# SDFIdk/malstroem

Measured on AMD Instinct MI355X. Metric: Mcells/s fill->D8->accum->label on 16384^2 f32 DEM, higher is better.
Workload: dtype f32 fill / f64 no-flats+D8+accum / u8 flowdir / i32 labels; 1 GPU; 16384x16384 float32 DEM (spectral fBm beta=2 seed 42 (SURVEY 8d recipe)): fill+depths -> no-flats fill -> D8 -> accumulation -> CCL+label_stats -> watersheds+label_count -> pour points; parallelism=1 GPU, one device context, fill_rounds=8, noflat_rounds=84, fill_tiles=70225, fill_visits=43501, fill_cycles=0, noflat_visits=412256, noflat_cycles=412256, nlabels=4637017, fill_algorithm=1, fill_launches=8, noflat_algorithm=2, pour_algorithm=1

## Files before the change

malstroem_amd/csrc/accum.hip:

```cpp
#include "common.hpp"
#include <type_traits>

namespace mh {
namespace {

constexpr int AT = 64;
constexpr int PERIM = 4 * AT - 4;
constexpr int NODE_STRIDE = 256;
constexpr int FS = AT + 32;
constexpr int WOFF = 16;
constexpr uint64_t SRC = 1ull << 63;
constexpr uint64_t TAINT = 1ull << 63;
constexpr uint32_t TAINT32 = 1u << 31;
constexpr int R_SHIFT = 13;
constexpr uint32_t A_MASK = 0x1fffu, R_MASK = 0xfffu, SENT13 = A_MASK;
constexpr uint16_t NO_EXIT = 0xffffu;
#ifndef ACC_ATN
#define ACC_ATN 256
#endif
constexpr int ATN = ACC_ATN;
constexpr int CPT = AT * AT / ATN;
constexpr int MAX_DOUBLINGS = 12;
constexpr int G_SHIFT = 44;
constexpr uint64_t G_ONE = 1ull << G_SHIFT, G_SUM = G_ONE - 1, G_PEND = 0x7ffffull;
// ... 614 lines not shown
        if (d != 0ull && (r0 + r) < H && (c0 + c) < W && !halo_row(r0 + r)) {
            const uint32_t kk = atomicAdd(&wl_n, 1u);
            wl_cell[kk] = (uint32_t)(r * AT + c);
            wl_add[kk] = d;
        }
    }
    for (int side = 0; side < 2; ++side) {
        const int64_t hr = side == 0 ? 0 : H - 1;
        if ((side == 0 ? !fixed_top : !fixed_bot) || hr < r0 || hr >= r0 + AT) continue;
        if (tid < AT && c0 + tid < W) {
            const int r = (int)(hr - r0), c = tid;
            const unsigned code = fd[hr * W + c0 + c];
            const double X = out[hr * W + c0 + c];
            if (code <= 7u && dir_dr((int)code) != 0 && X > 0.0) {
                const int nr = r + dir_dr((int)code), nc = c + dir_dc((int)code);
                if (nr >= 0 && nr < AT && nc >= 0 && nc < AT && (r0 + nr) < H && (c0 + nc) < W && !halo_row(r0 + nr)) {
                    const uint32_t kk = atomicAdd(&wl_n, 1u);
                    wl_cell[kk] = (uint32_t)(nr * AT + nc);
                    wl_add[kk] = (unsigned long long)X;
                }
            }
        }
    }
    __syncthreads();
    const uint32_t nw = wl_n;
    for (uint32_t w = tid; w < nw; w += ATN) {
        uint32_t a = wl_cell[w];
        const unsigned long long v = wl_add[w];
        do {
            if (S[a] == 0ull) break;
            atomicAdd(&S[a], v);
            a = P[a];
        } while (a != SENT13);
    }
    __syncthreads();
    for (int i = tid; i < AT * AT; i += ATN) {
        const int r = i / AT, c = i - r * AT;
        const int64_t rr = r0 + r, cc = c0 + c;
        if (rr < H && cc < W && !halo_row(rr)) out[rr * W + cc] = (double)S[i];
    }
}
}

int accum_band_delta_dev(const uint8_t *d_fd, double *d_out, int64_t H, int64_t W, hipStream_t s, int fixed_top, int fixed_bot, AccumKeep *keep, bool *done)
{
    *done = false;
    if (!keep || !keep->valid || keep->H != H || keep->W != W || keep->fixed_top != fixed_top || keep->fixed_bot != fixed_bot || !keep->nodes.p) return MHIP_OK;
    static const bool off = [] { const char *e = dev_env("MHIP_BAND_ACC"); return e && std::string(e) == "full"; }();
    if (off) return MHIP_OK;
    const int ntr = (int)cdiv(H, AT), ntc = (int)cdiv(W, AT);
    const int64_t ntiles = (int64_t)ntr * ntc, nnodes = ntiles * NODE_STRIDE;
    char *b = keep->nodes.as<char>();
    Nodes nd;
    nd.gstate = reinterpret_cast<uint64_t *>(b + keep->o[0]);
    nd.inflow = reinterpret_cast<uint64_t *>(b + keep->o[1]);
    nd.arrived = reinterpret_cast<uint32_t *>(b + keep->o[2]);
    nd.next = reinterpret_cast<int32_t *>(b + keep->o[3]);
    nd.dst = reinterpret_cast<int32_t *>(b + keep->o[4]);
    nd.exit_of = reinterpret_cast<uint16_t *>(b + keep->o[5]);
    nd.flags = reinterpret_cast<uint8_t *>(b + keep->o[6]);
    nd.halo_first = reinterpret_cast<int32_t *>(b + keep->o[7]);
    nd.bexit = reinterpret_cast<int32_t *>(b + keep->o[8]);
    DevBuf aux;
    MH_TRY(aux.alloc((size_t)ntiles + 64));
    uint8_t *touched = aux.as<uint8_t>() + 64;
    unsigned int *flag = aux.as<unsigned int>();
    MH_HIP(hipMemsetAsync(aux.p, 0, (size_t)ntiles + 64, s));
    MH_HIP(hipMemsetAsync(nd.inflow, 0, 8 * (size_t)nnodes, s));
    hipLaunchKernelGGL(accum_delta_graph_kernel, dim3((unsigned)cdiv(2 * W, 256)), dim3(256), 0, s, nd, d_fd, (const double *)d_out, H, W, ntc, ntiles, fixed_top,
                       fixed_bot, touched, flag);
    MH_HIP(hipGetLastError());
    unsigned int h_flag = 0;
    MH_HIP(hipMemcpyAsync(&h_flag, flag, 4, hipMemcpyDeviceToHost, s));
    MH_HIP(stream_sync(s));
    keep->valid = false;
    if (h_flag) return MHIP_OK;
    hipLaunchKernelGGL(accum_delta_tile_kernel, dim3((unsigned)ntiles), dim3(ATN), 0, s, d_fd, d_out, H, W, ntc, nd, fixed_top, fixed_bot, (const uint8_t *)touched);
    MH_HIP(hipGetLastError());
    MH_HIP(stream_sync(s));
    *done = true;
    return MHIP_OK;
}

int accum_dev(const uint8_t *d_fd, double *d_out, int64_t H, int64_t W, hipStream_t s, int fixed_top, int fixed_bot, int halo_zero,
              int32_t *d_exit_map, PourLink *pour, AccumKeep *keep)
{
    const int ntr = (int)cdiv(H, AT), ntc = (int)cdiv(W, AT);
    const int64_t ntiles = (int64_t)ntr * ntc, nnodes = ntiles * NODE_STRIDE;
    if (nnodes >= (int64_t)INT32_MAX || H * W >= (1ll << 37)) {
        set_error("accumulated_flow: raster too large for the int32 perimeter-node domain");
        return MHIP_ELIMIT;
    }
    DevBuf buf;
    auto align = [](size_t x) { return (x + 255) & ~size_t(255); };
    const size_t o_gstate = 0, o_inflow = align(o_gstate + 8 * (size_t)nnodes), o_arrived = align(o_inflow + 8 * (size_t)nnodes);
    const size_t o_next = align(o_arrived + 4 * (size_t)nnodes), o_dst = align(o_next + 4 * (size_t)nnodes);
    const size_t o_exit = align(o_dst + 4 * (size_t)nnodes), o_flags = align(o_exit + 2 * (size_t)nnodes);
    const size_t o_halo = align(o_flags + (size_t)nnodes);
    const size_t o_bexit = align(o_halo + (d_exit_map ? 8 * (size_t)W : 0));
    MH_TRY(buf.alloc(o_bexit + (d_exit_map ? 4 * (size_t)nnodes : 0)));
    char *b = buf.as<char>();
    Nodes nd;
    nd.gstate = reinterpret_cast<uint64_t *>(b + o_gstate);
    nd.inflow = reinterpret_cast<uint64_t *>(b + o_inflow);
    nd.arrived = reinterpret_cast<uint32_t *>(b + o_arrived);
    nd.next = reinterpret_cast<int32_t *>(b + o_next);
    nd.dst = reinterpret_cast<int32_t *>(b + o_dst);
    nd.exit_of = reinterpret_cast<uint16_t *>(b + o_exit);
    nd.flags = reinterpret_cast<uint8_t *>(b + o_flags);
    nd.halo_first = d_exit_map ? reinterpret_cast<int32_t *>(b + o_halo) : nullptr;
    nd.bexit = d_exit_map ? reinterpret_cast<int32_t *>(b + o_bexit) : nullptr;
    if (d_exit_map) MH_HIP(hipMemsetAsync(nd.halo_first, 0xff, 8 * (size_t)W, s));
    MH_HIP(hipMemsetAsync(nd.inflow, 0, o_next - o_inflow, s));
    const unsigned gn = (unsigned)cdiv(nnodes, 256);
    const bool walk_final = (!(fixed_top || fixed_bot) || halo_zero) && (!d_exit_map || halo_zero) && H * W < (int64_t)0x7fffffff;
    if (walk_final)
        hipLaunchKernelGGL((accum_tile_kernel<false, false, true>), dim3((unsigned)ntiles), dim3(ATN), 0, s, d_fd, d_out, H, W, ntc, nd, fixed_top, fixed_bot, halo_zero);
    else if ((fixed_top || fixed_bot) && !halo_zero)
        hipLaunchKernelGGL((accum_tile_kernel<false, true>), dim3((unsigned)ntiles), dim3(ATN), 0, s, d_fd, d_out, H, W, ntc, nd, fixed_top, fixed_bot, halo_zero);
    else
        hipLaunchKernelGGL((accum_tile_kernel<false, false>), dim3((unsigned)ntiles), dim3(ATN), 0, s, d_fd, d_out, H, W, ntc, nd, fixed_top, fixed_bot, halo_zero);
    hipLaunchKernelGGL(accum_link_kernel, dim3(gn), dim3(256), 0, s, nd, nnodes);
    if (d_exit_map)
        hipLaunchKernelGGL(accum_band_exit_kernel, dim3((unsigned)cdiv(2 * W, 256)), dim3(256), 0, s, nd, H, W, ntc, ntiles, fixed_top, fixed_bot, d_exit_map);
    hipLaunchKernelGGL(accum_mark_kernel, dim3(gn), dim3(256), 0, s, nd, nnodes);
    hipLaunchKernelGGL(accum_graph_walk_kernel, dim3(gn), dim3(256), 0, s, nd, nnodes);
    if (walk_final) {
        PourCandDev pc;
        if (pour && pour->wait && pour->wait(pour->arg) == 1 && pour->dev.key) {
            MH_HIP(hipStreamWaitEvent(s, pour->ev, 0));
            pc = pour->dev;
            pour->consumed = true;
        }
        hipLaunchKernelGGL(accum_final_walk_kernel, dim3((unsigned)ntiles), dim3(ATN), 0, s, d_fd, d_out, H, W, ntc, nd, pc, fixed_top, fixed_bot);
    }
    else if ((!(fixed_top || fixed_bot) || halo_zero) && H * W < (int64_t)0x7fffffff)
        hipLaunchKernelGGL((accum_tile_kernel<true, false>), dim3((unsigned)ntiles), dim3(ATN), 0, s, d_fd, d_out, H, W, ntc, nd, fixed_top, fixed_bot, halo_zero);
    else
        hipLaunchKernelGGL((accum_tile_kernel<true, true>), dim3((unsigned)ntiles), dim3(ATN), 0, s, d_fd, d_out, H, W, ntc, nd, fixed_top, fixed_bot, halo_zero);
    MH_HIP(hipGetLastError());
    MH_HIP(stream_sync(s));
    if (keep) {
        keep->valid = false;
        if (d_exit_map) {
            keep->nodes.release();
            keep->nodes.p = buf.p; keep->nodes.bytes = buf.bytes;
            buf.p = nullptr; buf.bytes = 0;
            const size_t offs[9] = {o_gstate, o_inflow, o_arrived, o_next, o_dst, o_exit, o_flags, o_halo, o_bexit};
            for (int k = 0; k < 9; ++k) keep->o[k] = offs[k];
            keep->H = H; keep->W = W; keep->fixed_top = fixed_top; keep->fixed_bot = fixed_bot;
            keep->valid = true;
        }
    }
#ifdef MH_PROFILE_ACCUM
    {
        unsigned long long pr[2][8];
        MH_HIP(hipMemcpyFromSymbol(pr, HIP_SYMBOL(g_accum_prof), sizeof(pr)));
        for (int f = 0; f < 2; ++f)
            fprintf(stderr, "[accum profile phase %d] ticks/tile (thread 0): load=%.0f init=%.0f solve=%.0f publish/write=%.0f\n", f ? 3 : 1,
                    pr[f][0] / (double)ntiles, pr[f][1] / (double)ntiles, pr[f][2] / (double)ntiles, pr[f][3] / (double)ntiles);
        unsigned long long z[2][8] = {};
        MH_HIP(hipMemcpyToSymbol(HIP_SYMBOL(g_accum_prof), z, sizeof(z)));
    }
#endif
    return MHIP_OK;
}

}
```

malstroem_amd/csrc/common.hpp:

```cpp
#pragma once
#include <hip/hip_runtime.h>
#include <cstdint>
#include <cstdio>
#include <cstring>
#include <string>
#include <vector>

#include "../../include/malstroem_hip.h"

struct mhip_polygons;
struct mhip_flowpaths;

namespace mh {

void set_error(const char *fmt, ...);
const char *get_error();
const char *dev_env(const char *name);
hipError_t stream_sync(hipStream_t s);
int require_device();

#define MH_HIP(expr)                                                                             \
    do {                                                                                         \
        hipError_t _e = (expr);                                                                  \
        if (_e != hipSuccess) {                                                                  \
// ... 164 lines not shown
};
void noflat_seed(FillRun &f, const float *d_filled, double sh, double dg, int64_t ncells_global);
struct PfRun;
struct FillHandover {
    PfRun *run = nullptr;
    const float *dem = nullptr;
    float *filled = nullptr, *depths = nullptr;
    int64_t H = 0, W = 0;
    const uint16_t *bslot = nullptr;
    const uint32_t *tabV = nullptr;
    int ntr = 0, ntc = 0;
    bool pending = false, queued = false, violated = false, repaired = false;
    bool suspect = false;
    FillStats st_repair;
    FillHandover() = default;
    FillHandover(const FillHandover &) = delete;
    FillHandover &operator=(const FillHandover &) = delete;
    ~FillHandover();
    void release();
};
int fill_handover_complete(FillHandover *ho, hipStream_t s);
int fill_handover_repair(FillHandover *ho, hipStream_t s);
int fill_plain_dev(const float *d_dem, float *d_out, int64_t H, int64_t W, hipStream_t s, FillStats *st, float *d_depths = nullptr,
                   bool *depths_done = nullptr, FillHandover *ho = nullptr);
int fill_check_f32_dev(const float *d_dem, const float *d_filled, int64_t H, int64_t W, int fixed_top, int fixed_bot, hipStream_t s,
                       unsigned int *d_flag);
int fill_plain_pflood_dev(const float *d_dem, float *d_out, float *d_depths, int64_t H, int64_t W, hipStream_t s, FillStats *st, bool *violated = nullptr,
                          uint32_t *overflow = nullptr, FillHandover *ho = nullptr);
struct PfRun {
    const float *dem = nullptr;
    float *out = nullptr;
    int64_t H = 0, W = 0;
    int fixed_top = 0, fixed_bot = 0;
    uint32_t overflow = 0;
    struct Impl;
    Impl *impl;
    PfRun();
    ~PfRun();
    PfRun(const PfRun &) = delete;
    PfRun &operator=(const PfRun &) = delete;
    int begin(hipStream_t s);
    int halo_changed(int side, hipStream_t s);
    int batch(hipStream_t s);
    int finish(hipStream_t s, float *d_depths, FillStats *st, bool *violated = nullptr, FillHandover *ho = nullptr);
    int finish_late(hipStream_t s, float *d_depths, bool *violated);
    int proof_flag(hipStream_t s, unsigned int *h_flag);
    int solve(hipStream_t s);
    int pack(hipStream_t s, int row0, int nrows);
    int publish_edges(hipStream_t s);
};
struct StageHook {
    enum Point { FIRST_VISIT = 0, TAIL_ROUNDS = 1, FINISH = 3 };
    void (*fn)(void *, hipStream_t) = nullptr;
    void *arg = nullptr;
    bool fired = false;
    int at = TAIL_ROUNDS;
    void fire(hipStream_t s)
    {
        if (fn && !fired) {
            fired = true;
            fn(arg, s);
        }
    }
    void fire_at(int point, hipStream_t s)
    {
        if (point == at) fire(s);
    }
};

struct GeoRun {
    const float *dem = nullptr, *filled = nullptr;
    double *out = nullptr;
    uint32_t *dist = nullptr;
    int64_t H = 0, W = 0;
    double sh = 0, dg = 0;
    int fixed_top = 0, fixed_bot = 0;
    bool allow_partial = false;
    double seed_add = 0;
    bool partial = false;
    StageHook *tail_hook = nullptr;
    uint8_t *d8_out = nullptr;
    unsigned int *d8_nodir = nullptr;
    bool d8_done = false;
    FillHandover *handover = nullptr;
    struct Impl;
    Impl *impl;
    GeoRun();
    ~GeoRun();
    GeoRun(const GeoRun &) = delete;
    GeoRun &operator=(const GeoRun &) = delete;
    int begin(hipStream_t s, bool *applicable, bool *active);
    int batch(hipStream_t s, bool *active);
    int halo_changed(int side, hipStream_t s);
    int end(hipStream_t s, bool *ok, FillStats *st);
    int launch_rounds(hipStream_t s, int nb);
};
struct D8Sink {
    uint8_t *flowdir = nullptr;
    unsigned int *nodir = nullptr;
    bool done = false;
};
int fill_noflat_geodesic_dev(const float *d_dem, const float *d_filled, double *d_out, int64_t H, int64_t W, double sh, double dg, double seed_add,
                             hipStream_t s, FillStats *st, bool *partial, StageHook *tail_hook = nullptr, D8Sink *d8 = nullptr, FillHandover *ho = nullptr);
int noflat_verify_dev(const float *d_dem, const double *d_out, int64_t H, int64_t W, double sh, double dg, hipStream_t s, bool *ok, int fixed_top = 0,
                      int fixed_bot = 0);
int fill_noflat_dev(const float *d_dem, double *d_out, int64_t H, int64_t W, double sh, double dg, hipStream_t s,
                    FillStats *st = nullptr, const float *d_filled = nullptr, StageHook *tail_hook = nullptr, D8Sink *d8 = nullptr,
                    FillHandover *ho = nullptr);
int short_diag_dev(const float *d_dem, int64_t n, double *sh, double *dg, hipStream_t s);
int depths_dev(const float *d_filled, const float *d_dem, float *d_out, int64_t n, hipStream_t s);
int d8_dev(const double *d_z, uint8_t *d_out, int64_t H, int64_t W, int edges_outward, hipStream_t s, int64_t row_off = 0,
           int64_t Hg = 0, unsigned int *d_interior_nodir = nullptr);
void short_diag_from_minmax(float mn, float mx, bool has_nan, double *sh, double *dg);
int minmax_dev(const float *d_x, int64_t n, float *mn, float *mx, int *has_nan, hipStream_t s);
int row_update_dev(void *d_dst, const void *d_src, int64_t nbytes, int *changed, hipStream_t s);
int copy_bandwidth_dev(size_t bytes, int reps, double *gbs, hipStream_t s);
int read_bandwidth_dev(size_t bytes, int reps, double *gbs, hipStream_t s);
int row_update_async(void *d_dst, const void *d_src, int64_t nbytes, int *d_changed, hipStream_t s);
int trace_downstream_dev(const uint8_t *d_fd, const int32_t *d_lab, int64_t H, int64_t W, const int64_t *d_cells, int64_t n, int use_bg,
                         int32_t bg, int32_t *d_label, int32_t *d_found, int64_t *d_len, const int64_t *d_offsets, int64_t *d_out_cells,
                         hipStream_t s);
int comm_unique_id(void *id128);
int comm_available();
int comm_create(void **comm, const void *id128, int rank, int nranks);
void comm_destroy(void *comm);
int comm_exchange_rows(void *comm, int rank, int nranks, const void *first_row, const void *last_row, void *stage, size_t rowbytes,
                       hipStream_t s);
int comm_allreduce_max(void *comm, double *d_value, hipStream_t s);
struct PourCandDev {
    uint16_t *mask0 = nullptr;
    uint2 *list = nullptr;
    uint32_t *tile_cnt = nullptr;
    unsigned long long *tile_key0 = nullptr;
    uint32_t *flags = nullptr;
    int components = 0;
    unsigned long long *key = nullptr;
    uint32_t nlab = 0;
};
constexpr uint32_t POUR_TILE_CAP = 512;
struct PourLink {
    PourCandDev dev;
    hipEvent_t ev = nullptr;
    void (*notify)(void *, int) = nullptr;
    int (*wait)(void *) = nullptr;
    void *arg = nullptr;
    bool consumed = false;
};
struct AccumKeep {
    DevBuf nodes;
    size_t o[9] = {};
    int64_t H = 0, W = 0;
    int fixed_top = 0, fixed_bot = 0;
    bool valid = false;
};
int accum_dev(const uint8_t *d_fd, double *d_out, int64_t H, int64_t W, hipStream_t s, int fixed_top = 0, int fixed_bot = 0, int halo_zero = 0,
              int32_t *d_exit_map = nullptr, PourLink *pour = nullptr, AccumKeep *keep = nullptr);
int accum_band_delta_dev(const uint8_t *d_fd, double *d_out, int64_t H, int64_t W, hipStream_t s, int fixed_top, int fixed_bot, AccumKeep *keep, bool *done);
int ccl8_f32_dev(const float *d_data, int32_t *d_labels, int32_t *d_tmp, int64_t H, int64_t W, int64_t *nlabels,
                 hipStream_t s, DevBuf *stats_out = nullptr);
int label_emit_stats_dev(const int32_t *d_parent, const unsigned long long *d_rootbits, const uint32_t *d_wordprefix, const float *d_data,
                         int32_t *d_labels, int64_t H, int64_t W, int64_t nlab, mhip_stat_record *d_rec, hipStream_t s);
int ccl8_u8_dev(const uint8_t *d_data, int32_t *d_labels, int32_t *d_tmp, int64_t H, int64_t W, int64_t *nlabels,
                hipStream_t s);
struct CclKeep {
    DevBuf bits, wprefix;
    int64_t H = 0, W = 0, nlocal = 0;
    bool valid = false;
};
int ccl8_f32_begin_dev(const float *d_data, int32_t *d_labels, int32_t *d_tmp, int64_t H, int64_t W, int64_t *nlabels, hipStream_t s, CclKeep *keep);
int ccl_emit_rows_dev(const int32_t *d_parent, const unsigned long long *d_rootbits, const uint32_t *d_wordprefix, int32_t *d_labels, int64_t base,
                      int64_t count, hipStream_t s);
int label_emit_sparse_dev(const int32_t *d_parent, const unsigned long long *d_rootbits, const uint32_t *d_wordprefix, const float *d_data,
                          int32_t *d_labels, int64_t H, int64_t W, int ht, int64_t H_owned, int64_t nlocal, int32_t offset,
                          const int32_t *d_dropped, const int32_t *d_target, int32_t ndropped, int64_t nlab_global, mhip_stat_record *d_rec,
                          hipStream_t s);
int relabel_lut_dev(int32_t *d_labels, const int32_t *d_lut, int64_t nlab, int64_t n, hipStream_t s);
int relabel_range_dev(int32_t *d_labels, int64_t n, int32_t lo, int32_t hi, const int32_t *d_lut, const int32_t *d_fid, const int32_t *d_fnew, int32_t nf,
                      hipStream_t s);
int band_trace_dev(const uint8_t *d_fd, const int32_t *d_lab, int64_t Hl, int64_t W, int64_t row_lo, int64_t own0, int64_t own1, int64_t Hg,
                   const int64_t *d_cells, const int32_t *d_src, int64_t n, int use_bg, int32_t bg, int32_t *d_label, int32_t *d_status,
                   int32_t *d_src_out, int64_t *d_exit, int64_t *d_len, const int64_t *d_offsets, int64_t *d_out_cells, hipStream_t s);
int relabel_sparse_dev(int32_t *d_labels, int64_t n, int64_t nlocal, int32_t offset, const int32_t *d_dropped, const int32_t *d_target,
                       int32_t ndropped, hipStream_t s);
int keep_mask_dev(const int32_t *d_labels, const uint8_t *d_keep, int64_t nlab, int64_t n, uint8_t *d_mask,
                  hipStream_t s);
int label_stats_dev(const float *d_data, const int32_t *d_labels, int64_t n, int64_t nlab, mhip_stat_record *d_rec,
                    hipStream_t s, int64_t W = 0, bool components = false);
int label_stats64_dev(const double *d_data, const int32_t *d_labels, int64_t n, int64_t nlab, mhip_stat_record *d_rec, hipStream_t s);
int label_stats_zero_sign_dev(const float *d_data, const int32_t *d_labels, int64_t n, int64_t nlab, mhip_stat_record *d_rec, hipStream_t s);
int label_stats_zero_sign_dev(const double *d_data, const int32_t *d_labels, int64_t n, int64_t nlab, mhip_stat_record *d_rec, hipStream_t s);
int label_arg_dev(const double *d_data, const int32_t *d_labels, int64_t H, int64_t W, int64_t nlab, bool is_max,
                  mhip_index_record *d_rec, hipStream_t s, bool components = false);
int label_count_dev(const int32_t *d_labels, int64_t n, int64_t nlab, int64_t *d_counts, hipStream_t s, int64_t W = 0);
int label_max_dev(const int32_t *d_labels, int64_t n, int32_t *out_max, hipStream_t s);
constexpr int64_t HYPS_MAX_BINS = (int64_t)1 << 30;
int hyps_layout_dev(const double *d_dmax, int64_t stride, int64_t nlab, double res, int64_t *d_offsets, int64_t *total, hipStream_t s);
int hyps_table_dev(const float *d_data, const int32_t *d_labels, int64_t n, int64_t W, int64_t nlab, double res, const int64_t *d_offsets,
                   int64_t total, uint32_t *d_counts, double *d_sums, int64_t *lds_spills, hipStream_t s, hipEvent_t ev0 = nullptr,
                   hipEvent_t ev1 = nullptr);
int hyps_levels_dev(int64_t nlab, const int64_t *d_offsets, const uint32_t *d_counts, const double *d_sums, const double *d_dmax, int64_t stride,
                    const double *d_q, mhip_final_record *d_rec, hipStream_t s);
int final_depths_dev(const float *d_data, const int32_t *d_labels, int64_t n, int64_t W, int64_t nlab, mhip_final_record *d_rec, float *d_out,
                     hipStream_t s, hipEvent_t ev0 = nullptr, hipEvent_t ev1 = nullptr);
bool wet_at_events_ok(int64_t K, const float *values);
int wet_at_dev(const float *d_data, const int32_t *d_labels, int64_t n, int64_t W, int64_t nlab, int K, const double *d_drawdown, int64_t stride,
               const float *values, float *d_out, int64_t *d_wet, int64_t wet_stride, hipStream_t s, hipEvent_t ev0 = nullptr,
               hipEvent_t ev1 = nullptr);
bool flow_distance_scale_ok(double scale);
int flow_distance_dev(const uint8_t *d_fd, const int32_t *d_lab, int64_t H, int64_t W, double scale, int64_t nlab, float *d_out, mhip_index_record *d_rec,
                      int64_t *unresolved, hipStream_t s);
int burn_check(int64_t nseg, const mhip_burn_segment *segs, int64_t nline, const mhip_burn_line *lines, const mhip_burn_result *results);
int burn_lines_dev(float *d_dem, int64_t H, int64_t W, int64_t nseg, const mhip_burn_segment *segs, int64_t nline, const mhip_burn_line *lines,
                   double nodata, mhip_burn_result *results, hipStream_t s);
int zones_check(int64_t H, int64_t W, int64_t nvert, const double *xy, int64_t nring, const int64_t *ring_offsets, const int32_t *ring_zone,
                int64_t nzone, int grow);
int zones_rasterize_dev(int32_t *d_out, int64_t H, int64_t W, int64_t nvert, const double *xy, int64_t nring, const int64_t *ring_offsets,
                        const int32_t *ring_zone, int64_t nzone, int grow, hipStream_t s);
int zone_stats_dev(const float *d_data, const int32_t *d_zones, int64_t n, int64_t W, int64_t nzone, mhip_zone_record *d_rec, hipStream_t s);
int polygonize_check(int64_t H, int64_t W);
int polygons_fetch_dev(const mhip_polygons *p, int32_t *xy, int64_t *ring_offsets, int32_t *ring_label);
int polygonize_dev(const int32_t *d_lab, int64_t H, int64_t W, DevBuf &d_xy, DevBuf &d_off, DevBuf &d_rl, int64_t *nring, int64_t *nvert, hipStream_t s);
int flowpaths_check(int64_t H, int64_t W, double threshold);
int flowpaths_dev(const uint8_t *d_fd, const double *d_acc, const int32_t *d_lab, int64_t H, int64_t W, double threshold, mhip_flowpaths *p, hipStream_t s);
int flowpaths_fetch_dev(const mhip_flowpaths *p, int32_t *xy, int64_t *reach_offsets, mhip_reach_record *records);
int watersheds_dev(const uint8_t *d_fd, int32_t *d_labels, int64_t H, int64_t W, int32_t unassigned, hipStream_t s,
                   bool band_mode = false, const unsigned int *d_known_interior_nodir = nullptr, const int32_t *d_src = nullptr, PourLink *pour = nullptr);
int pour_finish_dev(unsigned long long *d_key, const unsigned long long *d_tile_key0, int64_t ntiles, int64_t nlab, int64_t W, mhip_index_record *d_rec,
                    hipStream_t s);
int band_pseudo_labels_dev(int32_t *d_ws, int64_t H, int64_t W, int top, int bottom, hipStream_t s);
int negative_lut_dev(int32_t *d_lab, int64_t n, const int32_t *d_lut, int64_t nlut, hipStream_t s);
constexpr int32_t BAND_ROOT = 1, BAND_ROOTLESS = 0x7fffffff;
int band_root_labels_dev(int32_t *d_out, int64_t H, int64_t W, int64_t row_off, int64_t Hg, hipStream_t s);
int band_hide_rootless_dev(const int32_t *d_lab, const int32_t *d_rooted, int32_t *d_out, int64_t n, hipStream_t s);
int band_show_rootless_dev(int32_t *d_ws, const int32_t *d_lab, int64_t n, hipStream_t s);

__host__ __device__ inline int64_t cdiv(int64_t a, int64_t b) { return (a + b - 1) / b; }

constexpr int TR = 32;
struct TileGeom {
// ... 88 lines not shown
```

malstroem_amd/csrc/ctx.hip:

```cpp
#include <mutex>
#include <new>
#include <string>
#include <vector>

#include "ctx.hpp"

namespace mh {

static void drop_hyps(mhip_ctx *c)
{
    c->hyps_total = -1;
    c->have[MHIP_R_FINALDEPTHS] = false;
    c->wetat_events = -1;
    c->wetat_out.release();
}

static void drop_flow_distance(mhip_ctx *c)
{
    std::lock_guard<std::mutex> lk(c->fdist_mu);
    c->fdist_unresolved = -1;
    c->fdist_out.release();
    c->fdist_rec.release();
}

void ctx_wrote(mhip_ctx *c, int which, bool uploaded)
{
    switch (which) {
    case MHIP_R_DEM:
        for (int k = 0; k < MHIP_R_COUNT_; ++k) {
            if (k == MHIP_R_DEM) continue;
            c->have[k] = false;
            ctx_wrote(c, k, true);
        }
        break;
    case MHIP_R_FILLED:
        if (uploaded) c->fill_st.have_minmax = false;
        break;
    case MHIP_R_DEPTHS:
        c->stats_valid = false;
        drop_hyps(c);
        break;
    case MHIP_R_NOFLAT:
        c->pour_valid = false;
        break;
    case MHIP_R_FLOWDIR:
        c->nodir_valid = false;
        c->flowdir_own = false;
        c->acc_keep.valid = false;
        drop_flow_distance(c);
        break;
    case MHIP_R_ACCUM:
        c->acc_keep.valid = false;
        c->pour_valid = false;
        break;
    case MHIP_R_LABELS:
        c->nlabels = c->nlabels_raw = -1;
        c->labels_components = false;
        c->stats_valid = false;
        c->ws_counts_valid = false;
        c->pour_valid = false;
        drop_hyps(c);
        drop_flow_distance(c);
        break;
    case MHIP_R_WATERSHEDS:
        c->ws_counts_valid = false;
        break;
    default:
        break;
    }
}

int ctx_copy_rows(mhip_ctx *c, void *dev_base, size_t elem_bytes, int64_t row0, int64_t nrows, void *host, hipMemcpyKind kind)
{
    MH_HIP(hipSetDevice(c->device));
    const size_t rowb = elem_bytes * (size_t)c->W;
    char *dev = (char *)dev_base + rowb * (size_t)(c->ht + row0);
    const bool up = kind == hipMemcpyHostToDevice;
    MH_HIP(hipMemcpyAsync(up ? (void *)dev : host, up ? host : (void *)dev, rowb * (size_t)nrows, kind, cs(c)));
    MH_HIP(stream_sync(cs(c)));
    return MHIP_OK;
}

int ctx_fetch(mhip_ctx *c, const DevBuf &buf, size_t bytes, void *host)
{
    MH_HIP(hipSetDevice(c->device));
    return download(host, buf, bytes, c->stream);
}

int ctx_fork_join_events(mhip_ctx *c)
{
    if (c->ev_fork) return MHIP_OK;
    for (hipEvent_t *e : {&c->ev_flowdir, &c->ev_join, &c->ev_label, &c->ev_tail, &c->ev_fork}) MH_HIP(hipEventCreateWithFlags(e, hipEventDisableTiming));
    return MHIP_OK;
}

int ctx_ensure_labels_final(mhip_ctx *c, hipStream_t s)
{
    if (!c->labels_filtered) return ctx_apply_keep_on(c, nullptr, s);
    return MHIP_OK;
}

int ctx_label_max(mhip_ctx *c, hipStream_t s)
{
    if (c->nlabels < 0) {
        int32_t m = 0;
        MH_TRY(label_max_dev(c->r[MHIP_R_LABELS].as<int32_t>(), c->H * c->W, &m, s));
        c->nlabels = m < 0 ? 0 : m;
    }
    return MHIP_OK;
}

int ctx_apply_keep_on(mhip_ctx *c, const uint8_t *keep, hipStream_t s)
{
    MH_ARG(c && c->have[MHIP_R_LABELS] && c->nlabels_raw >= 0 && !c->labels_filtered, "ctx_apply_keep needs a fresh LABEL run");
    const int64_t n = c->H * c->W;
    const int64_t nraw = c->nlabels_raw;
    const bool components = c->labels_components;
    ctx_wrote(c, MHIP_R_LABELS);
    c->nlabels_raw = nraw;
    c->labels_components = components;
    if (keep) {
        std::vector<int32_t> lut;
        c->nlabels = build_rank_lut(keep, c->nlabels_raw, lut);
        DevBuf d_lut;
        MH_TRY(d_lut.alloc(lut.size() * 4));
        MH_HIP(hipMemcpyAsync(d_lut.p, lut.data(), lut.size() * 4, hipMemcpyHostToDevice, s));
        MH_TRY(relabel_lut_dev(c->r[MHIP_R_LABELS].as<int32_t>(), d_lut.as<int32_t>(), c->nlabels_raw, n, s));
        MH_TRY(c->stats.alloc(sizeof(mhip_stat_record) * (size_t)(c->nlabels + 1)));
        MH_TRY(label_stats_dev(c->r[MHIP_R_DEPTHS].as<float>(), c->r[MHIP_R_LABELS].as<int32_t>(), n, c->nlabels,
                               c->stats.as<mhip_stat_record>(), s, c->W, c->labels_components));
    } else {
        c->nlabels = c->nlabels_raw;
        MH_TRY(c->stats.alloc(sizeof(mhip_stat_record) * (size_t)(c->nlabels + 1)));
        MH_HIP(hipMemcpyAsync(c->stats.p, c->raw_stats.p, sizeof(mhip_stat_record) * (size_t)(c->nlabels + 1),
                              hipMemcpyDeviceToDevice, s));
    }
    c->labels_filtered = true;
    c->stats_valid = true;
    return MHIP_OK;
}

}

using namespace mh;

extern "C" {

int mhip_comm_available(void) { return comm_available(); }

int mhip_comm_unique_id(void *id128)
{
    MH_ARG(id128, "comm_unique_id(id128)");
    MH_TRY(require_device());
    return comm_unique_id(id128);
}

int mhip_ctx_create_band(mhip_ctx **out, int64_t H_global, int64_t W, int64_t row0, int64_t H_local, int device, int rank,
                         int nranks, const void *nccl_unique_id)
{
    MH_ARG(out && H_global >= 1 && W >= 1 && H_local >= 1 && row0 >= 0 && row0 + H_local <= H_global, "ctx_create_band geometry");
    MH_ARG(rank >= 0 && nranks >= 1 && rank < nranks, "ctx_create_band(rank, nranks)");
    MH_TRY(require_device());
    MH_HIP(hipSetDevice(device));
    void *comm = nullptr;
    if (nccl_unique_id) MH_TRY(comm_create(&comm, nccl_unique_id, rank, nranks));
    mhip_ctx *c = new mhip_ctx();
    c->comm = comm;
    c->ht = row0 > 0 ? 1 : 0;
    c->hb = row0 + H_local < H_global ? 1 : 0;
    c->H_owned = H_local;
    c->H = H_local + c->ht + c->hb;
    c->W = W; c->H_global = H_global; c->row0 = row0;
    c->device = device; c->rank = rank; c->nranks = nranks;
    int prio_least = 0, prio_greatest = 0;
    (void)hipDeviceGetStreamPriorityRange(&prio_least, &prio_greatest);
    if (hipStreamCreateWithPriority(&c->stream, hipStreamDefault, prio_greatest) != hipSuccess) {
        comm_destroy(c->comm);
        delete c;
        set_error("hipStreamCreate failed");
        return MHIP_EHIP;
    }
    *out = c;
    return MHIP_OK;
}

int mhip_ctx_create(mhip_ctx **out, int64_t H, int64_t W, int device)
{
    return mhip_ctx_create_band(out, H, W, 0, H, device, 0, 1, nullptr);
}

int mhip_ctx_destroy(mhip_ctx *c)
{
    if (!c) return MHIP_OK;
    (void)hipSetDevice(c->device);
    (void)stream_sync(c->stream);
    for (StageTimer &t : c->timers)
        for (hipEvent_t e : {t.a, t.b})
            if (e) (void)hipEventDestroy(e);
    (void)hipStreamDestroy(c->stream);
    for (hipStream_t st : {c->stream_b, c->stream_c}) {
        if (st) {
            (void)stream_sync(st);
            (void)hipStreamDestroy(st);
        }
    }
    for (hipEvent_t e : {c->ev_fork, c->ev_flowdir, c->ev_join, c->ev_label, c->ev_tail, c->ev_cand})
        if (e) (void)hipEventDestroy(e);
    delete c->geo;
    delete c->pf;
    delete c->run[0];
    delete c->run[1];
    comm_destroy(c->comm);
    comm_destroy(c->comm_b);
    delete c;
    return MHIP_OK;
}

int mhip_ctx_comm_add_side(mhip_ctx *c, const void *nccl_unique_id)
{
    MH_ARG(c && nccl_unique_id && c->comm && !c->comm_b, "ctx_comm_add_side(ctx, id) needs a band context with a communicator and no side communicator yet");
    MH_HIP(hipSetDevice(c->device));
    return comm_create(&c->comm_b, nccl_unique_id, c->rank, c->nranks);
}

int mhip_ctx_side_begin(mhip_ctx *c)
{
    MH_ARG(c, "ctx");
    MH_HIP(hipSetDevice(c->device));
    if (!c->stream_b) MH_HIP(hipStreamCreateWithFlags(&c->stream_b, hipStreamNonBlocking));
    MH_TRY(ctx_fork_join_events(c));
    MH_HIP(hipEventRecord(c->ev_fork, c->stream));
    MH_HIP(hipStreamWaitEvent(c->stream_b, c->ev_fork, 0));
    t_side_ctx = c;
    return MHIP_OK;
}

int mhip_ctx_side_end(mhip_ctx *c)
{
    MH_ARG(c && t_side_ctx == c, "ctx_side_end without ctx_side_begin on this thread");
    MH_HIP(hipSetDevice(c->device));
    MH_HIP(stream_sync(c->stream_b));
    t_side_ctx = nullptr;
    return MHIP_OK;
}

int mhip_ctx_upload(mhip_ctx *c, int which, const void *host)
{
    MH_ARG(c && host && which >= 0 && which < MHIP_R_COUNT_, "ctx_upload(ctx, which, host)");
    return mhip_ctx_upload_rows(c, which, 0, c->H_owned, host);
}

int mhip_ctx_upload_dem(mhip_ctx *c, const float *dem) { return mhip_ctx_upload(c, MHIP_R_DEM, dem); }

int mhip_ctx_upload_rows(mhip_ctx *c, int which, int64_t row0, int64_t nrows, const void *host)
{
    MH_ARG(c && host && which >= 0 && which < MHIP_R_COUNT_ && row0 >= 0 && nrows >= 1 && row0 + nrows <= c->H_owned,
           "ctx_upload_rows(ctx, which, row0, nrows, host)");
    MH_HIP(hipSetDevice(c->device));
    MH_TRY(ctx_raster(c, which));
    ctx_wrote(c, which, true);
    c->have[which] = false;
    MH_TRY(ctx_copy_rows(c, c->r[which].p, raster_elem(which), row0, nrows, const_cast<void *>(host), hipMemcpyHostToDevice));
    if (row0 + nrows == c->H_owned) {
        c->have[which] = true;
        if (which == MHIP_R_LABELS) c->labels_filtered = true;
    }
    return MHIP_OK;
}

int mhip_ctx_download_rows(mhip_ctx *c, int which, int64_t row0, int64_t nrows, void *host)
{
    MH_ARG(c && host && which >= 0 && which < MHIP_R_COUNT_ && row0 >= 0 && nrows >= 1 && row0 + nrows <= c->H_owned,
           "ctx_download_rows(ctx, which, row0, nrows, host)");
    MH_ARG(c->have[which], "raster has not been computed or uploaded");
    return ctx_copy_rows(c, c->r[which].p, raster_elem(which), row0, nrows, host, hipMemcpyDeviceToHost);
}

int mhip_ctx_download(mhip_ctx *c, int which, void *host)
{
    MH_ARG(c && host && which >= 0 && which < MHIP_R_COUNT_, "ctx_download(ctx, which, host)");
    return mhip_ctx_download_rows(c, which, 0, c->H_owned, host);
}

int mhip_ctx_trace_downstream(mhip_ctx *c, const int64_t *cells_rc, int64_t n, int use_background, int32_t background, int32_t *out_label,
                              int32_t *out_found, int64_t *out_len, const int64_t *offsets, int64_t *out_cells)
{
    MH_ARG(c && n >= 0 && (n == 0 || cells_rc), "ctx_trace_downstream(ctx, cells, n, ...)");
    MH_ARG(c->have[MHIP_R_FLOWDIR] && c->have[MHIP_R_LABELS], "ctx_trace_downstream needs flow directions and labels");
    MH_ARG(!c->ht && !c->hb, "stream tracing runs on an undivided raster");
    if (n == 0) return MHIP_OK;
    MH_HIP(hipSetDevice(c->device));
    return trace_on_device(c->r[MHIP_R_FLOWDIR].as<uint8_t>(), c->r[MHIP_R_LABELS].as<int32_t>(), c->H, c->W, cells_rc, n, use_background,
                           background, out_label, out_found, out_len, offsets, out_cells, c->stream);
}

int mhip_ctx_sync(mhip_ctx *c)
{
    MH_ARG(c, "ctx");
    MH_HIP(stream_sync(c->stream));
    return MHIP_OK;
}

int mhip_ctx_stage_ms(mhip_ctx *c, int stage, float *ms)
{
    MH_ARG(c && ms, "ctx_stage_ms(ctx, stage, ms)");
    const int k = timer_slot(stage);
    MH_ARG(k >= 0 && c->timers[k].valid, "stage has not been run");
    MH_HIP(hipEventSynchronize(c->timers[k].b));
    MH_HIP(hipEventElapsedTime(ms, c->timers[k].a, c->timers[k].b));
    return MHIP_OK;
}

int mhip_ctx_kernel_ms(mhip_ctx *c, const char *kernel, float *ms_total, int32_t *launches)
{
    MH_ARG(c && kernel && ms_total && launches, "ctx_kernel_ms(ctx, kernel, ms, launches)");
    const std::string k(kernel);
    if (k == "d8") {
        *launches = 1;
        return mhip_ctx_stage_ms(c, MHIP_STAGE_FLOWDIR, ms_total);
    }
    if (k == "d8_steady") {
        MH_ARG(c->have[MHIP_R_NOFLAT] && !c->ht && !c->hb, "d8_steady needs the no-flats surface on an undivided context");
        MH_HIP(hipSetDevice(c->device));
        MH_TRY(ctx_raster(c, MHIP_R_FLOWDIR));
        MH_TRY(c->nodir_cnt.alloc(4));
        constexpr int REPS = 16;
        StageTimer *t;
        MH_TRY(ctx_timer(c, D8_STEADY_SLOT, &t));
        hipStream_t s = c->stream;
        ctx_wrote(c, MHIP_R_FLOWDIR);
        MH_HIP(hipMemsetAsync(c->nodir_cnt.p, 0, 4, s));
        for (int i = 0; i < REPS + 2; ++i) {
            if (i == 2) MH_HIP(hipEventRecord(t->a, s));
            MH_TRY(d8_dev(c->r[MHIP_R_NOFLAT].as<double>(), c->r[MHIP_R_FLOWDIR].as<uint8_t>(), c->H, c->W, 1, s, 0, c->H_global,
                          c->nodir_cnt.as<unsigned int>()));
        }
        MH_HIP(hipEventRecord(t->b, s));
        MH_HIP(hipEventSynchronize(t->b));
        MH_HIP(hipEventElapsedTime(ms_total, t->a, t->b));
        c->have[MHIP_R_FLOWDIR] = true;
        c->nodir_valid = true;
        c->flowdir_own = true;
        *launches = REPS;
        return MHIP_OK;
    }
    if (k == "hyps_table" || k == "final_depths") {
        *launches = 1;
        return mhip_ctx_stage_ms(c, k == "hyps_table" ? HYPS_KERNEL_SLOT : FINAL_KERNEL_SLOT, ms_total);
    }
    if (k == "wet_at") {
        *launches = 1;
        return mhip_ctx_stage_ms(c, WETAT_KERNEL_SLOT, ms_total);
    }
    if (k == "fill_round") {
        *launches = c->fill_rounds;
        return mhip_ctx_stage_ms(c, MHIP_STAGE_FILL, ms_total);
    }
    if (k == "noflat_round") {
        *launches = c->noflat_rounds;
        return mhip_ctx_stage_ms(c, MHIP_STAGE_NOFLAT, ms_total);
    }
    set_error("unknown kernel family '%s'", kernel);
    return MHIP_EINVAL;
}

int mhip_ctx_get_i64(mhip_ctx *c, const char *key, int64_t *value)
{
    MH_ARG(c && key && value, "ctx_get_i64(ctx, key, value)");
    const std::string k(key);
    if (k == "nlabels_raw") *value = c->nlabels_raw;
    else if (k == "nlabels") {
        if (c->nlabels < 0 && c->have[MHIP_R_LABELS]) {
            MH_HIP(hipSetDevice(c->device));
            MH_TRY(ctx_label_max(c, c->stream));
        }
        *value = c->nlabels;
    }
    else if (k == "fill_rounds") *value = c->fill_rounds;
    else if (k == "noflat_rounds") *value = c->noflat_rounds;
    else if (k == "fill_visits") *value = c->fill_st.visits;
    else if (k == "fill_cycles") *value = c->fill_st.cycles;
    else if (k == "fill_tiles") *value = c->fill_st.tiles;
    else if (k == "fill_algorithm") *value = c->fill_st.algorithm;
    else if (k == "fill_handover") *value = c->fill_handover;
    else if (k == "fill_handover_rechecks") *value = c->fill_handover_rechecks;
    else if (k == "fill_overflow") *value = c->fill_st.overflow;
    else if (k == "fill_launches") *value = c->fill_st.rounds;
    else if (k == "fill_hot_launches") *value = c->fill_st.hot_launches;
    else if (k == "noflat_hot_launches") *value = c->noflat_st.hot_launches;
    else if (k == "accum_algorithm") *value = c->accum_algorithm;
    else if (k == "flowdir_computed") *value = (c->have[MHIP_R_FLOWDIR] && c->flowdir_own) ? 1 : 0;
    else if (k == "pour_algorithm") *value = c->pour_algorithm;
    else if (k == "noflat_algorithm") *value = c->noflat_st.algorithm;
    else if (k == "noflat_visits") *value = c->noflat_st.visits;
    else if (k == "noflat_reject") *value = c->noflat_st.geo_reject;
    else if (k == "noflat_reject_irregular") *value = c->noflat_st.geo_irregular;
    else if (k == "noflat_reject_unreached") *value = c->noflat_st.geo_unreached;
    else if (k == "noflat_reject_mismatch") *value = c->noflat_st.geo_mismatch;
    else if (k == "noflat_cycles") *value = c->noflat_st.cycles;
    else if (k == "hyps_bins") *value = c->hyps_total;
    else if (k == "hyps_lds_spills") *value = c->hyps_spills;
    else if (k == "wet_at_events") *value = c->wetat_events;
    else if (k == "flow_distance_unresolved") *value = c->fdist_unresolved;
    else if (k == "zones") *value = c->nzone;
    else if (k == "H") *value = c->H;
    else if (k == "W") *value = c->W;
    else {
        set_error("unknown key '%s'", key);
        return MHIP_EINVAL;
    }
    return MHIP_OK;
}

int mhip_ctx_get_f64(mhip_ctx *c, const char *key, double *value)
{
    MH_ARG(c && key && value, "ctx_get_f64(ctx, key, value)");
    const std::string k(key);
    if (k == "short") *value = c->sh;
    else if (k == "diag") *value = c->dg;
    else if (k == "fill_hot_ms") *value = c->fill_st.hot_ms;
    else if (k == "noflat_hot_ms") *value = c->noflat_st.hot_ms;
    else {
        set_error("unknown key '%s'", key);
        return MHIP_EINVAL;
    }
    return MHIP_OK;
}

int mhip_ctx_raw_stats(mhip_ctx *c, mhip_stat_record *records)
{
    MH_ARG(c && records && c->raw_stats.p && c->nlabels_raw >= 0, "ctx_raw_stats needs a LABEL run");
    return ctx_fetch(c, c->raw_stats, sizeof(mhip_stat_record) * (size_t)(c->nlabels_raw + 1), records);
}

int mhip_ctx_apply_keep(mhip_ctx *c, const uint8_t *keep)
{
    MH_ARG(c, "ctx");
    MH_HIP(hipSetDevice(c->device));
    return ctx_apply_keep_on(c, keep, c->stream);
}

int mhip_ctx_stats(mhip_ctx *c, mhip_stat_record *records)
{
    MH_ARG(c && records && c->stats_valid && c->labels_filtered, "ctx_stats needs LABEL + apply_keep (or mhip_ctx_hyps) on the resident depths and labels");
    return ctx_fetch(c, c->stats, sizeof(mhip_stat_record) * (size_t)(c->nlabels + 1), records);
}

int mhip_ctx_watershed_counts(mhip_ctx *c, int64_t *counts)
{
    MH_ARG(c && counts && c->ws_counts_valid, "ctx_watershed_counts needs a WATERSHED run on the resident labels");
    return ctx_fetch(c, c->ws_counts, 8 * (size_t)(c->nlabels + 1), counts);
}

int mhip_ctx_pourpoints(mhip_ctx *c, mhip_index_record *records)
{
    MH_ARG(c && records && c->pour_valid, "ctx_pourpoints needs a POURPOINTS run on the resident labels and accumulated flow");
    return ctx_fetch(c, c->pour, sizeof(mhip_index_record) * (size_t)(c->nlabels + 1), records);
}

int mhip_ctx_hyps(mhip_ctx *c, double res, int64_t *total)
{
    MH_ARG(c && total && hyps_res_ok(res), "ctx_hyps(ctx, 0 < res < inf, total)");
    MH_ARG(!(c->nranks > 1 || c->ht || c->hb), "hypsometry on a row band is not built (the tables of the bands add up: a later step); use an undivided context");
    MH_ARG(c->have[MHIP_R_DEPTHS] && c->have[MHIP_R_LABELS] && !c->ccl_pending, "ctx_hyps needs the DEPTHS and LABELS rasters");
    MH_ARG(c->labels_filtered, "ctx_hyps needs mhip_ctx_apply_keep after the LABEL run");
    MH_HIP(hipSetDevice(c->device));
    hipStream_t s = c->stream;
    const int64_t n = c->H * c->W;
    c->hyps_total = -1;
    if (!c->stats_valid) {
        MH_TRY(ctx_label_max(c, s));
        MH_TRY(c->stats.alloc(sizeof(mhip_stat_record) * (size_t)(c->nlabels + 1)));
        MH_TRY(label_stats_dev(c->r[MHIP_R_DEPTHS].as<float>(), c->r[MHIP_R_LABELS].as<int32_t>(), n, c->nlabels, c->stats.as<mhip_stat_record>(), s,
                               c->W, c->labels_components));
        c->stats_valid = true;
    }
// ... 252 lines not shown
```

malstroem_amd/csrc/ctx.hpp:

```cpp
#pragma once
#include <atomic>
#include <condition_variable>
#include <functional>
#include <mutex>
#include <thread>

#include "common.hpp"

namespace mh {

class SideThread {
    std::thread th_;
    std::mutex mu_;
    std::condition_variable cv_;
    std::function<void()> task_;
    bool busy_ = false, stop_ = false;

public:
    ~SideThread()
    {
        {
            std::lock_guard<std::mutex> lk(mu_);
            stop_ = true;
        }
        cv_.notify_all();
        if (th_.joinable()) th_.join();
    }
    void run(std::function<void()> f)
    {
        std::unique_lock<std::mutex> lk(mu_);
        if (!th_.joinable())
            th_ = std::thread([this] {
                std::unique_lock<std::mutex> l2(mu_);
                for (;;) {
                    cv_.wait(l2, [this] { return stop_ || (busy_ && task_); });
                    if (stop_) return;
                    std::function<void()> f2 = std::move(task_);
                    task_ = nullptr;
                    l2.unlock();
                    f2();
                    l2.lock();
                    busy_ = false;
                    cv_.notify_all();
                }
            });
        task_ = std::move(f);
        busy_ = true;
        cv_.notify_all();
    }
    void wait()
    {
        std::unique_lock<std::mutex> lk(mu_);
        cv_.wait(lk, [this] { return !busy_; });
    }
};

struct StageTimer {
    hipEvent_t a = nullptr, b = nullptr;
    bool valid = false;
};
constexpr int N_STAGE_BITS = 9;
constexpr int WETAT_KERNEL_SLOT = 1 << 27, FINAL_KERNEL_SLOT = 1 << 28, HYPS_KERNEL_SLOT = 1 << 29, D8_STEADY_SLOT = 1 << 30;
constexpr int N_TIMERS = N_STAGE_BITS + 4;

}

struct mhip_ctx {
    mh::SideThread side;
    int64_t H = 0, W = 0;
    int64_t H_global = 0, row0 = 0, H_owned = 0;
    int ht = 0, hb = 0;
    mh::FillRun *run[2] = {nullptr, nullptr};
    mh::GeoRun *geo = nullptr;
    uint32_t pf_overflow = 0;
    mh::PfRun *pf = nullptr;
    bool pf_done = false;
    mh::DevBuf nodir_cnt;
    bool nodir_valid = false;
    bool flowdir_own = false;
    int device = 0, rank = 0, nranks = 1;
    hipStream_t stream = nullptr;
    mh::DevBuf r[MHIP_R_COUNT_];
    bool have[MHIP_R_COUNT_] = {};
    mh::DevBuf tmp_i32;
    mh::CclKeep ccl_keep;
    bool ccl_pending = false;
    bool pf_depths = false;
    mh::DevBuf raw_stats, stats, ws_counts, pour;
    mh::AccumKeep acc_keep;
    int accum_algorithm = 0;
    mh::DevBuf pp_mask0, pp_list, pp_tiles, pp_misc, pp_key;
    hipEvent_t ev_cand = nullptr;
    int pour_algorithm = 0;
    int64_t nlabels_raw = -1, nlabels = -1;
    bool labels_components = false;
    bool labels_filtered = false;
    std::atomic<bool> stats_valid{false};
    std::atomic<bool> ws_counts_valid{false};
    std::atomic<bool> pour_valid{false};
    mh::DevBuf hyps_off, hyps_cnt, hyps_sum, hyps_rec;
    int64_t hyps_total = -1, hyps_spills = 0;
    mh::DevBuf wetat_out;
    int wetat_events = -1;
    mh::DevBuf fdist_out, fdist_rec;
    std::atomic<int64_t> fdist_unresolved{-1};
    std::mutex fdist_mu;
    mh::DevBuf zones;
    int64_t nzone = -1;
    double sh = 0, dg = 0;
    int32_t fill_rounds = 0, noflat_rounds = 0;
    int64_t fill_handover_rechecks = 0;
    int32_t fill_handover = 0;
    mh::FillStats fill_st, noflat_st;
    mh::StageTimer timers[mh::N_TIMERS];
    void *comm = nullptr;
    void *comm_b = nullptr;
    mh::DevBuf comm_stage, comm_word, comm_flags, comm_stage_b;
    hipStream_t stream_b = nullptr, stream_c = nullptr;
    hipEvent_t ev_fork = nullptr, ev_flowdir = nullptr, ev_join = nullptr, ev_label = nullptr, ev_tail = nullptr;
};

namespace mh {

inline size_t raster_elem(int which)
{
    switch (which) {
    case MHIP_R_DEM: case MHIP_R_FILLED: case MHIP_R_DEPTHS: case MHIP_R_LABELS: case MHIP_R_WATERSHEDS: case MHIP_R_NGDIST:
    case MHIP_R_FINALDEPTHS: return 4;
    case MHIP_R_NOFLAT: case MHIP_R_ACCUM: return 8;
    case MHIP_R_FLOWDIR: return 1;
    default: return 0;
    }
}

inline int ctx_raster(mhip_ctx *c, int which)
{
    if (!c->r[which].p) MH_TRY(c->r[which].alloc(raster_elem(which) * (size_t)(c->H * c->W)));
    return MHIP_OK;
}

inline int timer_slot(int stage)
{
    for (int b = 0; b < N_STAGE_BITS; ++b)
        if (stage == 1 << b) return b;
    return stage == FINAL_KERNEL_SLOT ? N_STAGE_BITS : stage == HYPS_KERNEL_SLOT ? N_STAGE_BITS + 1 : stage == D8_STEADY_SLOT ? N_STAGE_BITS + 2 :
           stage == WETAT_KERNEL_SLOT ? N_STAGE_BITS + 3 : -1;
}
inline int ctx_timer(mhip_ctx *c, int stage, StageTimer **t)
{
    const int k = timer_slot(stage);
    MH_ARG(k >= 0, "not a stage");
    *t = &c->timers[k];
    if (!(*t)->a) {
        hipEvent_t e0, e1;
        MH_HIP(hipEventCreate(&e0));
        MH_HIP(hipEventCreate(&e1));
        (*t)->a = e0;
        (*t)->b = e1;
    }
    return MHIP_OK;
}
inline int stage_begin(mhip_ctx *c, int stage, hipStream_t s)
{
    StageTimer *t;
    MH_TRY(ctx_timer(c, stage, &t));
    MH_HIP(hipEventRecord(t->a, s));
    return MHIP_OK;
}
inline int stage_end(mhip_ctx *c, int stage, hipStream_t s)
{
    StageTimer &t = c->timers[timer_slot(stage)];
    MH_HIP(hipEventRecord(t.b, s));
    t.valid = true;
    return MHIP_OK;
}

inline thread_local mhip_ctx *t_side_ctx = nullptr;
static inline hipStream_t cs(mhip_ctx *c) { return (t_side_ctx == c && c->stream_b) ? c->stream_b : c->stream; }
static inline bool on_side(mhip_ctx *c) { return t_side_ctx == c; }

void ctx_wrote(mhip_ctx *c, int which, bool uploaded = false);
int ctx_copy_rows(mhip_ctx *c, void *dev_base, size_t elem_bytes, int64_t row0, int64_t nrows, void *host, hipMemcpyKind kind);
int ctx_fetch(mhip_ctx *c, const DevBuf &buf, size_t bytes, void *host);
int ctx_fork_join_events(mhip_ctx *c);
int ctx_apply_keep_on(mhip_ctx *c, const uint8_t *keep, hipStream_t s);
int ctx_ensure_labels_final(mhip_ctx *c, hipStream_t s);
int ctx_label_max(mhip_ctx *c, hipStream_t s);

}
```

malstroem_amd/csrc/ctx_band.hip:

```cpp
#include <string>

#include "ctx.hpp"

using namespace mh;

static size_t row_bytes(mhip_ctx *c, int which) { return raster_elem(which) * (size_t)c->W; }
static char *row_ptr(mhip_ctx *c, int which, int side)
{
    const int64_t row = side == 0 ? c->ht : side == 1 ? c->ht + c->H_owned - 1 : side == 2 ? 0 : c->H - 1;
    return c->r[which].as<char>() + row_bytes(c, which) * (size_t)row;
}

static int update_halo_rows(mhip_ctx *c, int which, const void *top, const void *bottom, int *d_flags, int32_t *changed, hipStream_t s)
{
    const int64_t rowb = (int64_t)row_bytes(c, which);
    MH_HIP(hipMemsetAsync(d_flags, 0, 8, s));
    if (top) MH_TRY(row_update_async(row_ptr(c, which, 2), top, rowb, d_flags, s));
    if (bottom) MH_TRY(row_update_async(row_ptr(c, which, 3), bottom, rowb, d_flags + 1, s));
    int h[2] = {0, 0};
    MH_HIP(hipMemcpyAsync(h, d_flags, 8, hipMemcpyDeviceToHost, s));
    MH_HIP(stream_sync(s));
    changed[0] = h[0];
    changed[1] = h[1];
    return MHIP_OK;
}

static int copy_edge_rows(mhip_ctx *c, int which, int side0, void *dst0, int side1, void *dst1, hipMemcpyKind kind, const char *usage)
{
    MH_ARG(c && which >= 0 && which < MHIP_R_COUNT_, usage);
    MH_ARG(c->r[which].p, "raster has not been computed or uploaded");
    const int side[2] = {side0, side1};
    void *const dst[2] = {dst0, dst1};
    for (int k = 0; k < 2; ++k) MH_ARG(!dst[k] || side[k] < 2 || (side[k] == 2 ? c->ht : c->hb), "this band has no halo row on that side");
    if (!dst0 && !dst1) return MHIP_OK;
    MH_HIP(hipSetDevice(c->device));
    hipStream_t s = cs(c);
    for (int k = 0; k < 2; ++k)
        if (dst[k]) MH_HIP(hipMemcpyAsync(dst[k], row_ptr(c, which, side[k]), row_bytes(c, which), kind, s));
    MH_HIP(stream_sync(s));
    return MHIP_OK;
}

static void labels_renumbered(mhip_ctx *c, int64_t nlabels)
{
    const bool components = c->labels_components;
    ctx_wrote(c, MHIP_R_LABELS);
    c->labels_components = components;
    c->nlabels = c->nlabels_raw = nlabels;
    c->labels_filtered = true;
}

static FillRun *new_fill_run(mhip_ctx *c, int kind)
{
    delete c->run[kind];
    FillRun *f = c->run[kind] = new FillRun();
    f->noflat = kind != 0;
    f->dem = c->r[MHIP_R_DEM].as<float>();
    f->out = c->r[kind ? MHIP_R_NOFLAT : MHIP_R_FILLED].p;
    f->H = c->H; f->W = c->W;
    f->fixed_top = c->ht; f->fixed_bot = c->hb;
    f->rounds_per_batch = 16;
    return f;
}
static bool fill_begun(mhip_ctx *c, int kind) { return c->run[kind] || (kind == 0 && (c->pf || c->pf_done)); }

extern "C" {


int mhip_ctx_band_info(mhip_ctx *c, int64_t *row_off, int64_t *rows_local, int32_t *halo_top, int32_t *halo_bottom)
{
    MH_ARG(c, "ctx");
    if (row_off) *row_off = c->row0 - c->ht;
    if (rows_local) *rows_local = c->H;
    if (halo_top) *halo_top = c->ht;
    if (halo_bottom) *halo_bottom = c->hb;
    return MHIP_OK;
}

int mhip_ctx_get_edge_row(mhip_ctx *c, int which, int side, void *host)
{
    static const char *const usage = "ctx_get_edge_row(ctx, which, side, host)";
    MH_ARG(host && side >= 0 && side <= 3, usage);
    return copy_edge_rows(c, which, side, host, 0, nullptr, hipMemcpyDeviceToHost, usage);
}

int mhip_ctx_set_halo_row(mhip_ctx *c, int which, int side, const void *host, int32_t *changed)
{
    MH_ARG(c && host && which >= 0 && which < MHIP_R_COUNT_ && (side == 0 || side == 1), "ctx_set_halo_row(ctx, which, side, host)");
    MH_ARG(side == 0 ? c->ht : c->hb, "this band has no halo row on that side");
    int32_t ch[2];
    MH_TRY(mhip_ctx_set_halo_rows(c, which, side == 0 ? host : nullptr, side == 1 ? host : nullptr, ch));
    if (changed) *changed = ch[side];
    return MHIP_OK;
}

int mhip_ctx_get_edge_row_dev(mhip_ctx *c, int which, int side, void *dev_dst)
{
    static const char *const usage = "ctx_get_edge_row_dev(ctx, which, side, dev)";
    MH_ARG(dev_dst && side >= 0 && side <= 3, usage);
    return copy_edge_rows(c, which, side, dev_dst, 0, nullptr, hipMemcpyDeviceToDevice, usage);
}

int mhip_ctx_set_halo_row_dev(mhip_ctx *c, int which, int side, const void *dev_src, int32_t *changed)
{
    MH_ARG(c && dev_src && which >= 0 && which < MHIP_R_COUNT_ && (side == 0 || side == 1), "ctx_set_halo_row_dev(ctx, which, side, dev)");
    MH_ARG(side == 0 ? c->ht : c->hb, "this band has no halo row on that side");
    MH_HIP(hipSetDevice(c->device));
    MH_TRY(ctx_raster(c, which));
    int ch = 0;
    MH_TRY(row_update_dev(row_ptr(c, which, 2 + side), dev_src, (int64_t)row_bytes(c, which), &ch, cs(c)));
    if (changed) *changed = ch;
    return MHIP_OK;
}

int mhip_ctx_get_edge_rows(mhip_ctx *c, int which, void *host_first, void *host_last)
{
    return copy_edge_rows(c, which, 0, host_first, 1, host_last, hipMemcpyDeviceToHost, "ctx_get_edge_rows(ctx, which, first, last)");
}

int mhip_ctx_set_halo_rows(mhip_ctx *c, int which, const void *host_top, const void *host_bottom, int32_t *changed)
{
    MH_ARG(c && changed && which >= 0 && which < MHIP_R_COUNT_, "ctx_set_halo_rows(ctx, which, top, bottom, changed[2])");
    MH_ARG((!host_top || c->ht) && (!host_bottom || c->hb), "this band has no halo row on that side");
    changed[0] = changed[1] = 0;
    if (!host_top && !host_bottom) return MHIP_OK;
    MH_HIP(hipSetDevice(c->device));
    MH_TRY(ctx_raster(c, which));
    hipStream_t s = cs(c);
    const size_t rowb = row_bytes(c, which);
    DevBuf &stage = on_side(c) ? c->comm_stage_b : c->comm_stage;
    DevBuf flags;
    MH_TRY(stage.alloc(2 * rowb));
    MH_TRY(flags.alloc(8));
    char *top = stage.as<char>(), *bottom = top + rowb;
    if (host_top) MH_HIP(hipMemcpyAsync(top, host_top, rowb, hipMemcpyHostToDevice, s));
    if (host_bottom) MH_HIP(hipMemcpyAsync(bottom, host_bottom, rowb, hipMemcpyHostToDevice, s));
    return update_halo_rows(c, which, host_top ? top : nullptr, host_bottom ? bottom : nullptr, flags.as<int>(), changed, s);
}

int mhip_ctx_exchange_halo(mhip_ctx *c, int which, int32_t *changed)
{
    MH_ARG(c && changed && which >= 0 && which < MHIP_R_COUNT_, "ctx_exchange_halo(ctx, which, changed[2])");
    MH_ARG(c->comm || c->nranks == 1, "this band context has no RCCL communicator (created without an ncclUniqueId)");
    changed[0] = changed[1] = 0;
    if (!c->ht && !c->hb) return MHIP_OK;
    MH_ARG(c->r[which].p, "raster has not been computed or uploaded");
    MH_HIP(hipSetDevice(c->device));
    hipStream_t s = cs(c);
    const size_t rowb = row_bytes(c, which);
    MH_TRY(c->comm_stage.alloc(2 * rowb));
    MH_TRY(c->comm_flags.alloc(8));
    char *from_up = c->comm_stage.as<char>(), *from_down = from_up + rowb;
    MH_TRY(comm_exchange_rows(c->comm, c->rank, c->nranks, row_ptr(c, which, 0), row_ptr(c, which, 1), from_up, rowb, s));
    return update_halo_rows(c, which, c->ht ? from_up : nullptr, c->hb ? from_down : nullptr, c->comm_flags.as<int>(), changed, s);
}

int mhip_ctx_exchange_edge_rows(mhip_ctx *c, int which, void *host_from_up, void *host_from_down)
{
    MH_ARG(c && which >= 0 && which < MHIP_R_COUNT_, "ctx_exchange_edge_rows(ctx, which, from_up, from_down)");
    void *comm = on_side(c) ? c->comm_b : c->comm;
    MH_ARG(comm || c->nranks == 1, on_side(c) ? "this band context has no side communicator (mhip_ctx_comm_add_side)"
                                              : "this band context has no RCCL communicator (created without an ncclUniqueId)");
    if (!c->ht && !c->hb) return MHIP_OK;
    MH_ARG(c->r[which].p, "raster has not been computed or uploaded");
    MH_ARG((!c->ht || host_from_up) && (!c->hb || host_from_down), "ctx_exchange_edge_rows: a buffer per neighbour");
    MH_HIP(hipSetDevice(c->device));
    hipStream_t s = cs(c);
    const size_t rowb = row_bytes(c, which);
    DevBuf &stage = on_side(c) ? c->comm_stage_b : c->comm_stage;
    MH_TRY(stage.alloc(2 * rowb));
    MH_TRY(comm_exchange_rows(comm, c->rank, c->nranks, row_ptr(c, which, 0), row_ptr(c, which, 1), stage.p, rowb, s));
    if (c->ht) MH_HIP(hipMemcpyAsync(host_from_up, stage.p, rowb, hipMemcpyDeviceToHost, s));
    if (c->hb) MH_HIP(hipMemcpyAsync(host_from_down, stage.as<char>() + rowb, rowb, hipMemcpyDeviceToHost, s));
    MH_HIP(stream_sync(s));
    return MHIP_OK;
}

int mhip_ctx_allreduce_max(mhip_ctx *c, double value, double *out)
{
    MH_ARG(c && out, "ctx_allreduce_max(ctx, value, out)");
    if (c->nranks == 1 && !c->comm) {
        *out = value;
        return MHIP_OK;
    }
    MH_ARG(c->comm, "this band context has no RCCL communicator (created without an ncclUniqueId)");
    MH_HIP(hipSetDevice(c->device));
    hipStream_t s = cs(c);
    MH_TRY(c->comm_word.alloc(8));
    MH_HIP(hipMemcpyAsync(c->comm_word.p, &value, 8, hipMemcpyHostToDevice, s));
    MH_TRY(comm_allreduce_max(c->comm, c->comm_word.as<double>(), s));
    MH_HIP(hipMemcpyAsync(out, c->comm_word.p, 8, hipMemcpyDeviceToHost, s));
    MH_HIP(stream_sync(s));
    return MHIP_OK;
}

int mhip_ctx_has_comm(mhip_ctx *c) { return (c && c->comm) ? ((c->comm_b) ? 2 : 1) : 0; }

int mhip_ctx_zero_raster(mhip_ctx *c, int which)
{
    MH_ARG(c && which >= 0 && which < MHIP_R_COUNT_, "ctx_zero_raster(ctx, which)");
    MH_HIP(hipSetDevice(c->device));
    MH_TRY(ctx_raster(c, which));
    ctx_wrote(c, which);
    MH_HIP(hipMemsetAsync(c->r[which].p, 0, raster_elem(which) * (size_t)(c->H * c->W), cs(c)));
    return MHIP_OK;
}

int mhip_ctx_band_accum_boundary(mhip_ctx *c, int32_t *exit_map)
{
    MH_ARG(c && exit_map && c->have[MHIP_R_FLOWDIR], "ctx_band_accum_boundary(ctx, exit_map[2 * W]) needs flow directions");
    MH_HIP(hipSetDevice(c->device));
    MH_TRY(ctx_raster(c, MHIP_R_ACCUM));
    DevBuf d_map;
    MH_TRY(d_map.alloc(8 * (size_t)c->W));
    ctx_wrote(c, MHIP_R_ACCUM);
    MH_TRY(accum_dev(c->r[MHIP_R_FLOWDIR].as<uint8_t>(), c->r[MHIP_R_ACCUM].as<double>(), c->H, c->W, cs(c), c->ht, c->hb, 1,
                     d_map.as<int32_t>(), nullptr, &c->acc_keep));
    MH_HIP(hipMemcpyAsync(exit_map, d_map.p, 8 * (size_t)c->W, hipMemcpyDeviceToHost, cs(c)));
    MH_HIP(stream_sync(cs(c)));
    return MHIP_OK;
}

int mhip_ctx_band_ccl_local(mhip_ctx *c, int64_t *nlocal)
{
    MH_ARG(c && nlocal && c->have[MHIP_R_DEPTHS], "ctx_band_ccl_local needs bluespot depths");
    MH_HIP(hipSetDevice(c->device));
    MH_TRY(ctx_raster(c, MHIP_R_LABELS));
    if (!c->tmp_i32.p) MH_TRY(c->tmp_i32.alloc(4 * (size_t)(c->H * c->W)));
    ctx_wrote(c, MHIP_R_LABELS);
    MH_TRY(ccl8_f32_dev(c->r[MHIP_R_DEPTHS].as<float>(), c->r[MHIP_R_LABELS].as<int32_t>(), c->tmp_i32.as<int32_t>(), c->H, c->W,
                        nlocal, cs(c)));
    c->nlabels_raw = *nlocal;
    c->have[MHIP_R_LABELS] = true;
    c->labels_components = true;
    c->labels_filtered = false;
    return MHIP_OK;
}

int mhip_ctx_band_relabel(mhip_ctx *c, const int32_t *lut, int64_t nlocal, int64_t nlabels_global)
{
    MH_ARG(c && lut && nlocal >= 0 && c->have[MHIP_R_LABELS], "ctx_band_relabel(ctx, lut, nlocal, nglobal)");
    MH_HIP(hipSetDevice(c->device));
    DevBuf d_lut;
    MH_TRY(d_lut.alloc(4 * (size_t)(nlocal + 1)));
    MH_HIP(hipMemcpyAsync(d_lut.p, lut, 4 * (size_t)(nlocal + 1), hipMemcpyHostToDevice, cs(c)));
    MH_TRY(relabel_lut_dev(c->r[MHIP_R_LABELS].as<int32_t>(), d_lut.as<int32_t>(), nlocal, c->H * c->W, cs(c)));
    labels_renumbered(c, nlabels_global);
    return MHIP_OK;
}

int mhip_ctx_band_relabel_sparse(mhip_ctx *c, int64_t nlocal, int64_t offset, const int32_t *dropped, const int32_t *target,
                                 int64_t ndropped, int64_t nlabels_global)
{
    MH_ARG(c && nlocal >= 0 && ndropped >= 0 && (ndropped == 0 || (dropped && target)) && c->have[MHIP_R_LABELS] &&
               offset + nlocal < (int64_t)INT32_MAX, "ctx_band_relabel_sparse");
    for (int64_t k = 1; k < ndropped; ++k) MH_ARG(dropped[k - 1] < dropped[k], "ctx_band_relabel_sparse: dropped labels must be sorted and unique");
    MH_HIP(hipSetDevice(c->device));
    DevBuf d_d, d_t;
    MH_TRY(d_d.alloc(4 * (size_t)(ndropped + 1)));
    MH_TRY(d_t.alloc(4 * (size_t)(ndropped + 1)));
    if (ndropped) {
        MH_HIP(hipMemcpyAsync(d_d.p, dropped, 4 * (size_t)ndropped, hipMemcpyHostToDevice, cs(c)));
        MH_HIP(hipMemcpyAsync(d_t.p, target, 4 * (size_t)ndropped, hipMemcpyHostToDevice, cs(c)));
    }
    MH_TRY(relabel_sparse_dev(c->r[MHIP_R_LABELS].as<int32_t>(), c->H * c->W, nlocal, (int32_t)offset, d_d.as<int32_t>(), d_t.as<int32_t>(),
                              (int32_t)ndropped, cs(c)));
    labels_renumbered(c, nlabels_global);
    return MHIP_OK;
}

int mhip_ctx_band_ccl_begin(mhip_ctx *c, int64_t *nlocal)
{
    MH_ARG(c && nlocal && c->have[MHIP_R_DEPTHS], "ctx_band_ccl_begin needs bluespot depths");
    MH_HIP(hipSetDevice(c->device));
    MH_TRY(ctx_raster(c, MHIP_R_LABELS));
    ctx_wrote(c, MHIP_R_LABELS);
    c->have[MHIP_R_LABELS] = false;
    if (!c->tmp_i32.p) MH_TRY(c->tmp_i32.alloc(4 * (size_t)(c->H * c->W)));
    MH_TRY(ccl8_f32_begin_dev(c->r[MHIP_R_DEPTHS].as<float>(), c->r[MHIP_R_LABELS].as<int32_t>(), c->tmp_i32.as<int32_t>(), c->H, c->W,
                              nlocal, cs(c), &c->ccl_keep));
    c->ccl_keep.nlocal = *nlocal;
    c->ccl_pending = true;
    return MHIP_OK;
}

// ... 150 lines not shown
        MH_HIP(stream_sync(s));
        c->have[MHIP_R_WATERSHEDS] = true;
        return MHIP_OK;
    }
    c->have[MHIP_R_WATERSHEDS] = false;
    DevBuf tmp, zero;
    MH_TRY(tmp.alloc(4 * (size_t)n));
    MH_TRY(zero.alloc(4));
    MH_HIP(hipMemsetAsync(zero.p, 0, 4, s));
    if (step == 1) MH_TRY(band_root_labels_dev(tmp.as<int32_t>(), c->H, c->W, c->row0 - c->ht, c->H_global, s));
    else MH_TRY(band_hide_rootless_dev(lab, ws, tmp.as<int32_t>(), n, s));
    MH_TRY(band_pseudo_labels_dev(tmp.as<int32_t>(), c->H, c->W, c->ht, c->hb, s));
    MH_TRY(watersheds_dev(c->r[MHIP_R_FLOWDIR].as<uint8_t>(), ws, c->H, c->W, 0, s, true, zero.as<unsigned int>(), tmp.as<int32_t>(), nullptr));
    MH_HIP(stream_sync(s));
    return MHIP_OK;
}

int mhip_ctx_band_apply_neg_lut(mhip_ctx *c, int which, const int32_t *lut, int64_t n)
{
    MH_ARG(c && lut && n >= 1 && (which == MHIP_R_WATERSHEDS || which == MHIP_R_LABELS) && c->r[which].p, "ctx_band_apply_neg_lut");
    MH_HIP(hipSetDevice(c->device));
    if (which == MHIP_R_LABELS) labels_renumbered(c, c->nlabels);
    else ctx_wrote(c, which);
    DevBuf d_lut;
    MH_TRY(d_lut.alloc(4 * (size_t)n));
    MH_HIP(hipMemcpyAsync(d_lut.p, lut, 4 * (size_t)n, hipMemcpyHostToDevice, cs(c)));
    MH_TRY(negative_lut_dev(c->r[which].as<int32_t>(), c->H * c->W, d_lut.as<int32_t>(), n, cs(c)));
    MH_HIP(stream_sync(cs(c)));
    return MHIP_OK;
}

namespace {
__global__ void global_rows_kernel(mhip_index_record *rec, int64_t n, int64_t row0)
{
    const int64_t i = (int64_t)blockIdx.x * blockDim.x + threadIdx.x;
    if (i < n && rec[i].row >= 0) rec[i].row += row0;
}
__global__ void gather_bytes_kernel(const char *src, const int64_t *ids, int64_t nids, int elem, char *dst)
{
    const int64_t i = (int64_t)blockIdx.x * blockDim.x + threadIdx.x;
    if (i >= nids * elem) return;
    dst[i] = src[ids[i / elem] * elem + i % elem];
}
__global__ void foreign_counts_kernel(const int64_t *cnt, int64_t n, int64_t lo, int64_t hi, int64_t cap, int64_t *ids, int64_t *vals,
                                      unsigned long long *nout)
{
    const int64_t i = (int64_t)blockIdx.x * blockDim.x + threadIdx.x;
    if (i <= 0 || i >= n || (i >= lo && i <= hi)) return;
    const int64_t v = cnt[i];
    if (v <= 0) return;
    const unsigned long long k = atomicAdd(nout, 1ull);
    if ((int64_t)k < cap) {
        ids[k] = i;
        vals[k] = v;
    }
}
}

static size_t band_record_size(int which) { return which == 0 ? sizeof(mhip_stat_record) : which == 1 ? 8 : sizeof(mhip_index_record); }
static DevBuf &band_record_buf(mhip_ctx *c, int which) { return which == 0 ? c->stats : which == 1 ? c->ws_counts : c->pour; }
static std::atomic<bool> &band_record_valid(mhip_ctx *c, int which) { return which == 0 ? c->stats_valid : which == 1 ? c->ws_counts_valid : c->pour_valid; }
static const char *const BAND_RECORDS_MISSING = "the record set needs mhip_ctx_band_records(which) on the resident rasters (which 0: or mhip_ctx_band_ccl_finish with statistics)";

int mhip_ctx_band_records(mhip_ctx *c, int which)
{
    MH_ARG(c && which >= 0 && which <= 3 && c->have[MHIP_R_LABELS] && c->nlabels >= 0, "ctx_band_records(ctx, which) needs global labels");
    MH_HIP(hipSetDevice(c->device));
    const int64_t off = c->W * c->ht, n = c->H_owned * c->W, nrec = c->nlabels + 1;
    DevBuf &buf = band_record_buf(c, which);
    MH_TRY(buf.alloc(band_record_size(which) * (size_t)nrec));
    if (which == 0) {
        MH_ARG(c->have[MHIP_R_DEPTHS], "label_stats needs the depths");
        MH_TRY(label_stats_dev(c->r[MHIP_R_DEPTHS].as<float>() + off, c->r[MHIP_R_LABELS].as<int32_t>() + off, n, c->nlabels,
                               buf.as<mhip_stat_record>(), cs(c), c->W, c->labels_components));
        if (!c->labels_components)
            MH_TRY(label_stats_zero_sign_dev(c->r[MHIP_R_DEPTHS].as<float>() + off, c->r[MHIP_R_LABELS].as<int32_t>() + off, n, c->nlabels,
                                             buf.as<mhip_stat_record>(), cs(c)));
    } else if (which == 1) {
        MH_ARG(c->have[MHIP_R_WATERSHEDS], "watershed counts need the watersheds");
        MH_TRY(label_count_dev(c->r[MHIP_R_WATERSHEDS].as<int32_t>() + off, n, c->nlabels, buf.as<int64_t>(), cs(c), c->W));
    } else {
        const int src = which == 2 ? MHIP_R_ACCUM : MHIP_R_NOFLAT;
        MH_ARG(c->have[src], which == 2 ? "pour points need the accumulated flow" : "pour points need the no-flats surface");
        MH_TRY(label_arg_dev(c->r[src].as<double>() + off, c->r[MHIP_R_LABELS].as<int32_t>() + off, c->H_owned, c->W, c->nlabels,
                             which == 2, buf.as<mhip_index_record>(), cs(c), c->labels_components));
        hipLaunchKernelGGL(global_rows_kernel, dim3((unsigned)cdiv(nrec, 256)), dim3(256), 0, cs(c), buf.as<mhip_index_record>(), nrec,
                           c->row0);
        MH_HIP(hipGetLastError());
    }
    band_record_valid(c, which) = true;
    return MHIP_OK;
}

int mhip_ctx_band_fetch(mhip_ctx *c, int which, int64_t first, int64_t count, void *out)
{
    MH_ARG(c && which >= 0 && which <= 3 && first >= 0 && count >= 0 && (out || count == 0), "ctx_band_fetch(ctx, which, first, count, out)");
    MH_ARG(band_record_valid(c, which), BAND_RECORDS_MISSING);
    MH_ARG(first + count <= c->nlabels + 1, "ctx_band_fetch: records outside [0, nlabels]");
    if (count == 0) return MHIP_OK;
    MH_HIP(hipSetDevice(c->device));
    const size_t e = band_record_size(which);
    MH_HIP(hipMemcpyAsync(out, band_record_buf(c, which).as<char>() + e * (size_t)first, e * (size_t)count, hipMemcpyDeviceToHost, cs(c)));
    MH_HIP(stream_sync(cs(c)));
    return MHIP_OK;
}

int mhip_ctx_band_gather(mhip_ctx *c, int which, const int64_t *ids, int64_t nids, void *out)
{
    MH_ARG(c && which >= 0 && which <= 3 && nids >= 0 && ((ids && out) || nids == 0), "ctx_band_gather");
    MH_ARG(band_record_valid(c, which), BAND_RECORDS_MISSING);
    if (nids == 0) return MHIP_OK;
    for (int64_t k = 0; k < nids; ++k) MH_ARG(ids[k] >= 0 && ids[k] <= c->nlabels, "ctx_band_gather: label outside [0, nlabels]");
    MH_HIP(hipSetDevice(c->device));
    const int e = (int)band_record_size(which);
    DevBuf d_ids, d_out;
    MH_TRY(d_ids.alloc(8 * (size_t)nids));
    MH_TRY(d_out.alloc((size_t)e * (size_t)nids));
    MH_HIP(hipMemcpyAsync(d_ids.p, ids, 8 * (size_t)nids, hipMemcpyHostToDevice, cs(c)));
    hipLaunchKernelGGL(gather_bytes_kernel, dim3((unsigned)cdiv(nids * e, 256)), dim3(256), 0, cs(c), band_record_buf(c, which).as<char>(),
                       d_ids.as<int64_t>(), nids, e, d_out.as<char>());
    MH_HIP(hipGetLastError());
    MH_HIP(hipMemcpyAsync(out, d_out.p, (size_t)e * (size_t)nids, hipMemcpyDeviceToHost, cs(c)));
    MH_HIP(stream_sync(cs(c)));
    return MHIP_OK;
}

int mhip_ctx_band_foreign_counts(mhip_ctx *c, int64_t lo, int64_t hi, int64_t cap, int64_t *ids, int64_t *counts, int64_t *nfound)
{
    MH_ARG(c && cap >= 0 && nfound && ((ids && counts) || cap == 0), "ctx_band_foreign_counts");
    MH_ARG(c->ws_counts_valid, BAND_RECORDS_MISSING);
    MH_HIP(hipSetDevice(c->device));
    DevBuf d_ids, d_vals, d_n;
    MH_TRY(d_ids.alloc(8 * (size_t)(cap + 1)));
    MH_TRY(d_vals.alloc(8 * (size_t)(cap + 1)));
    MH_TRY(d_n.alloc(8));
    MH_HIP(hipMemsetAsync(d_n.p, 0, 8, cs(c)));
    const int64_t nrec = c->nlabels + 1;
    hipLaunchKernelGGL(foreign_counts_kernel, dim3((unsigned)cdiv(nrec, 256)), dim3(256), 0, cs(c), c->ws_counts.as<int64_t>(), nrec, lo, hi,
                       cap, d_ids.as<int64_t>(), d_vals.as<int64_t>(), d_n.as<unsigned long long>());
    MH_HIP(hipGetLastError());
    unsigned long long k = 0;
    MH_HIP(hipMemcpyAsync(&k, d_n.p, 8, hipMemcpyDeviceToHost, cs(c)));
    MH_HIP(stream_sync(cs(c)));
    *nfound = (int64_t)k;
    const int64_t take = (int64_t)k < cap ? (int64_t)k : cap;
    if (take > 0) {
        MH_HIP(hipMemcpyAsync(ids, d_ids.p, 8 * (size_t)take, hipMemcpyDeviceToHost, cs(c)));
        MH_HIP(hipMemcpyAsync(counts, d_vals.p, 8 * (size_t)take, hipMemcpyDeviceToHost, cs(c)));
        MH_HIP(stream_sync(cs(c)));
    }
    return MHIP_OK;
}

int mhip_ctx_dem_minmax(mhip_ctx *c, float *mn, float *mx, int32_t *has_nan)
{
    MH_ARG(c && mn && mx && has_nan && c->have[MHIP_R_DEM], "ctx_dem_minmax needs the DEM");
    MH_HIP(hipSetDevice(c->device));
    if (c->have[MHIP_R_FILLED] && c->fill_st.have_minmax) {
        *mn = c->fill_st.dem_min;
        *mx = c->fill_st.dem_max;
        *has_nan = c->fill_st.dem_nan ? 1 : 0;
        return MHIP_OK;
    }
    int hn = 0;
    MH_TRY(minmax_dev(c->r[MHIP_R_DEM].as<float>() + c->W * c->ht, c->H_owned * c->W, mn, mx, &hn, cs(c)));
    *has_nan = hn;
    return MHIP_OK;
}

int mhip_ctx_fill_begin(mhip_ctx *c, int kind, double short_, double diag, int32_t *active)
{
    MH_ARG(c && active && (kind == 0 || kind == 1) && c->have[MHIP_R_DEM], "ctx_fill_begin(ctx, kind, short, diag, active)");
    MH_HIP(hipSetDevice(c->device));
    const int which = kind ? MHIP_R_NOFLAT : MHIP_R_FILLED;
    MH_TRY(ctx_raster(c, which));
    ctx_wrote(c, which);
    if (kind == 0) {
        const bool force_iter = [] { const char *e = dev_env("MHIP_FILL"); return e && std::string(e) == "iterative"; }();
        delete c->pf;
        c->pf = nullptr;
        c->pf_done = false;
        c->pf_depths = false;
        c->pf_overflow = 0;
        if (!force_iter) {
            PfRun *p = new PfRun();
            p->dem = c->r[MHIP_R_DEM].as<float>();
            p->out = c->r[MHIP_R_FILLED].as<float>();
            p->H = c->H; p->W = c->W;
            p->fixed_top = c->ht; p->fixed_bot = c->hb;
            const int rc = p->begin(c->stream);
            if (rc == MHIP_OK) {
                c->pf = p;
                *active = 0;
                return MHIP_OK;
            }
            c->pf_overflow = p->overflow;
            delete p;
            if (rc != MHIP_ELIMIT) return rc;
        }
    }
    if (kind) {
        delete c->geo;
        c->geo = nullptr;
    }
    FillRun *f = new_fill_run(c, kind);
    if (kind) {
        MH_ARG(c->have[MHIP_R_FILLED], "the no-flats fill of a band starts from the converged plain fill");
        f->sh = short_; f->dg = diag;
        c->sh = short_; c->dg = diag;
        noflat_seed(*f, c->r[MHIP_R_FILLED].as<float>(), short_, diag, c->H_global * c->W);
    }
    bool a = false;
    MH_TRY(f->begin(c->stream, &a));
    *active = a;
    return MHIP_OK;
}

int mhip_ctx_fill_attach(mhip_ctx *c, int kind, double short_, double diag)
{
    MH_ARG(c && (kind == 0 || kind == 1) && c->have[MHIP_R_DEM], "ctx_fill_attach(ctx, kind, short, diag)");
    const int which = kind ? MHIP_R_NOFLAT : MHIP_R_FILLED;
    MH_ARG(c->r[which].p, "ctx_fill_attach: the raster to start from does not exist");
    MH_HIP(hipSetDevice(c->device));
    ctx_wrote(c, which);
    if (kind == 0) {
        delete c->pf;
        c->pf = nullptr;
    }
    FillRun *f = new_fill_run(c, kind);
    if (kind) {
        f->sh = short_; f->dg = diag;
        c->sh = short_; c->dg = diag;
    }
    return f->attach(c->stream);
}

int mhip_ctx_noflat_verify(mhip_ctx *c, int32_t *ok)
{
    MH_ARG(c && ok && c->have[MHIP_R_NOFLAT] && c->have[MHIP_R_DEM], "ctx_noflat_verify(ctx, ok) needs the no-flats surface");
    MH_HIP(hipSetDevice(c->device));
    bool good = false;
    MH_TRY(noflat_verify_dev(c->r[MHIP_R_DEM].as<float>(), c->r[MHIP_R_NOFLAT].as<double>(), c->H, c->W, c->sh, c->dg, c->stream, &good, c->ht, c->hb));
    *ok = good ? 1 : 0;
    return MHIP_OK;
}

static int ctx_attach_iterative_fill(mhip_ctx *c) { return new_fill_run(c, 0)->attach(c->stream); }

int mhip_ctx_fill_batch(mhip_ctx *c, int kind, int32_t *active)
{
    MH_ARG(c && active && (kind == 0 || kind == 1) && fill_begun(c, kind), "ctx_fill_batch needs ctx_fill_begin");
    MH_HIP(hipSetDevice(c->device));
    if (kind == 0 && !c->pf && !c->run[0]) {
        *active = 0;
        return MHIP_OK;
    }
    if (kind == 0 && c->pf) {
        const int rc = c->pf->batch(c->stream);
        *active = 0;
        if (rc != MHIP_ELIMIT) return rc;
        c->pf_overflow = c->pf->overflow;
        delete c->pf;
        c->pf = nullptr;
        bool a0 = false;
        MH_TRY(new_fill_run(c, 0)->begin(c->stream, &a0));
        *active = a0;
        return MHIP_OK;
    }
    bool a = false;
    MH_TRY(c->run[kind]->batch(c->stream, &a));
    *active = a;
    return MHIP_OK;
}

int mhip_ctx_fill_certify(mhip_ctx *c, int kind, int32_t *changed)
{
    MH_ARG(c && changed && (kind == 0 || kind == 1) && fill_begun(c, kind), "ctx_fill_certify needs ctx_fill_begin");
    MH_HIP(hipSetDevice(c->device));
    if (kind == 0 && c->pf) {
        bool violated = false;
        FillStats st;
        MH_TRY(ctx_raster(c, MHIP_R_DEPTHS));
        ctx_wrote(c, MHIP_R_DEPTHS);
        MH_TRY(c->pf->finish(c->stream, c->r[MHIP_R_DEPTHS].as<float>(), &st, &violated));
        delete c->pf;
        c->pf = nullptr;
        c->fill_st = st;
        c->fill_rounds = st.rounds;
        c->pf_done = true;
        c->pf_depths = true;
        *changed = 0;
        if (violated) {
            MH_TRY(ctx_attach_iterative_fill(c));
            *changed = 1;
        }
        return MHIP_OK;
    }
    if (kind == 0 && c->pf_done && !c->run[0]) {
        *changed = 0;
        return MHIP_OK;
    }
    bool ch = false;
    MH_TRY(c->run[kind]->certify(c->stream, &ch));
    *changed = ch ? 1 : 0;
    return MHIP_OK;
}

int mhip_ctx_fill_halo_changed(mhip_ctx *c, int kind, int side)
{
    MH_ARG(c && (kind == 0 || kind == 1) && fill_begun(c, kind) && (side == 0 || side == 1), "ctx_fill_halo_changed needs ctx_fill_begin");
    MH_HIP(hipSetDevice(c->device));
    if (kind == 0 && c->pf) return c->pf->halo_changed(side, c->stream);
    if (kind == 0 && !c->run[0]) MH_TRY(ctx_attach_iterative_fill(c));
    return c->run[kind]->activate_row(side, c->stream);
}

int mhip_ctx_fill_end(mhip_ctx *c, int kind)
{
    MH_ARG(c && (kind == 0 || kind == 1) && fill_begun(c, kind), "ctx_fill_end needs ctx_fill_begin");
    MH_HIP(hipSetDevice(c->device));
    FillStats st;
    bool depths_written = false;
    if (kind == 0 && c->pf) {
        MH_TRY(ctx_raster(c, MHIP_R_DEPTHS));
        MH_TRY(c->pf->finish(c->stream, c->r[MHIP_R_DEPTHS].as<float>(), &st));
        delete c->pf;
        c->pf = nullptr;
        depths_written = true;
    } else if (kind == 0 && !c->run[0]) {
        st = c->fill_st;
        depths_written = c->pf_depths;
    } else {
        MH_TRY(c->run[kind]->finish(c->stream, &st));
        delete c->run[kind];
        c->run[kind] = nullptr;
        if (kind == 0 && c->pf_done) {
            st.rounds += c->fill_st.rounds;
            st.visits += c->fill_st.visits;
            st.algorithm = 4;
        }
    }
    if (kind == 0) {
        c->pf_done = false;
        st.overflow = c->pf_overflow;
    }
    if (kind) { c->noflat_rounds = st.rounds; c->noflat_st = st; ctx_wrote(c, MHIP_R_NOFLAT); c->have[MHIP_R_NOFLAT] = true; }
    else {
        c->fill_rounds = st.rounds; c->fill_st = st; c->have[MHIP_R_FILLED] = true;
        ctx_wrote(c, MHIP_R_DEPTHS);
        c->pf_depths = false;
        MH_TRY(ctx_raster(c, MHIP_R_DEPTHS));
        const float *f = c->r[MHIP_R_FILLED].as<float>(), *d = c->r[MHIP_R_DEM].as<float>();
        float *o = c->r[MHIP_R_DEPTHS].as<float>();
        if (!depths_written) {
            MH_TRY(depths_dev(f, d, o, c->H * c->W, c->stream));
        } else {
            if (c->ht) MH_TRY(depths_dev(f, d, o, c->ht * c->W, c->stream));
            const int64_t below = (c->ht + c->H_owned) * c->W;
            if (c->hb) MH_TRY(depths_dev(f + below, d + below, o + below, c->hb * c->W, c->stream));
        }
        c->have[MHIP_R_DEPTHS] = true;
    }
    return MHIP_OK;
}

int mhip_ctx_geo_begin(mhip_ctx *c, double short_, double diag, int32_t *applicable, int32_t *active)
{
    MH_ARG(c && applicable && active && c->have[MHIP_R_DEM] && c->have[MHIP_R_FILLED], "ctx_geo_begin(ctx, short, diag, applicable, active) needs the plain fill");
    MH_HIP(hipSetDevice(c->device));
    MH_TRY(ctx_raster(c, MHIP_R_NOFLAT));
    MH_TRY(ctx_raster(c, MHIP_R_NGDIST));
    ctx_wrote(c, MHIP_R_NOFLAT);
    delete c->geo;
    GeoRun *g = c->geo = new GeoRun();
    g->dem = c->r[MHIP_R_DEM].as<float>();
    g->filled = c->r[MHIP_R_FILLED].as<float>();
    g->out = c->r[MHIP_R_NOFLAT].as<double>();
    g->dist = c->r[MHIP_R_NGDIST].as<uint32_t>();
    g->H = c->H; g->W = c->W; g->sh = short_; g->dg = diag;
    g->fixed_top = c->ht; g->fixed_bot = c->hb;
    g->allow_partial = true;
    g->seed_add = 1.01 * (double)(c->H_global * c->W) * diag;
    c->sh = short_; c->dg = diag;
    bool ap = false, ac = false;
    MH_TRY(g->begin(c->stream, &ap, &ac));
    *applicable = ap ? 1 : 0;
    *active = ac ? 1 : 0;
    if (!ap) {
        delete c->geo;
        c->geo = nullptr;
    }
    c->have[MHIP_R_NGDIST] = ap;
    return MHIP_OK;
}

int mhip_ctx_geo_batch(mhip_ctx *c, int32_t *active)
{
    MH_ARG(c && active && c->geo, "ctx_geo_batch needs ctx_geo_begin");
    MH_HIP(hipSetDevice(c->device));
    bool a = false;
    MH_TRY(c->geo->batch(c->stream, &a));
    *active = a ? 1 : 0;
    return MHIP_OK;
}

int mhip_ctx_geo_halo_changed(mhip_ctx *c, int side)
{
    MH_ARG(c && c->geo && (side == 0 || side == 1), "ctx_geo_halo_changed needs ctx_geo_begin");
    MH_HIP(hipSetDevice(c->device));
    return c->geo->halo_changed(side, c->stream);
}

int mhip_ctx_geo_end(mhip_ctx *c, int32_t *ok, int32_t *partial)
{
    MH_ARG(c && ok && partial && c->geo, "ctx_geo_end needs ctx_geo_begin");
    MH_HIP(hipSetDevice(c->device));
    FillStats st;
    bool good = false;
    MH_TRY(c->geo->end(c->stream, &good, &st));
    *partial = c->geo->partial ? 1 : 0;
    delete c->geo;
    c->geo = nullptr;
    *ok = good ? 1 : 0;
    if (good) {
        c->noflat_rounds = st.rounds;
        c->noflat_st = st;
        ctx_wrote(c, MHIP_R_NOFLAT);
        c->have[MHIP_R_NOFLAT] = true;
    }
    return MHIP_OK;
}

}
```

malstroem_amd/csrc/ctx_run.hip:

```cpp
#include <atomic>
#include <future>
#include <string>

#include "ctx.hpp"

using namespace mh;

constexpr int LABEL_START_DEFAULT = 3;
constexpr int FILL_HANDOVER_DEFAULT = 1;

static bool fill_handover_env()
{
    const char *e = dev_env("MHIP_FILL_HANDOVER");
    return e ? e[0] != '0' : FILL_HANDOVER_DEFAULT != 0;
}

static int stage_depths(mhip_ctx *c, hipStream_t s)
{
    MH_ARG(c->have[MHIP_R_FILLED] && c->have[MHIP_R_DEM], "depths need the filled surface");
    MH_TRY(ctx_raster(c, MHIP_R_DEPTHS));
    MH_TRY(depths_dev(c->r[MHIP_R_FILLED].as<float>(), c->r[MHIP_R_DEM].as<float>(), c->r[MHIP_R_DEPTHS].as<float>(), c->H * c->W, s));
    ctx_wrote(c, MHIP_R_DEPTHS);
    c->have[MHIP_R_DEPTHS] = true;
    return MHIP_OK;
}

static int stage_fill(mhip_ctx *c, hipStream_t s, bool with_depths = true, FillHandover *ho = nullptr)
{
    const int64_t H = c->H, W = c->W;
    MH_ARG(c->have[MHIP_R_DEM], "FILL needs the DEM");
    MH_TRY(ctx_raster(c, MHIP_R_FILLED));
    MH_TRY(ctx_raster(c, MHIP_R_DEPTHS));
    MH_TRY(stage_begin(c, MHIP_STAGE_FILL, s));
    FillStats st;
    bool depths_done = false;
    MH_TRY(fill_plain_dev(c->r[MHIP_R_DEM].as<float>(), c->r[MHIP_R_FILLED].as<float>(), H, W, s, &st, c->r[MHIP_R_DEPTHS].as<float>(),
                          &depths_done, ho));
    ctx_wrote(c, MHIP_R_FILLED);
    ctx_wrote(c, MHIP_R_DEPTHS);
    const bool owed = ho && ho->pending;
    c->have[MHIP_R_FILLED] = !owed;
    c->have[MHIP_R_DEPTHS] = depths_done && !owed;
    if (with_depths && !depths_done) MH_TRY(stage_depths(c, s));
    MH_TRY(stage_end(c, MHIP_STAGE_FILL, s));
    c->fill_rounds = st.rounds;
    c->fill_st = st;
    return MHIP_OK;
}

static void ctx_handover_settled(mhip_ctx *c, FillHandover *ho)
{
    if (!ho || ho->pending || c->have[MHIP_R_FILLED]) return;
    c->have[MHIP_R_FILLED] = true;
    c->have[MHIP_R_DEPTHS] = true;
    c->fill_handover = ho->queued ? 1 : 0;
    if (ho->suspect) ++c->fill_handover_rechecks;
    if (ho->repaired) {
        c->fill_st.algorithm = 4;
        c->fill_st.rounds += ho->st_repair.rounds;
        c->fill_st.visits += ho->st_repair.visits;
        c->fill_st.cycles += ho->st_repair.cycles;
        c->fill_rounds = c->fill_st.rounds;
    }
}

static int stage_noflat(mhip_ctx *c, hipStream_t s, bool shdg_done = false, StageHook *tail_hook = nullptr, bool with_flowdir = false,
                        bool *flowdir_done = nullptr, FillHandover *ho = nullptr)
{
    const int64_t H = c->H, W = c->W, n = H * W;
    MH_ARG(c->have[MHIP_R_DEM], "NOFLAT needs the DEM");
    MH_TRY(ctx_raster(c, MHIP_R_NOFLAT));
    MH_TRY(stage_begin(c, MHIP_STAGE_NOFLAT, s));
    if (!shdg_done) {
        if ((c->have[MHIP_R_FILLED] || (ho && ho->pending)) && c->fill_st.have_minmax) short_diag_from_minmax(c->fill_st.dem_min, c->fill_st.dem_max, c->fill_st.dem_nan, &c->sh, &c->dg);
        else MH_TRY(short_diag_dev(c->r[MHIP_R_DEM].as<float>(), n, &c->sh, &c->dg, s));
    }
    FillStats st;
    if (!c->have[MHIP_R_FILLED] && !(ho && ho->pending)) {
        MH_TRY(ctx_raster(c, MHIP_R_FILLED));
        FillStats st0;
        MH_TRY(fill_plain_dev(c->r[MHIP_R_DEM].as<float>(), c->r[MHIP_R_FILLED].as<float>(), H, W, s, &st0));
        ctx_wrote(c, MHIP_R_FILLED);
        c->have[MHIP_R_FILLED] = true;
    }
    D8Sink d8;
    static const bool fuse_d8 = [] { const char *e = dev_env("MHIP_D8_FUSE"); return !(e && e[0] == '0'); }();
    if (with_flowdir && fuse_d8 && !c->ht && !c->hb) {
        MH_TRY(ctx_raster(c, MHIP_R_FLOWDIR));
        MH_TRY(c->nodir_cnt.alloc(4));
        MH_HIP(hipMemsetAsync(c->nodir_cnt.p, 0, 4, s));
        d8.flowdir = c->r[MHIP_R_FLOWDIR].as<uint8_t>();
        d8.nodir = c->nodir_cnt.as<unsigned int>();
    }
    const int rc_nf = fill_noflat_dev(c->r[MHIP_R_DEM].as<float>(), c->r[MHIP_R_NOFLAT].as<double>(), H, W, c->sh, c->dg, s, &st,
                                      c->r[MHIP_R_FILLED].as<float>(), tail_hook, d8.flowdir ? &d8 : nullptr, ho);
    ctx_handover_settled(c, ho);
    MH_TRY(rc_nf);
    if (flowdir_done) *flowdir_done = d8.done;
    MH_TRY(stage_end(c, MHIP_STAGE_NOFLAT, s));
    c->noflat_rounds = st.rounds;
    c->noflat_st = st;
    ctx_wrote(c, MHIP_R_NOFLAT);
    c->have[MHIP_R_NOFLAT] = true;
    return MHIP_OK;
}

static int stage_flowdir(mhip_ctx *c, hipStream_t s)
{
    MH_ARG(c->have[MHIP_R_NOFLAT], "FLOWDIR needs the no-flats surface");
    MH_TRY(ctx_raster(c, MHIP_R_FLOWDIR));
    MH_TRY(stage_begin(c, MHIP_STAGE_FLOWDIR, s));
    ctx_wrote(c, MHIP_R_FLOWDIR);
    MH_TRY(c->nodir_cnt.alloc(4));
    MH_HIP(hipMemsetAsync(c->nodir_cnt.p, 0, 4, s));
    MH_TRY(d8_dev(c->r[MHIP_R_NOFLAT].as<double>(), c->r[MHIP_R_FLOWDIR].as<uint8_t>(), c->H, c->W, 1, s, c->row0 - c->ht,
                  c->H_global, c->nodir_cnt.as<unsigned int>()));
    MH_TRY(stage_end(c, MHIP_STAGE_FLOWDIR, s));
    c->have[MHIP_R_FLOWDIR] = true;
    c->flowdir_own = true;
    c->nodir_valid = !c->ht && !c->hb;
    return MHIP_OK;
}

static int stage_flowdir_fused(mhip_ctx *c, hipStream_t s)
{
    MH_TRY(stage_begin(c, MHIP_STAGE_FLOWDIR, s));
    MH_TRY(stage_end(c, MHIP_STAGE_FLOWDIR, s));
    ctx_wrote(c, MHIP_R_FLOWDIR);
    c->have[MHIP_R_FLOWDIR] = true;
    c->nodir_valid = true;
    c->flowdir_own = true;
    return MHIP_OK;
}

static int stage_accum(mhip_ctx *c, hipStream_t s, PourLink *pour = nullptr)
{
    MH_ARG(c->have[MHIP_R_FLOWDIR], "ACCUM needs flow directions");
    MH_TRY(ctx_raster(c, MHIP_R_ACCUM));
    MH_TRY(stage_begin(c, MHIP_STAGE_ACCUM, s));
    bool delta_done = false;
    if ((c->ht || c->hb) && c->acc_keep.valid)
        MH_TRY(accum_band_delta_dev(c->r[MHIP_R_FLOWDIR].as<uint8_t>(), c->r[MHIP_R_ACCUM].as<double>(), c->H, c->W, s, c->ht, c->hb, &c->acc_keep, &delta_done));
    c->accum_algorithm = delta_done ? 1 : 0;
    ctx_wrote(c, MHIP_R_ACCUM);
    if (!delta_done)
        MH_TRY(accum_dev(c->r[MHIP_R_FLOWDIR].as<uint8_t>(), c->r[MHIP_R_ACCUM].as<double>(), c->H, c->W, s, c->ht, c->hb, 0, nullptr, pour));
    MH_TRY(stage_end(c, MHIP_STAGE_ACCUM, s));
    c->have[MHIP_R_ACCUM] = true;
    return MHIP_OK;
}

static int stage_label(mhip_ctx *c, hipStream_t s)
{
    const int64_t H = c->H, W = c->W, n = H * W;
    MH_ARG(c->have[MHIP_R_DEPTHS] || c->have[MHIP_R_FILLED], "LABEL needs bluespot depths");
    MH_TRY(ctx_raster(c, MHIP_R_LABELS));
    if (!c->tmp_i32.p) MH_TRY(c->tmp_i32.alloc(4 * (size_t)n));
    MH_TRY(stage_begin(c, MHIP_STAGE_LABEL, s));
    if (!c->have[MHIP_R_DEPTHS]) MH_TRY(stage_depths(c, s));
    ctx_wrote(c, MHIP_R_LABELS);
    MH_TRY(ccl8_f32_dev(c->r[MHIP_R_DEPTHS].as<float>(), c->r[MHIP_R_LABELS].as<int32_t>(), c->tmp_i32.as<int32_t>(), H, W,
                        &c->nlabels_raw, s, &c->raw_stats));
    MH_TRY(stage_end(c, MHIP_STAGE_LABEL, s));
    c->have[MHIP_R_LABELS] = true;
    c->labels_components = true;
    c->labels_filtered = false;
    c->nlabels = c->nlabels_raw;
    return MHIP_OK;
}

static int pour_link_buffers(mhip_ctx *c, PourLink *pl, hipStream_t s)
{
    const int64_t H = c->H, W = c->W;
    const int64_t ntiles = cdiv(H, 64) * cdiv(W, 64);
    MH_TRY(c->pp_mask0.alloc(2 * 256 * (size_t)ntiles));
    MH_TRY(c->pp_list.alloc(8 * (size_t)POUR_TILE_CAP * (size_t)ntiles));
    MH_TRY(c->pp_tiles.alloc(12 * (size_t)ntiles));
    MH_TRY(c->pp_misc.alloc(16));
    MH_TRY(c->pp_key.alloc(8 * (size_t)(c->nlabels + 1)));
    MH_HIP(hipMemsetAsync(c->pp_misc.p, 0, 16, s));
    MH_HIP(hipMemsetAsync(c->pp_key.p, 0, 8 * (size_t)(c->nlabels + 1), s));
    pl->dev.mask0 = c->pp_mask0.as<uint16_t>();
    pl->dev.list = c->pp_list.as<uint2>();
    pl->dev.tile_key0 = c->pp_tiles.as<unsigned long long>();
    pl->dev.tile_cnt = reinterpret_cast<uint32_t *>(c->pp_tiles.as<unsigned long long>() + ntiles);
    pl->dev.flags = c->pp_misc.as<uint32_t>() + 1;
    pl->dev.components = c->labels_components ? 1 : 0;
    pl->dev.key = c->pp_key.as<unsigned long long>();
    pl->dev.nlab = (uint32_t)c->nlabels;
    pl->ev = c->ev_cand;
    return MHIP_OK;
}

static int stage_watershed(mhip_ctx *c, hipStream_t s, PourLink *pour = nullptr)
{
    const int64_t H = c->H, W = c->W, n = H * W;
    MH_ARG(c->have[MHIP_R_LABELS] && c->have[MHIP_R_FLOWDIR], "WATERSHED needs labels and flow directions");
    MH_TRY(ctx_ensure_labels_final(c, s));
    MH_TRY(ctx_label_max(c, s));
    MH_TRY(ctx_raster(c, MHIP_R_WATERSHEDS));
    MH_TRY(stage_begin(c, MHIP_STAGE_WATERSHED, s));
    ctx_wrote(c, MHIP_R_WATERSHEDS);
    if (pour) MH_TRY(pour_link_buffers(c, pour, s));
    MH_TRY(watersheds_dev(c->r[MHIP_R_FLOWDIR].as<uint8_t>(), c->r[MHIP_R_WATERSHEDS].as<int32_t>(), H, W, 0, s, false,
                          c->nodir_valid ? c->nodir_cnt.as<unsigned int>() : nullptr, c->r[MHIP_R_LABELS].as<int32_t>(), pour));
    MH_TRY(c->ws_counts.alloc(8 * (size_t)(c->nlabels + 1)));
    MH_TRY(label_count_dev(c->r[MHIP_R_WATERSHEDS].as<int32_t>(), n, c->nlabels, c->ws_counts.as<int64_t>(), s, W));
    MH_TRY(stage_end(c, MHIP_STAGE_WATERSHED, s));
    c->have[MHIP_R_WATERSHEDS] = true;
    c->ws_counts_valid = true;
    return MHIP_OK;
}

static int stage_pourpoints(mhip_ctx *c, hipStream_t s, PourLink *pour = nullptr)
{
    const int64_t H = c->H, W = c->W;
    MH_ARG(c->have[MHIP_R_LABELS] && (c->have[MHIP_R_ACCUM] || c->have[MHIP_R_NOFLAT]),
           "POURPOINTS needs labels and accumulated flow or the no-flats surface");
    MH_TRY(ctx_ensure_labels_final(c, s));
    MH_TRY(ctx_label_max(c, s));
    MH_TRY(c->pour.alloc(sizeof(mhip_index_record) * (size_t)(c->nlabels + 1)));
    MH_TRY(stage_begin(c, MHIP_STAGE_POURPOINTS, s));
    bool from_keys = false;
    if (pour && pour->consumed && c->have[MHIP_R_ACCUM]) {
        uint32_t h[3] = {0, 1, 1};
        MH_HIP(hipMemcpyAsync(h, c->pp_misc.p, 12, hipMemcpyDeviceToHost, s));
        MH_TRY(pour_finish_dev(c->pp_key.as<unsigned long long>(), c->pp_tiles.as<unsigned long long>(), cdiv(H, 64) * cdiv(W, 64), c->nlabels, W,
                               c->pour.as<mhip_index_record>(), s));
        MH_HIP(stream_sync(s));
        from_keys = !h[1] && !h[2];
    }
    c->pour_algorithm = from_keys ? 1 : 0;
    if (from_keys) {
    } else if (c->have[MHIP_R_ACCUM])
        MH_TRY(label_arg_dev(c->r[MHIP_R_ACCUM].as<double>(), c->r[MHIP_R_LABELS].as<int32_t>(), H, W, c->nlabels, true,
                             c->pour.as<mhip_index_record>(), s, c->labels_components));
    else
        MH_TRY(label_arg_dev(c->r[MHIP_R_NOFLAT].as<double>(), c->r[MHIP_R_LABELS].as<int32_t>(), H, W, c->nlabels, false,
                             c->pour.as<mhip_index_record>(), s));
    MH_TRY(stage_end(c, MHIP_STAGE_POURPOINTS, s));
    c->pour_valid = true;
    return MHIP_OK;
}

static int label_start_env()
{
    const char *e = dev_env("MHIP_LABEL_START");
    const int v = e ? atoi(e) : LABEL_START_DEFAULT;
    return v >= 0 && v <= 3 ? v : LABEL_START_DEFAULT;
}

extern "C" int mhip_ctx_run(mhip_ctx *c, int mask)
{
    MH_ARG(c, "ctx");
    MH_HIP(hipSetDevice(c->device));
    hipStream_t s = c->stream;
    if (c->nranks > 1 || c->ht || c->hb) {
        MH_ARG((mask & ~(MHIP_STAGE_FLOWDIR | MHIP_STAGE_ACCUM)) == 0,
               "this stage runs through the band entry points on a row band (mhip_ctx_fill_*, mhip_ctx_band_*)");
    }
    const bool serial_env = [] { const char *e = dev_env("MHIP_SERIAL"); return e && e[0] == '1'; }();
    const int side_a = mask & (MHIP_STAGE_NOFLAT | MHIP_STAGE_FLOWDIR | MHIP_STAGE_ACCUM);
    const int side_b = mask & (MHIP_STAGE_LABEL | MHIP_STAGE_WATERSHED);
    const bool overlap = side_a && side_b && !serial_env;
    FillHandover handover;
    FillHandover *const ho =
        ((mask & MHIP_STAGE_FILL) && (mask & MHIP_STAGE_NOFLAT) && c->nranks == 1 && !c->ht && !c->hb && fill_handover_env()) ? &handover : nullptr;
    c->fill_handover = 0;

    if (!overlap) {
        if (mask & MHIP_STAGE_FILL) MH_TRY(stage_fill(c, s, true, ho));
        bool fd_done = false;
        if (mask & MHIP_STAGE_NOFLAT) MH_TRY(stage_noflat(c, s, false, nullptr, (mask & MHIP_STAGE_FLOWDIR) != 0, &fd_done, ho));
        if (mask & MHIP_STAGE_FLOWDIR) MH_TRY(fd_done ? stage_flowdir_fused(c, s) : stage_flowdir(c, s));
        if (mask & MHIP_STAGE_ACCUM) MH_TRY(stage_accum(c, s));
        if (mask & MHIP_STAGE_LABEL) MH_TRY(stage_label(c, s));
        if (mask & MHIP_STAGE_WATERSHED) MH_TRY(stage_watershed(c, s));
        if (mask & MHIP_STAGE_POURPOINTS) MH_TRY(stage_pourpoints(c, s));
        return MHIP_OK;
    }

    StageTimer *t;
    for (int st : {MHIP_STAGE_FILL, MHIP_STAGE_NOFLAT, MHIP_STAGE_FLOWDIR, MHIP_STAGE_ACCUM, MHIP_STAGE_LABEL, MHIP_STAGE_WATERSHED,
                   MHIP_STAGE_POURPOINTS})
        if (mask & st) MH_TRY(ctx_timer(c, st, &t));
    auto side_stream = [&](hipStream_t *st) -> int {
        int least = 0, greatest = 0;
        MH_HIP(hipDeviceGetStreamPriorityRange(&least, &greatest));
        MH_HIP(hipStreamCreateWithPriority(st, hipStreamNonBlocking, least));
        return MHIP_OK;
    };
    if (!c->stream_b) MH_TRY(side_stream(&c->stream_b));
    if (!c->stream_c) MH_TRY(side_stream(&c->stream_c));
    MH_TRY(ctx_fork_join_events(c));
    if (!c->ev_cand) MH_HIP(hipEventCreateWithFlags(&c->ev_cand, hipEventDisableTiming));
    hipStream_t sb = c->stream_b;
    const bool do_fill = (mask & MHIP_STAGE_FILL) != 0;
    MH_ARG(c->have[MHIP_R_DEM] || !(mask & (MHIP_STAGE_FILL | MHIP_STAGE_NOFLAT)), "FILL / NOFLAT need the DEM");

    std::promise<int> fill_done, shdg_done, flowdir_ready, label_ready, tail_reached;
    std::future<int> fill_fut = fill_done.get_future(), shdg_fut = shdg_done.get_future(), tail_fut = tail_reached.get_future();
    struct TailCtx {
        mhip_ctx *c;
        std::promise<int> *p;
        FillHandover *ho;
    } tail_ctx{c, &tail_reached, ho};
    StageHook tail_hook;
    tail_hook.arg = &tail_ctx;
    tail_hook.fn = [](void *arg, hipStream_t st) {
        TailCtx *t = static_cast<TailCtx *>(arg);
        ctx_handover_settled(t->c, t->ho);
        t->p->set_value(hipEventRecord(t->c->ev_tail, st) == hipSuccess ? MHIP_OK : MHIP_EHIP);
    };
    std::future<int> flowdir_fut = flowdir_ready.get_future(), label_fut = label_ready.get_future();
    struct CandHand {
        std::promise<int> p;
        std::future<int> f;
        std::atomic<bool> set{false};
    } cand_hand;
    cand_hand.f = cand_hand.p.get_future();
    PourLink pour_link;
    pour_link.arg = &cand_hand;
    pour_link.notify = [](void *a, int v) {
        CandHand *h = static_cast<CandHand *>(a);
        if (!h->set.exchange(true)) h->p.set_value(v);
    };
    pour_link.wait = [](void *a) { return static_cast<CandHand *>(a)->f.get(); };
    static const bool pour_pass = [] { const char *e = dev_env("MHIP_POUR"); return e && std::string(e) == "pass"; }();
    PourLink *const pour = ((mask & MHIP_STAGE_ACCUM) && (mask & MHIP_STAGE_WATERSHED) && (mask & MHIP_STAGE_POURPOINTS) && !pour_pass) ? &pour_link : nullptr;
    const bool ws_needs_new_flowdir = (mask & MHIP_STAGE_WATERSHED) && (mask & MHIP_STAGE_FLOWDIR);
    int rc_b = MHIP_OK;
    char err_b[512] = "";
    bool shdg_set = false, label_set = false;
    c->side.run([&] {
        rc_b = [&]() -> int {
            MH_HIP(hipSetDevice(c->device));
            int rc_e = MHIP_OK;
            if ((mask & MHIP_STAGE_NOFLAT) && !do_fill) rc_e = short_diag_dev(c->r[MHIP_R_DEM].as<float>(), c->H * c->W, &c->sh, &c->dg, sb);
            if (rc_e != MHIP_OK) snprintf(err_b, sizeof(err_b), "%s", get_error());
            shdg_done.set_value(rc_e);
            shdg_set = true;
            int rc_l = rc_e == MHIP_OK ? fill_fut.get() : rc_e;
            if (rc_l == MHIP_OK) rc_l = tail_fut.get();
            if (rc_l == MHIP_OK && hipStreamWaitEvent(sb, c->ev_tail, 0) != hipSuccess) rc_l = MHIP_EHIP;
            if (rc_l == MHIP_OK && (mask & MHIP_STAGE_LABEL)) rc_l = stage_label(c, sb);
            else if (rc_l == MHIP_OK && do_fill && !c->have[MHIP_R_DEPTHS]) rc_l = stage_depths(c, sb);
            if (rc_l == MHIP_OK && (mask & (MHIP_STAGE_WATERSHED | MHIP_STAGE_POURPOINTS)) && c->have[MHIP_R_LABELS]) {
                rc_l = ctx_ensure_labels_final(c, sb);
                if (rc_l == MHIP_OK) rc_l = ctx_label_max(c, sb);
            }
            if (rc_l == MHIP_OK && hipEventRecord(c->ev_label, sb) != hipSuccess) rc_l = MHIP_EHIP;
            if (rc_l != MHIP_OK && !err_b[0]) snprintf(err_b, sizeof(err_b), "%s", get_error());
            label_ready.set_value(rc_l);
            label_set = true;
            MH_TRY(rc_l);
            hipStream_t sw = sb;
            if (mask & MHIP_STAGE_WATERSHED) {
                sw = c->stream_c;
                MH_HIP(hipStreamWaitEvent(sw, c->ev_label, 0));
                if (ws_needs_new_flowdir) {
                    MH_TRY(flowdir_fut.get());
                    MH_HIP(hipStreamWaitEvent(sw, c->ev_flowdir, 0));
                }
                MH_TRY(stage_watershed(c, sw, pour));
            }
            MH_HIP(hipEventRecord(c->ev_join, sw));
            return MHIP_OK;
        }();
        if (rc_b != MHIP_OK && !err_b[0]) snprintf(err_b, sizeof(err_b), "%s", get_error());
        if (!shdg_set) shdg_done.set_value(rc_b);
        if (!label_set) label_ready.set_value(rc_b);
        pour_link.notify(pour_link.arg, 0);
    });
    int rc_a = MHIP_OK;
    if (do_fill) rc_a = stage_fill(c, s, false, ho);
    if (rc_a == MHIP_OK && hipEventRecord(c->ev_fork, s) != hipSuccess) rc_a = MHIP_EHIP;
    fill_done.set_value(rc_a);
    const int rc_e = shdg_fut.get();
    if (rc_a == MHIP_OK) rc_a = [&]() -> int {
        MH_TRY(rc_e);
        if (do_fill && (mask & MHIP_STAGE_NOFLAT)) {
            if (c->fill_st.have_minmax) short_diag_from_minmax(c->fill_st.dem_min, c->fill_st.dem_max, c->fill_st.dem_nan, &c->sh, &c->dg);
            else MH_TRY(short_diag_dev(c->r[MHIP_R_DEM].as<float>(), c->H * c->W, &c->sh, &c->dg, s));
        }
        const int label_start = label_start_env();
        const bool owed = ho && ho->pending;
        if (label_start == 0 && !owed) tail_hook.fire(s);
        tail_hook.at = label_start;
        const bool armed = label_start == StageHook::TAIL_ROUNDS || label_start == StageHook::FINISH || (label_start == StageHook::FIRST_VISIT && owed);
        bool fd_done = false;
        if (mask & MHIP_STAGE_NOFLAT)
            MH_TRY(stage_noflat(c, s, true, armed ? &tail_hook : nullptr, (mask & MHIP_STAGE_FLOWDIR) != 0, &fd_done, ho));
        if (mask & MHIP_STAGE_FLOWDIR) {
            MH_TRY(fd_done ? stage_flowdir_fused(c, s) : stage_flowdir(c, s));
            MH_HIP(hipEventRecord(c->ev_flowdir, s));
        }
        return MHIP_OK;
    }();
    tail_hook.fire(s);
    flowdir_ready.set_value(rc_a);
    if (rc_a == MHIP_OK && (mask & MHIP_STAGE_ACCUM)) rc_a = stage_accum(c, s, pour);
    const int rc_l = label_fut.get();
    if (rc_a == MHIP_OK && rc_l == MHIP_OK && (mask & MHIP_STAGE_POURPOINTS)) {
        rc_a = hipStreamWaitEvent(s, c->ev_label, 0) == hipSuccess ? stage_pourpoints(c, s, pour) : MHIP_EHIP;
    }
    c->side.wait();
    if (rc_a != MHIP_OK) return rc_a;
    if (rc_b != MHIP_OK) {
        set_error("%s", err_b);
        return rc_b;
    }
    MH_HIP(hipStreamWaitEvent(s, c->ev_join, 0));
    return MHIP_OK;
}
```

malstroem_amd/csrc/noflat_geo.hip:

```cpp
#include <algorithm>
#include <cmath>
#include <cstdlib>
#include <mutex>
#include <string>
#include <type_traits>
#include <vector>

#include "common.hpp"
#include "handover_addr.hpp"

namespace mh {

namespace {

constexpr int WN = 64;
constexpr int TI = 62;
constexpr uint32_t DINF = 0xE0000000u;
constexpr uint32_t WMAX = 1u << 28;
constexpr uint32_t D_IRR = 0xFFFFFFFFu;
constexpr uint32_t M_NOFLAT = 0xFF00u;
constexpr uint32_t M_IRR = 0xFD00u;
constexpr uint32_t M_WALL = 0xFE00u;
constexpr int DPP_WF_SL1 = 0x130;
constexpr int DPP_WF_SR1 = 0x138;
// ... 940 lines not shown
                if (lane == 0) base = atomicAdd(a.count_next, (uint32_t)__builtin_popcountll(bal));
                base = (uint32_t)__builtin_amdgcn_readfirstlane((int)base);
                if (fresh) a.list_next[base + (uint32_t)__builtin_popcountll(bal & ((1ull << lane) - 1ull))] = tp;
            }
        } else if (mine) {
            a.mark[tp] = 1;
        }
    }
#ifdef NG_PROFILE
    if (!FIRST) {
        asm volatile("s_waitcnt vmcnt(0)" ::: "memory");
        const long long tp4 = __builtin_amdgcn_s_memtime();
        if (lane == 0) {
            const int o = C_STATS + 128 + ((hdr & HDR_OPEN) ? 8 : 0);
            atomicAdd(&a.counters[o + 0], 1ull);
            atomicAdd(&a.counters[o + 1], (unsigned long long)(tp1 - tp0));
            atomicAdd(&a.counters[o + 2], (unsigned long long)(tp2 - tp1));
            atomicAdd(&a.counters[o + 3], (unsigned long long)(tp3 - tp2));
            atomicAdd(&a.counters[o + 4], (unsigned long long)(tp4 - tp3));
        }
    }
#endif
}

template <bool FIRST, int WPB = 4, bool HANDOVER = false>
__device__ __forceinline__ void round_body(const GeoArgs &a)
{
    extern __shared__ __attribute__((aligned(16))) uint32_t lds[];
    const int lane = threadIdx.x & 63;
    const int wave = __builtin_amdgcn_readfirstlane(threadIdx.x >> 6);
    const uint32_t scr_b = (uint32_t)(uintptr_t)(__attribute__((address_space(3))) uint32_t *)(lds + wave * (WN * (WN + 1)));
    uint32_t *tab_l = lds + WPB * (WN * (WN + 1));
    const int nwaves = (int)gridDim.x * WPB, gw = (int)blockIdx.x * WPB + wave;
    uint32_t tw[512 / (64 * WPB)];
#pragma unroll
    for (int k = 0; k < 512 / (64 * WPB); ++k) tw[k] = a.tab[threadIdx.x + k * 64 * WPB];
    const int n = FIRST ? a.nt : (int)__builtin_amdgcn_readfirstlane((int)*a.count);
    const int t_first = FIRST ? 0 : a.list[gw < a.nt ? gw : a.nt - 1];
#pragma unroll
    for (int k = 0; k < 512 / (64 * WPB); ++k) tab_l[threadIdx.x + k * 64 * WPB] = tw[k];
    __syncthreads();
    unsigned visits = 0, cycles = 0;
    for (int i = gw; i < n; i += nwaves) {
        const int t = FIRST ? i : __builtin_amdgcn_readfirstlane(i == gw ? t_first : a.list[i]);
        visit<FIRST, HANDOVER>(a, t, tab_l, scr_b, lane, visits, cycles);
    }
    if (lane == 0 && visits) {
        unsigned long long *st = a.counters + C_STATS + 2 * (gw & 63);
        atomicAdd(&st[0], (unsigned long long)visits);
        atomicAdd(&st[1], (unsigned long long)cycles);
    }
}
__global__ __launch_bounds__(256, 2) void ng_first_kernel(GeoArgs a) { round_body<true>(a); }
__global__ __launch_bounds__(256, 2) void ng_round_kernel(GeoArgs a) { round_body<false>(a); }
__global__ __launch_bounds__(64, 2) void ng_round_w1_kernel(GeoArgs a) { round_body<false, 1>(a); }
__global__ __launch_bounds__(256, 2) void ng_handover_kernel(GeoArgs a) { round_body<true, 4, true>(a); }

__global__ __launch_bounds__(256) void ng_compact_kernel(unsigned long long *mark8, int nwords, int *list, uint32_t *count)
{
    __shared__ uint32_t n_l, base_l;
    if (threadIdx.x == 0) n_l = 0;
    __syncthreads();
    const int w = (int)blockIdx.x * 256 + (int)threadIdx.x;
    const unsigned long long v = w < nwords ? mark8[w] : 0ull;
    unsigned k = 0;
    uint32_t o = 0;
    if (v) {
        mark8[w] = 0;
#pragma unroll
        for (int j = 0; j < 8; ++j) k += ((v >> (8 * j)) & 0xffull) ? 1u : 0u;
        o = atomicAdd(&n_l, k);
    }
    __syncthreads();
    if (threadIdx.x == 0) base_l = n_l ? atomicAdd(count, n_l) : 0u;
    __syncthreads();
    if (v) {
        o += base_l;
#pragma unroll
        for (int j = 0; j < 8; ++j)
            if ((v >> (8 * j)) & 0xffull) list[o++] = 8 * w + j;
    }
}

__global__ __launch_bounds__(256) void ng_assemble_kernel(const float *__restrict__ F, const uint32_t *__restrict__ d, double *__restrict__ G, int64_t n,
                                                          double seed_add, unsigned long long *counters)
{
    const int64_t i0 = ((int64_t)blockIdx.x * 256 + threadIdx.x) * 4;
    if (i0 >= n) return;
    unsigned bad = 0;
    auto value = [&](float f, uint32_t dd) {
        if (dd == D_IRR) return (double)f + seed_add;
        if (dd >= 0x80000000u) {
            ++bad;
            return (double)f + seed_add;
        }
        const uint32_t e = class_above(f);
        return dd ? (double)f + (double)dd * class_ulp(e) : (double)f;
    };
    if (i0 + 4 <= n) {
        const float4 f = *reinterpret_cast<const float4 *>(F + i0);
        const uint4 dv = *reinterpret_cast<const uint4 *>(d + i0);
        typedef double __attribute__((ext_vector_type(2))) v2d;
        *reinterpret_cast<v2d *>(G + i0) = v2d{value(f.x, dv.x), value(f.y, dv.y)};
        *reinterpret_cast<v2d *>(G + i0 + 2) = v2d{value(f.z, dv.z), value(f.w, dv.w)};
    } else {
        for (int64_t i = i0; i < n; ++i) G[i] = value(F[i], d[i]);
    }
    if (bad) atomicAdd(&counters[C_UNREACHED], (unsigned long long)bad);
}

constexpr int VRB = 16;
__global__ __launch_bounds__(256) void ng_verify_kernel(const float *__restrict__ dem, const double *__restrict__ G, int64_t H, int64_t W, double sh,
                                                        double dg, int fixed_top, int fixed_bot, unsigned long long *counters)
{
    const int64_t c = (int64_t)blockIdx.x * 256 + threadIdx.x;
    const int64_t rb = (int64_t)blockIdx.y * VRB;
    if (c >= W) return;
    const double PINF = __builtin_inf();
    const bool cl = c > 0, cr = c + 1 < W;
    auto row = [&](int64_t r, double (&v)[3]) {
        const bool in = r >= 0 && r < H;
        const double *p = G + (in ? r : 0) * W + c;
        v[0] = (in && cl) ? p[-1] : PINF;
        v[1] = in ? p[0] : PINF;
        v[2] = (in && cr) ? p[1] : PINF;
    };
    double a[3], b[3], n[3];
    row(rb - 1, a);
    row(rb, b);
    unsigned bad = 0;
#pragma unroll 4
    for (int i = 0; i < VRB; ++i) {
        const int64_t r = rb + i;
        if (r >= H) break;
        row(r + 1, n);
        const double own = b[1], dv = (double)dem[r * W + c];
        double want = dv;
        if (r > 0 && r < H - 1 && cl && cr) {
            const double md = fmin(fmin(a[0], a[2]), fmin(n[0], n[2])) + dg;
            const double me = fmin(fmin(a[1], b[0]), fmin(b[2], n[1])) + sh;
            want = fmax(fmin(md, me), dv);
        }
        const bool halo = (r == 0 && fixed_top) || (r == H - 1 && fixed_bot);
        bad += (own == want || halo) ? 0u : 1u;
#pragma unroll
        for (int k = 0; k < 3; ++k) {
            a[k] = b[k];
            b[k] = n[k];
        }
    }
    if (bad) atomicAdd(&counters[C_MISMATCH], (unsigned long long)bad);
}

constexpr int FRB = 32;
__device__ __forceinline__ double dleft(double v)
{
    const uint64_t b = (uint64_t)__double_as_longlong(v);
    const uint32_t lo = from_left((uint32_t)b), hi = from_left((uint32_t)(b >> 32));
    return __longlong_as_double((long long)(((uint64_t)hi << 32) | lo));
}
__device__ __forceinline__ double dright(double v)
{
    const uint64_t b = (uint64_t)__double_as_longlong(v);
    const uint32_t lo = from_right((uint32_t)b), hi = from_right((uint32_t)(b >> 32));
    return __longlong_as_double((long long)(((uint64_t)hi << 32) | lo));
}
template <bool D8>
__global__ __launch_bounds__(256) void ng_finish_kernel(const float *__restrict__ F, const uint32_t *__restrict__ d, const float *__restrict__ dem,
                                                        double *__restrict__ G, int64_t H, int64_t W, double sh, double dg, double seed_add, int fixed_top,
                                                        int fixed_bot, unsigned long long *counters, uint8_t *__restrict__ flowdir, unsigned int *nodir)
{
    const int lane = threadIdx.x & 63, wave = threadIdx.x >> 6;
    const int64_t c = ((int64_t)blockIdx.x * 4 + wave) * TI + lane - 1;
    const int64_t rb = (int64_t)blockIdx.y * FRB;
    const bool col_in = c >= 0 && c < W;
    const int64_t cc = c < 0 ? 0 : (c < W ? c : W - 1);
    const bool mine = lane >= 1 && lane <= TI && col_in;
    const bool inner_col = c > 0 && c + 1 < W;
    const double PINF = __builtin_inf();
    unsigned unreached = 0, bad = 0, anynodir = 0;
    auto value = [&](int64_t r) -> double {
        if (!(r >= 0 && r < H && col_in)) return PINF;
        const float f = F[r * W + cc];
        const uint32_t dd = d[r * W + cc];
        if (dd == D_IRR) return (double)f + seed_add;
        if (dd >= 0x80000000u) {
            unreached += mine && r >= rb && r < rb + FRB ? 1u : 0u;
            return (double)f + seed_add;
        }
        return dd ? (double)f + (double)dd * class_ulp(class_above(f)) : (double)f;
    };
    double a = value(rb - 1), b = value(rb);
    for (int i = 0; i < FRB; ++i) {
        const int64_t r = rb + i;
        if (r >= H) break;
        const double n = value(r + 1);
        const double al = dleft(a), ar = dright(a), bl = dleft(b), br = dright(b), nl = dleft(n), nr = dright(n);
        if (mine) {
            const double dv = (double)dem[r * W + c];
            double want = dv;
            if (r > 0 && r < H - 1 && inner_col) {
                const double md = fmin(fmin(al, ar), fmin(nl, nr)) + dg;
                const double me = fmin(fmin(a, bl), fmin(br, n)) + sh;
                want = fmax(fmin(md, me), dv);
            }
            const bool halo = (r == 0 && fixed_top) || (r == H - 1 && fixed_bot);
            bad += (b == want || halo) ? 0u : 1u;
            G[r * W + c] = b;
            if (D8) {
                unsigned code;
                if (r == 0 || r == H - 1 || c == 0 || c == W - 1) code = edge_code(r, c, H - 1, W - 1);
                else {
                    code = d8_code(b, a, ar, br, nr, n, nl, bl, al);
                    anynodir |= code == 8u ? 1u : 0u;
                }
                flowdir[r * W + c] = (uint8_t)code;
            }
        }
        a = b;
        b = n;
    }
    if (unreached) atomicAdd(&counters[C_UNREACHED], (unsigned long long)unreached);
    if (bad) atomicAdd(&counters[C_MISMATCH], (unsigned long long)bad);
    if (D8 && __any(anynodir != 0u) && lane == 0) *nodir = 1u;
}

#ifndef NG_FINISH_AHEAD
#define NG_FINISH_AHEAD 1
#endif
#ifndef NG_FINISH_WAVES
#define NG_FINISH_WAVES 8
#endif
#if NG_FINISH_WAVES < 8
#define NG_FINISH_RESIDENCY __attribute__((amdgpu_waves_per_eu(1, NG_FINISH_WAVES)))
#else
#define NG_FINISH_RESIDENCY
#endif
#if NG_FINISH_AHEAD
template <>
__global__ __launch_bounds__(256) NG_FINISH_RESIDENCY void ng_finish_kernel<true>(const float *__restrict__ F, const uint32_t *__restrict__ d,
                                                                                  const float *__restrict__ dem, double *__restrict__ G, int64_t H, int64_t W,
                                                                                  double sh, double dg, double seed_add, int fixed_top, int fixed_bot,
                                                                                  unsigned long long *counters, uint8_t *__restrict__ flowdir,
                                                                                  unsigned int *nodir)
{
    const int lane = threadIdx.x & 63, wave = threadIdx.x >> 6;
    const int64_t c = ((int64_t)blockIdx.x * 4 + wave) * TI + lane - 1;
    const int64_t rb = (int64_t)blockIdx.y * FRB;
    const bool col_in = c >= 0 && c < W;
    const int64_t cc = c < 0 ? 0 : (c < W ? c : W - 1);
    const bool mine = lane >= 1 && lane <= TI && col_in;
    const bool inner_col = c > 0 && c + 1 < W;
    const double PINF = __builtin_inf();
    unsigned unreached = 0, bad = 0, anynodir = 0;
    struct Row {
        float f, z;
        uint32_t dd;
    };
    auto load = [&](int64_t r) -> Row {
        const int64_t at = (r < 0 ? 0 : (r < H ? r : H - 1)) * W + cc;
        return Row{F[at], dem[at], d[at]};
    };
    auto value = [&](int64_t r, const Row &x) -> double {
        if (!(r >= 0 && r < H && col_in)) return PINF;
        if (x.dd == D_IRR) return (double)x.f + seed_add;
        if (x.dd >= 0x80000000u) {
            unreached += mine && r >= rb && r < rb + FRB ? 1u : 0u;
            return (double)x.f + seed_add;
        }
        return x.dd ? (double)x.f + (double)x.dd * class_ulp(class_above(x.f)) : (double)x.f;
    };
    const Row xa = load(rb - 1), xb = load(rb);
    Row x0 = load(rb + 1), x1{0.0f, 0.0f, 0u};
    double a = value(rb - 1, xa), b = value(rb, xb);
    double dvb = (double)xb.z;
    auto row = [&](int i, const Row &xn, Row &xnn, auto more) {
        const int64_t r = rb + i;
        const double dv = dvb;
        if (decltype(more)::value) xnn = load(r + 2);
        const double n = value(r + 1, xn);
        dvb = (double)xn.z;
        asm volatile("" : "+v"(dvb));
        const double al = dleft(a), ar = dright(a), bl = dleft(b), br = dright(b), nl = dleft(n), nr = dright(n);
        if (mine && r < H) {
            double want = dv;
            if (r > 0 && r < H - 1 && inner_col) {
                const double md = fmin(fmin(al, ar), fmin(nl, nr)) + dg;
                const double me = fmin(fmin(a, bl), fmin(br, n)) + sh;
                want = fmax(fmin(md, me), dv);
            }
            const bool halo = (r == 0 && fixed_top) || (r == H - 1 && fixed_bot);
            bad += (b == want || halo) ? 0u : 1u;
            G[r * W + c] = b;
            unsigned code;
            if (r == 0 || r == H - 1 || c == 0 || c == W - 1) code = edge_code(r, c, H - 1, W - 1);
            else {
                code = d8_code(b, a, ar, br, nr, n, nl, bl, al);
                anynodir |= code == 8u ? 1u : 0u;
            }
            flowdir[r * W + c] = (uint8_t)code;
        }
        a = b;
        b = n;
    };
    static_assert(FRB % 2 == 0, "rows in pairs");
    int i = 0;
    for (; i < FRB - 2 && rb + i < H; i += 2) {
        row(i, x0, x1, std::true_type());
        row(i + 1, x1, x0, std::true_type());
    }
    if (i == FRB - 2 && rb + i < H) {
        row(i, x0, x1, std::true_type());
        row(i + 1, x1, x0, std::false_type());
    }
    if (unreached) atomicAdd(&counters[C_UNREACHED], (unsigned long long)unreached);
    if (bad) atomicAdd(&counters[C_MISMATCH], (unsigned long long)bad);
    if (__any(anynodir != 0u) && lane == 0) *nodir = 1u;
}
#endif

uint32_t class_weight(double eps, int e)
{
    if (!(eps > 0.0) || std::isinf(eps)) return 0;
    int q;
    const double fr = std::frexp(eps, &q);
    const uint64_t M = (uint64_t)std::ldexp(fr, 53);
    const int k = (e - 127 - 52) - (q - 53);
    if (k <= 24 || k > 52) return 0;
    const uint64_t half = 1ull << (k - 1), rem = M & ((1ull << k) - 1);
    if (rem == half) return 0;
    const uint64_t w = (M >> k) + (rem > half ? 1 : 0);
    return (w >= 1 && w < WMAX) ? (uint32_t)w : 0;
}

}

struct GeoRun::Impl {
    DevBuf ws;
    uint32_t *d_tab = nullptr, *d_any = nullptr, *d_hdr = nullptr, *d_blk = nullptr;
    unsigned long long *d_cnt = nullptr;
    uint8_t *d_mark = nullptr;
    int *d_list = nullptr, *d_list2 = nullptr, *d_amark = nullptr;
    int ntr = 0, ntc = 0, round = 0, used = 0;
    std::vector<std::pair<hipEvent_t, hipEvent_t>> span;
    int span_rounds = 0;
    uint32_t last_count = 0xffffffffu;
    bool light = false;
    int light_from = 0;
    int64_t nt = 0;
    size_t lds = 0;
    int maxcyc = NG_MAXCYC;
    bool debug = false;
    unsigned long long irregular = 0;
};
namespace {
constexpr int MAXR = 8192, BATCH = 32, BATCH_HEAD = 16;
constexpr uint32_t LIGHT_TILES = 6144;
__global__ void ng_mark_row_kernel(uint8_t *mark, int ti, int ntc)
{
    const int tj = blockIdx.x * blockDim.x + threadIdx.x;
    if (tj < ntc) mark[(int64_t)ti * ntc + tj] = 1;
}
}

GeoRun::GeoRun() : impl(new Impl) {}
GeoRun::~GeoRun()
{
    for (auto &e : impl->span) {
        (void)hipEventDestroy(e.first);
        (void)hipEventDestroy(e.second);
    }
    delete impl;
}

int GeoRun::launch_rounds(hipStream_t s, int nb)
{
    {
        Impl &mm = *impl;
        hipEvent_t e0, e1;
        MH_HIP(hipEventCreate(&e0));
        MH_HIP(hipEventCreate(&e1));
        mm.span.emplace_back(e0, e1);
        MH_HIP(hipEventRecord(e0, s));
    }
    struct CloseSpan {
        Impl &m;
        hipStream_t s;
        ~CloseSpan() { (void)hipEventRecord(m.span.back().second, s); }
    } close_span{*impl, s};
    Impl &m = *impl;
    GeoArgs a;
    a.H = H; a.W = W; a.ntr = m.ntr; a.ntc = m.ntc; a.nt = (int)m.nt; a.F = filled; a.d = dist; a.tab = m.d_tab; a.counters = m.d_cnt;
    a.blk = m.d_blk; a.hdr = m.d_hdr; a.mark = m.d_mark; a.list = m.d_list; a.fixed_top = fixed_top; a.fixed_bot = fixed_bot;
    a.append = 0; a.round_next = 0; a.amark = m.d_amark; a.list_next = nullptr; a.count_next = nullptr;
    a.ho_dem = nullptr; a.ho_bslot = nullptr; a.ho_tabV = nullptr; a.ho_F = nullptr; a.ho_depths = nullptr;
    const unsigned grid = (unsigned)std::min<int64_t>((m.nt + 3) / 4, 512);
    for (int k = 0; k < nb; ++k, ++m.round) {
        a.maxcyc = m.maxcyc;
        a.count = m.d_any + m.round;
        if (!m.round && handover && handover->pending) {
            a.ho_dem = handover->dem; a.ho_bslot = handover->bslot; a.ho_tabV = handover->tabV;
// ... 90 lines not shown
        }
    }
    m.round = 0;
    m.last_count = 0xffffffffu;
    m.used = 0;
    if (handover && handover->pending &&
        !(handover->ntr == m.ntr && handover->ntc == m.ntc && handover->H == H && handover->W == W && handover->filled == filled && handover->dem == dem &&
          !fixed_top && !fixed_bot))
        MH_TRY(fill_handover_complete(handover, s));
    const bool took = handover && handover->pending;
    MH_TRY(launch_rounds(s, 1));
    unsigned long long h_c[5] = {0, 0, 0, 0, 0};
    MH_HIP(hipMemcpyAsync(h_c, m.d_cnt, sizeof(h_c), hipMemcpyDeviceToHost, s));
    MH_HIP(stream_sync(s));
    if (took) {
        if (h_c[C_PROOF] != 0 || dev_env("MHIP_HO_RECHECK") != nullptr) {
            handover->suspect = true;
            m.ws.release();
            return MHIP_OK;
        }
        handover->release();
    }
    m.used = 1;
    m.irregular = h_c[C_IRREGULAR];
    if (h_c[C_FATAL] || (m.irregular && !allow_partial)) {
        if (m.debug) fprintf(stderr, "[noflat geodesic] %llu irregular flat cells, %llu NaN cells: float64 relaxation\n", m.irregular, h_c[C_FATAL]);
        return MHIP_OK;
    }
    *applicable = true;
    *active = true;
    return MHIP_OK;
}

int GeoRun::batch(hipStream_t s, bool *active)
{
    Impl &m = *impl;
    const char *eb = dev_env("MHIP_NG_BATCH");
    const int nb_env = eb && atoi(eb) >= 1 && atoi(eb) <= BATCH ? atoi(eb) : 0;
    for (;;) {
        const int nb = nb_env ? nb_env : (!m.light ? BATCH_HEAD : (m.last_count <= 64 ? 8 : (m.last_count <= 512 ? 16 : BATCH)));
        if (m.round + BATCH > MAXR) {
            set_error("no-flats fill (geodesic) did not converge within %d rounds", MAXR);
            return MHIP_ENOTCONV;
        }
        MH_TRY(launch_rounds(s, nb));
        if (tail_hook) tail_hook->fire_at(StageHook::TAIL_ROUNDS, s);
        uint32_t h_any[BATCH];
        MH_HIP(hipMemcpyAsync(h_any, m.d_any + (m.round - nb), sizeof(uint32_t) * nb, hipMemcpyDeviceToHost, s));
        MH_HIP(stream_sync(s));
        for (int k = 0; k < nb; ++k) {
            if (!h_any[k]) {
                *active = false;
                m.light = false;
                return MHIP_OK;
            }
            ++m.used;
        }
        m.last_count = h_any[nb - 1];
        if (!m.light && h_any[nb - 1] <= LIGHT_TILES) {
            m.light = true;
            m.light_from = m.round;
        }
    }
}

int GeoRun::halo_changed(int side, hipStream_t s)
{
    Impl &m = *impl;
    hipLaunchKernelGGL(ng_mark_row_kernel, dim3((unsigned)((m.ntc + 255) / 256)), dim3(256), 0, s, m.d_mark, side == 0 ? 0 : m.ntr - 1, m.ntc);
    MH_HIP(hipGetLastError());
    return MHIP_OK;
}

int GeoRun::end(hipStream_t s, bool *ok, FillStats *st)
{
    Impl &m = *impl;
    const int64_t n = H * W;
    partial = m.irregular != 0 && allow_partial;
    if (dev_env("MHIP_NG_CORRUPT") && W > 8)
        MH_HIP(hipMemsetAsync(dist + (H / 2) * W + 1, 0x01, 4 * (size_t)(W - 2), s));
    d8_done = false;
    const bool with_d8 = !partial && d8_out && d8_nodir && !fixed_top && !fixed_bot;
    if (tail_hook) tail_hook->fire_at(StageHook::FINISH, s);
    if (with_d8)
        hipLaunchKernelGGL(ng_finish_kernel<true>, dim3((unsigned)((W + 4 * TI - 1) / (4 * TI)), (unsigned)((H + FRB - 1) / FRB)), dim3(256), 0, s, filled, dist, dem,
                           out, H, W, sh, dg, seed_add, fixed_top, fixed_bot, m.d_cnt, d8_out, d8_nodir);
    else if (!partial)
        hipLaunchKernelGGL(ng_finish_kernel<false>, dim3((unsigned)((W + 4 * TI - 1) / (4 * TI)), (unsigned)((H + FRB - 1) / FRB)), dim3(256), 0, s, filled, dist, dem,
                           out, H, W, sh, dg, seed_add, fixed_top, fixed_bot, m.d_cnt, (uint8_t *)nullptr, (unsigned int *)nullptr);
    else
        hipLaunchKernelGGL(ng_assemble_kernel, dim3((unsigned)((n + 1023) / 1024)), dim3(256), 0, s, filled, dist, out, n, seed_add, m.d_cnt);
    MH_HIP(hipGetLastError());
    unsigned long long h_all[C_STATS + 128 + 16];
    MH_HIP(hipMemcpyAsync(h_all, m.d_cnt, sizeof(h_all), hipMemcpyDeviceToHost, s));
    MH_HIP(stream_sync(s));
    if (allow_partial && h_all[C_UNREACHED]) partial = true;
    if (st) {
        *st = FillStats();
        st->geo_irregular = (int64_t)m.irregular;
        st->geo_unreached = (int64_t)h_all[C_UNREACHED];
        st->geo_mismatch = (int64_t)h_all[C_MISMATCH];
        st->rounds = m.used;
        st->tiles = m.nt;
        st->algorithm = partial ? 3 : 2;
        for (auto &e : m.span) {
            float ms = 0;
            if (hipEventElapsedTime(&ms, e.first, e.second) == hipSuccess) st->hot_ms += ms;
            else (void)hipGetLastError();
        }
        st->hot_launches = m.used > 0 ? m.used - 1 : 0;
        for (int k = 0; k < 64; ++k) {
            st->visits += (int64_t)h_all[C_STATS + 2 * k];
            st->cycles += (int64_t)h_all[C_STATS + 2 * k + 1];
        }
    }
    if (m.debug) {
        std::vector<uint32_t> cnt((size_t)m.round);
        MH_HIP(hipMemcpy(cnt.data(), m.d_any, 4 * (size_t)m.round, hipMemcpyDeviceToHost));
        unsigned long long v = 0, cy = 0;
        for (int k = 0; k < 64; ++k) {
            v += h_all[C_STATS + 2 * k];
            cy += h_all[C_STATS + 2 * k + 1];
        }
        fprintf(stderr, "[noflat geodesic] tiles %lld, visits %llu, cycles %llu; tiles per round:", (long long)m.nt, v, cy);
        for (int k = 1; k < m.round && k < 200; ++k) fprintf(stderr, " %u", cnt[k]);
#ifdef NG_PROFILE
        for (int o = 0; o < 2; ++o) {
            const unsigned long long *q = h_all + C_STATS + 128 + 8 * o;
            if (q[0]) fprintf(stderr, "\n[noflat visits, %s] %llu: ticks per visit: setup+issue %.0f, wait for loads %.0f, relax %.0f, store %.0f", o ? "open" : "masked", q[0],
                              (double)q[1] / q[0], (double)q[2] / q[0], (double)q[3] / q[0], (double)q[4] / q[0]);
        }
#endif
        fprintf(stderr, "\n[noflat geodesic] %lld x %lld: rounds %d, unreached %llu, mismatches %llu\n", (long long)H, (long long)W, m.used, h_all[C_UNREACHED],
                h_all[C_MISMATCH]);
    }
    *ok = partial ? true : !(h_all[C_UNREACHED] || h_all[C_MISMATCH]);
    d8_done = with_d8 && !partial && *ok;
    m.ws.release();
    return MHIP_OK;
}

int noflat_verify_dev(const float *d_dem, const double *d_out, int64_t H, int64_t W, double sh, double dg, hipStream_t s, bool *ok, int fixed_top,
                      int fixed_bot)
{
    DevBuf cnt;
    MH_TRY(cnt.alloc(8 * (C_STATS + 128 + 16)));
    MH_HIP(hipMemsetAsync(cnt.p, 0, 8 * (C_STATS + 128), s));
    hipLaunchKernelGGL(ng_verify_kernel, dim3((unsigned)((W + 255) / 256), (unsigned)((H + VRB - 1) / VRB)), dim3(256), 0, s, d_dem, d_out, H, W, sh, dg, fixed_top,
                       fixed_bot, cnt.as<unsigned long long>());
    MH_HIP(hipGetLastError());
    unsigned long long bad = 0;
    MH_HIP(hipMemcpyAsync(&bad, cnt.as<unsigned long long>() + C_MISMATCH, 8, hipMemcpyDeviceToHost, s));
    MH_HIP(stream_sync(s));
    *ok = bad == 0;
    return MHIP_OK;
}

int fill_noflat_geodesic_dev(const float *d_dem, const float *d_filled, double *d_out, int64_t H, int64_t W, double sh, double dg, double seed_add,
                             hipStream_t s, FillStats *st, bool *partial, StageHook *tail_hook, D8Sink *d8, FillHandover *ho)
{
    GeoRun g;
    g.handover = ho;
    g.tail_hook = tail_hook;
    if (d8) { g.d8_out = d8->flowdir; g.d8_nodir = d8->nodir; d8->done = false; }
    g.dem = d_dem; g.filled = d_filled; g.out = d_out; g.H = H; g.W = W; g.sh = sh; g.dg = dg;
    g.allow_partial = partial != nullptr && seed_add == seed_add && seed_add < 1e300;
    g.seed_add = seed_add;
    bool applicable = false, active = false, ok = false;
    MH_TRY(g.begin(s, &applicable, &active));
    if (ho && ho->pending) {
        const bool again = ho->suspect;
        MH_TRY(fill_handover_complete(ho, s));
        if (again) {
            g.handover = nullptr;
            MH_TRY(g.begin(s, &applicable, &active));
        }
    }
    if (tail_hook) tail_hook->fire_at(StageHook::FIRST_VISIT, s);
    if (!applicable) {
        if (st) st->geo_reject = 1;
        return MHIP_ELIMIT;
    }
    while (active) MH_TRY(g.batch(s, &active));
    MH_TRY(g.end(s, &ok, st));
    if (partial) *partial = g.partial;
    if (d8) d8->done = g.d8_done;
    if (!ok && st) st->geo_reject = 2;
    return ok ? MHIP_OK : MHIP_ELIMIT;
}

}
```

malstroem_amd/csrc/pflood.hip:

```cpp
#include "common.hpp"
#include <algorithm>
#include <vector>

namespace mh {

namespace {

constexpr int WN = 64, TI = 62, NC = WN * WN;
constexpr int NBMAX = 1024;
constexpr int HE = 2048;
constexpr int HEU = 2032;
constexpr int SE = 512;
constexpr int SPMAX = 192;
constexpr int LMAX = 256;
constexpr int NSMAX = 128;
constexpr int LH = 1024;
constexpr uint32_t KINV = 0xFFFFFFFFu;
constexpr uint32_t EMPTY = 0xFFFFFFFFu;
constexpr int OCEAN = 255, NOLAB = 254;
constexpr unsigned PF_OV_NB = 1u, PF_OV_PAIRS = 2u, PF_OV_NS = 4u, PF_OV_SPILL = 8u, PF_OV_LINKS = 16u, PF_OV_EMAX = 32u, PF_OV_HALO = 64u;
constexpr uint8_t C_VALID = 1, C_BORDER = 2, C_RING = 4;

struct PfArgs {
    int64_t H, W;
// ... 925 lines not shown
    unsigned int pad3[58];
    unsigned int slots[1];
};
static_assert(offsetof(PfQueue, slots) == 1024, "header = four lines of 256 bytes");
constexpr unsigned int PFQ_SPIN_LIMIT = 1u << 21;
constexpr int PFQ_BLK_BITS = 20;

__device__ __forceinline__ unsigned int ld_sc1(const unsigned int *p) { return __hip_atomic_load(p, __ATOMIC_RELAXED, __HIP_MEMORY_SCOPE_AGENT); }
__device__ __forceinline__ void st_sc1(unsigned int *p, unsigned int v) { __hip_atomic_store(p, v, __ATOMIC_RELAXED, __HIP_MEMORY_SCOPE_AGENT); }

__global__ void pf_queue_init_kernel(PfQueue *q, unsigned int *mark, int nbr, int nbc, int mode, int row_a, int row_b, unsigned int cap_mask)
{
    const int i = (int)(blockIdx.x * blockDim.x + threadIdx.x);
    int n, blk;
    if (mode == 0) {
        const int h = nbr, w = nbc;
        n = (h == 1 || w == 1) ? h * w : 2 * (w - 1) + 2 * (h - 1);
        if (i >= n) return;
        int bi, bj;
        if (h == 1 || w == 1) { bi = w == 1 ? i : 0; bj = w == 1 ? 0 : i; }
        else if (i < w - 1) { bi = 0; bj = i; }
        else if (i < (w - 1) + (h - 1)) { bi = i - (w - 1); bj = w - 1; }
        else if (i < 2 * (w - 1) + (h - 1)) { bi = h - 1; bj = w - 1 - (i - (w - 1) - (h - 1)); }
        else { bi = h - 1 - (i - 2 * (w - 1) - (h - 1)); bj = 0; }
        blk = bi * nbc + bj;
    } else {
        const int two = row_b != row_a ? 2 : 1;
        n = two * nbc;
        if (i >= n) return;
        blk = (i < nbc ? row_a : row_b) * nbc + (i < nbc ? i : i - nbc);
    }
    mark[blk] = 1u;
    q->slots[i] = (1u << PFQ_BLK_BITS) | (unsigned int)blk;
    if (i == 0) {
        q->head = 0u;
        q->tail = (unsigned int)n;
        q->finished = 0u;
        q->abort = 0u;
        q->cap_mask = cap_mask;
    }
}

__device__ __forceinline__ void pf_solve_queue_body(const SolveArgs &sa, PfQueue *q, const int *__restrict__ ecount)
{
    __shared__ uint32_t L[RT * RT * NSMAX + 4];
    constexpr int LSENT = RT * RT * NSMAX;
    __shared__ uint32_t Lold[BT * BT * NSMAX];
    __shared__ int s_wake, s_blk, s_or[3];
    const PfArgs &a = sa.a;
    const int t = threadIdx.x;
    int or_turn = 0;
    auto wg_or = [&](bool p) -> bool {
        if (__any(p) && (t & 63) == 0) s_or[or_turn] = 1;
        __syncthreads();
        const bool r = s_or[or_turn] != 0;
        if (t == 0) s_or[or_turn == 0 ? 2 : or_turn - 1] = 0;
        or_turn = or_turn == 2 ? 0 : or_turn + 1;
        return r;
    };
    if (t == 0) { s_or[0] = 0; s_or[1] = 0; s_or[2] = 0; L[LSENT] = 0u; }
    const unsigned int cap_mask = q->cap_mask, cap_shift = (unsigned int)__builtin_popcount(cap_mask);
    for (;;) {
        __syncthreads();
        if (t == 0) {
            int blk = -1;
            const unsigned int ticket = atomicAdd(&q->head, 1u);
            const unsigned int gen = (ticket >> cap_shift) + 1u;
            if (gen >= (1u << (32 - PFQ_BLK_BITS)) - 1u) atomicExch(&q->abort, 1u);
            else {
                const unsigned int *slot = &q->slots[ticket & cap_mask];
                for (unsigned int n = 0;; ++n) {
                    const unsigned int v = ld_sc1(slot);
                    if ((v >> PFQ_BLK_BITS) == gen) { blk = (int)(v & ((1u << PFQ_BLK_BITS) - 1u)); break; }
                    if ((n & 7u) == 7u) {
                        const unsigned int fin = ld_sc1(&q->finished);
                        asm volatile("s_waitcnt vmcnt(0)" ::: "memory");
                        if (fin == ld_sc1(&q->tail) || ld_sc1(&q->abort)) break;
                    }
                    if (n > PFQ_SPIN_LIMIT) { atomicExch(&q->abort, 1u); break; }
                    if (n < 64u) __builtin_amdgcn_s_sleep(8);
                    else __builtin_amdgcn_s_sleep(48);
                }
            }
            if (blk >= 0) (void)atomicExch(&sa.mark_cur[blk], 2u);
            s_blk = blk;
            s_wake = 0;
        }
        __syncthreads();
        const int blk = s_blk;
        if (blk < 0) return;
        const int bi = blk / sa.nbc, bj = blk - bi * sa.nbc;
        int tv = t;
        asm volatile("" : "+v"(tv));
        {
            constexpr int NLV = RT * RT * NSMAX / ST;
            uint32_t lv[NLV];
#pragma unroll
            for (int u = 0; u < NLV; ++u) {
                const int i = tv + u * ST;
                const int rt = i / NSMAX, k = i - rt * NSMAX;
                const int p = bi * BT + rt / RT - 1, qq = bj * BT + rt % RT - 1;
                const bool ok = p >= 0 && p < a.ntr && qq >= 0 && qq < a.ntc;
                lv[u] = EMPTY;
                if (ok) lv[u] = ld_sc1(&a.Lv[(size_t)(p * a.ntc + qq) * NSMAX + k]);
            }
#pragma unroll
            for (int u = 0; u < NLV; ++u) {
                const int i = tv + u * ST;
                const int rt = i / NSMAX, k = i - rt * NSMAX, ri = rt / RT, rj = rt - ri * RT;
                L[i] = lv[u];
                if (ri >= 1 && ri <= BT && rj >= 1 && rj <= BT) Lold[((ri - 1) * BT + rj - 1) * NSMAX + k] = lv[u];
            }
        }
        const int ne = ecount[blk];
        unsigned long long er[EMAX / ST];
#pragma unroll
        for (int k = 0; k < EMAX / ST; ++k) {
            er[k] = ~0ull;
            if (t + k * ST < ne) er[k] = sa.eblk[(size_t)blk * EMAX + t + k * ST];
        }
#pragma unroll
        for (int k = 0; k < EMAX / ST; ++k) {
            const unsigned long long r = er[k];
            const unsigned src = (unsigned)(r >> 32) & 0xffffu;
            const unsigned long long dst = r == ~0ull ? (unsigned long long)LSENT : r >> 48;
            er[k] = (dst << 48) | ((unsigned long long)(src == 0xFFFFu ? (unsigned)LSENT : src) << 32) | (r & 0xffffffffull);
        }
        __syncthreads();
        int dbg_sweeps = 0;
        for (int it = 0; it < BT * BT * NSMAX; ++it) {
            bool ch = false;
            ++dbg_sweeps;
#pragma unroll
            for (int k = 0; k < EMAX / ST; ++k) {
                const unsigned long long r = er[k];
                const int dst = (int)(r >> 48), src = (int)((r >> 32) & 0xffffu);
                const uint32_t v = max((uint32_t)r, L[src]);
                if (v < L[dst]) {
                    atomicMin(&L[dst], v);
                    ch = true;
                }
            }
            if (!wg_or(ch)) break;
        }
        bool moved = false;
        for (int i = tv; i < BT * BT * NSMAX; i += ST) {
            const int bt = i / NSMAX, k = i - bt * NSMAX;
            const int p = bi * BT + bt / BT, qq = bj * BT + bt % BT;
            const uint32_t v = L[((bt / BT + 1) * RT + bt % BT + 1) * NSMAX + k];
            if (v < Lold[i] && p < a.ntr && qq < a.ntc) {
                atomicMin(&a.Lv[(size_t)(p * a.ntc + qq) * NSMAX + k], v);
                moved = true;
            }
        }
        asm volatile("s_waitcnt vmcnt(0)" ::: "memory");
        const bool dbg_moved = wg_or(moved);
        if (dbg_moved) {
            unsigned wake = 0;
#pragma unroll
            for (int k = 0; k < EMAX / ST; ++k) {
                const unsigned long long r = er[k];
                const int dst = (int)(r >> 48), src = (int)((r >> 32) & 0xffffu);
                if (src == LSENT) continue;
                const int st = src / NSMAX, si = st / RT, sj = st % RT;
                if (si >= 1 && si <= BT && sj >= 1 && sj <= BT) continue;
                const int dt = dst / NSMAX, di_ = dt / RT - 1, dj_ = dt % RT - 1;
                if (L[dst] < Lold[(di_ * BT + dj_) * NSMAX + dst % NSMAX]) {
// ... 797 lines not shown
```

Before: 12680 Mcells/s.

## Defer no-flats f64 surface store and pre-allocate accumulation node buffers

The geodesic no-flats finish kernel gains a template flag that skips writing the f64 no-flats raster when D8 is fused. The surface is instead assembled lazily from the filled raster and distance field the first time it is read, through a settle hook added to every context accessor. Accumulation node buffers can also be allocated and zeroed ahead of time on another stream and handed over through an event. The aim is to remove a large f64 write and the allocation/memset from the timed critical path, at the cost of extra bookkeeping and a risk of stale reads if an accessor misses the settle hook. A wait on the vector memory counter is also added after a pflood queue atomic.

```diff
diff --git a/malstroem_amd/csrc/accum.hip b/malstroem_amd/csrc/accum.hip
--- a/malstroem_amd/csrc/accum.hip
+++ b/malstroem_amd/csrc/accum.hip
@@ -720,8 +720,44 @@
     return MHIP_OK;
 }
 
+namespace {
+struct NodeLayout {
+    size_t o_gstate, o_inflow, o_arrived, o_next, o_dst, o_exit, o_flags, o_halo, o_bexit, bytes;
+    NodeLayout(int64_t nnodes, int64_t W, bool exit_map)
+    {
+        auto align = [](size_t x) { return (x + 255) & ~size_t(255); };
+        o_gstate = 0; o_inflow = align(o_gstate + 8 * (size_t)nnodes); o_arrived = align(o_inflow + 8 * (size_t)nnodes);
+        o_next = align(o_arrived + 4 * (size_t)nnodes); o_dst = align(o_next + 4 * (size_t)nnodes);
+        o_exit = align(o_dst + 4 * (size_t)nnodes); o_flags = align(o_exit + 2 * (size_t)nnodes);
+        o_halo = align(o_flags + (size_t)nnodes);
+        o_bexit = align(o_halo + (exit_map ? 8 * (size_t)W : 0));
+        bytes = o_bexit + (exit_map ? 4 * (size_t)nnodes : 0);
+    }
+};
+inline int64_t accum_nodes(int64_t H, int64_t W) { return cdiv(H, AT) * cdiv(W, AT) * NODE_STRIDE; }
+}
+
+AccumPrep::~AccumPrep()
+{
+    if (valid && ready) (void)hipEventSynchronize(ready);
+}
+
+int accum_prepare_dev(AccumPrep *prep, int64_t H, int64_t W, hipStream_t s, hipEvent_t ready)
+{
+    prep->valid = false;
+    const int64_t nnodes = accum_nodes(H, W);
+    if (nnodes >= (int64_t)INT32_MAX || H * W >= (1ll << 37)) return MHIP_OK;
+    const NodeLayout L(nnodes, W, false);
+    MH_TRY(prep->nodes.alloc(L.bytes));
+    MH_HIP(hipMemsetAsync(prep->nodes.as<char>() + L.o_inflow, 0, L.o_next - L.o_inflow, s));
+    MH_HIP(hipEventRecord(ready, s));
+    prep->ready = ready; prep->H = H; prep->W = W;
+    prep->valid = true;
+    return MHIP_OK;
+}
+
 int accum_dev(const uint8_t *d_fd, double *d_out, int64_t H, int64_t W, hipStream_t s, int fixed_top, int fixed_bot, int halo_zero,
-              int32_t *d_exit_map, PourLink *pour, AccumKeep *keep)
+              int32_t *d_exit_map, PourLink *pour, AccumKeep *keep, AccumPrep *prep)
 {
     const int ntr = (int)cdiv(H, AT), ntc = (int)cdiv(W, AT);
     const int64_t ntiles = (int64_t)ntr * ntc, nnodes = ntiles * NODE_STRIDE;
@@ -730,13 +766,17 @@
         return MHIP_ELIMIT;
     }
     DevBuf buf;
-    auto align = [](size_t x) { return (x + 255) & ~size_t(255); };
-    const size_t o_gstate = 0, o_inflow = align(o_gstate + 8 * (size_t)nnodes), o_arrived = align(o_inflow + 8 * (size_t)nnodes);
-    const size_t o_next = align(o_arrived + 4 * (size_t)nnodes), o_dst = align(o_next + 4 * (size_t)nnodes);
-    const size_t o_exit = align(o_dst + 4 * (size_t)nnodes), o_flags = align(o_exit + 2 * (size_t)nnodes);
-    const size_t o_halo = align(o_flags + (size_t)nnodes);
-    const size_t o_bexit = align(o_halo + (d_exit_map ? 8 * (size_t)W : 0));
-    MH_TRY(buf.alloc(o_bexit + (d_exit_map ? 4 * (size_t)nnodes : 0)));
+    const NodeLayout L(nnodes, W, d_exit_map != nullptr);
+    const size_t o_gstate = L.o_gstate, o_inflow = L.o_inflow, o_arrived = L.o_arrived, o_next = L.o_next, o_dst = L.o_dst, o_exit = L.o_exit,
+                 o_flags = L.o_flags, o_halo = L.o_halo, o_bexit = L.o_bexit;
+    const bool prepared = prep && prep->valid && prep->H == H && prep->W == W && !d_exit_map && !keep;
+    if (prepared) {
+        buf.p = prep->nodes.p; buf.bytes = prep->nodes.bytes;
+        prep->nodes.p = nullptr; prep->nodes.bytes = 0;
+        prep->valid = false;
+        MH_HIP(hipStreamWaitEvent(s, prep->ready, 0));
+    } else
+        MH_TRY(buf.alloc(L.bytes));
     char *b = buf.as<char>();
     Nodes nd;
     nd.gstate = reinterpret_cast<uint64_t *>(b + o_gstate);
@@ -749,7 +789,7 @@
     nd.halo_first = d_exit_map ? reinterpret_cast<int32_t *>(b + o_halo) : nullptr;
     nd.bexit = d_exit_map ? reinterpret_cast<int32_t *>(b + o_bexit) : nullptr;
     if (d_exit_map) MH_HIP(hipMemsetAsync(nd.halo_first, 0xff, 8 * (size_t)W, s));
-    MH_HIP(hipMemsetAsync(nd.inflow, 0, o_next - o_inflow, s));
+    if (!prepared) MH_HIP(hipMemsetAsync(nd.inflow, 0, o_next - o_inflow, s));
     const unsigned gn = (unsigned)cdiv(nnodes, 256);
     const bool walk_final = (!(fixed_top || fixed_bot) || halo_zero) && (!d_exit_map || halo_zero) && H * W < (int64_t)0x7fffffff;
     if (walk_final)
diff --git a/malstroem_amd/csrc/common.hpp b/malstroem_amd/csrc/common.hpp
--- a/malstroem_amd/csrc/common.hpp
+++ b/malstroem_amd/csrc/common.hpp
@@ -270,6 +270,8 @@
     uint8_t *d8_out = nullptr;
     unsigned int *d8_nodir = nullptr;
     bool d8_done = false;
+    bool defer_out = false;
+    bool out_deferred = false;
     FillHandover *handover = nullptr;
     struct Impl;
     Impl *impl;
@@ -287,7 +289,10 @@
     uint8_t *flowdir = nullptr;
     unsigned int *nodir = nullptr;
     bool done = false;
-};
+    uint32_t *dist = nullptr;
+    bool defer = false, deferred = false;
+};
+int noflat_assemble_dev(const float *d_filled, const uint32_t *d_dist, double *d_out, int64_t n, double seed_add, hipStream_t s);
 int fill_noflat_geodesic_dev(const float *d_dem, const float *d_filled, double *d_out, int64_t H, int64_t W, double sh, double dg, double seed_add,
                              hipStream_t s, FillStats *st, bool *partial, StageHook *tail_hook = nullptr, D8Sink *d8 = nullptr, FillHandover *ho = nullptr);
 int noflat_verify_dev(const float *d_dem, const double *d_out, int64_t H, int64_t W, double sh, double dg, hipStream_t s, bool *ok, int fixed_top = 0,
@@ -341,8 +346,16 @@
     int fixed_top = 0, fixed_bot = 0;
     bool valid = false;
 };
+struct AccumPrep {
+    DevBuf nodes;
+    int64_t H = 0, W = 0;
+    hipEvent_t ready = nullptr;
+    bool valid = false;
+    ~AccumPrep();
+};
+int accum_prepare_dev(AccumPrep *prep, int64_t H, int64_t W, hipStream_t s, hipEvent_t ready);
 int accum_dev(const uint8_t *d_fd, double *d_out, int64_t H, int64_t W, hipStream_t s, int fixed_top = 0, int fixed_bot = 0, int halo_zero = 0,
-              int32_t *d_exit_map = nullptr, PourLink *pour = nullptr, AccumKeep *keep = nullptr);
+              int32_t *d_exit_map = nullptr, PourLink *pour = nullptr, AccumKeep *keep = nullptr, AccumPrep *prep = nullptr);
 int accum_band_delta_dev(const uint8_t *d_fd, double *d_out, int64_t H, int64_t W, hipStream_t s, int fixed_top, int fixed_bot, AccumKeep *keep, bool *done);
 int ccl8_f32_dev(const float *d_data, int32_t *d_labels, int32_t *d_tmp, int64_t H, int64_t W, int64_t *nlabels,
                  hipStream_t s, DevBuf *stats_out = nullptr);
diff --git a/malstroem_amd/csrc/ctx.hip b/malstroem_amd/csrc/ctx.hip
--- a/malstroem_amd/csrc/ctx.hip
+++ b/malstroem_amd/csrc/ctx.hip
@@ -27,6 +27,7 @@
 {
     switch (which) {
     case MHIP_R_DEM:
+        c->noflat_pending = false;
         for (int k = 0; k < MHIP_R_COUNT_; ++k) {
             if (k == MHIP_R_DEM) continue;
             c->have[k] = false;
@@ -78,6 +79,19 @@
     const bool up = kind == hipMemcpyHostToDevice;
     MH_HIP(hipMemcpyAsync(up ? (void *)dev : host, up ? host : (void *)dev, rowb * (size_t)nrows, kind, cs(c)));
     MH_HIP(stream_sync(cs(c)));
+    return MHIP_OK;
+}
+
+int ctx_noflat(mhip_ctx *c, double **g)
+{
+    if (c->noflat_pending) {
+        MH_HIP(hipSetDevice(c->device));
+        MH_TRY(noflat_assemble_dev(c->r[MHIP_R_FILLED].as<float>(), c->r[MHIP_R_NGDIST].as<uint32_t>(), c->r[MHIP_R_NOFLAT].as<double>(), c->H * c->W, 0.0,
+                                   c->stream));
+        c->noflat_pending = false;
+        if (cs(c) != c->stream) MH_HIP(stream_sync(c->stream));
+    }
+    if (g) *g = c->r[MHIP_R_NOFLAT].as<double>();
     return MHIP_OK;
 }
 
@@ -204,7 +218,7 @@
             (void)hipStreamDestroy(st);
         }
     }
-    for (hipEvent_t e : {c->ev_fork, c->ev_flowdir, c->ev_join, c->ev_label, c->ev_tail, c->ev_cand})
+    for (hipEvent_t e : {c->ev_fork, c->ev_flowdir, c->ev_join, c->ev_label, c->ev_tail, c->ev_cand, c->ev_prep})
         if (e) (void)hipEventDestroy(e);
     delete c->geo;
     delete c->pf;
@@ -258,6 +272,7 @@
            "ctx_upload_rows(ctx, which, row0, nrows, host)");
     MH_HIP(hipSetDevice(c->device));
     MH_TRY(ctx_raster(c, which));
+    MH_TRY(ctx_settle(c, which, true));
     ctx_wrote(c, which, true);
     c->have[which] = false;
     MH_TRY(ctx_copy_rows(c, c->r[which].p, raster_elem(which), row0, nrows, const_cast<void *>(host), hipMemcpyHostToDevice));
@@ -273,6 +288,7 @@
     MH_ARG(c && host && which >= 0 && which < MHIP_R_COUNT_ && row0 >= 0 && nrows >= 1 && row0 + nrows <= c->H_owned,
            "ctx_download_rows(ctx, which, row0, nrows, host)");
     MH_ARG(c->have[which], "raster has not been computed or uploaded");
+    MH_TRY(ctx_settle(c, which, false));
     return ctx_copy_rows(c, c->r[which].p, raster_elem(which), row0, nrows, host, hipMemcpyDeviceToHost);
 }
 
@@ -322,6 +338,8 @@
     if (k == "d8_steady") {
         MH_ARG(c->have[MHIP_R_NOFLAT] && !c->ht && !c->hb, "d8_steady needs the no-flats surface on an undivided context");
         MH_HIP(hipSetDevice(c->device));
+        double *g = nullptr;
+        MH_TRY(ctx_noflat(c, &g));
         MH_TRY(ctx_raster(c, MHIP_R_FLOWDIR));
         MH_TRY(c->nodir_cnt.alloc(4));
         constexpr int REPS = 16;
@@ -332,8 +350,7 @@
         MH_HIP(hipMemsetAsync(c->nodir_cnt.p, 0, 4, s));
         for (int i = 0; i < REPS + 2; ++i) {
             if (i == 2) MH_HIP(hipEventRecord(t->a, s));
-            MH_TRY(d8_dev(c->r[MHIP_R_NOFLAT].as<double>(), c->r[MHIP_R_FLOWDIR].as<uint8_t>(), c->H, c->W, 1, s, 0, c->H_global,
-                          c->nodir_cnt.as<unsigned int>()));
+            MH_TRY(d8_dev(g, c->r[MHIP_R_FLOWDIR].as<uint8_t>(), c->H, c->W, 1, s, 0, c->H_global, c->nodir_cnt.as<unsigned int>()));
         }
         MH_HIP(hipEventRecord(t->b, s));
         MH_HIP(hipEventSynchronize(t->b));
@@ -392,6 +409,7 @@
     else if (k == "flowdir_computed") *value = (c->have[MHIP_R_FLOWDIR] && c->flowdir_own) ? 1 : 0;
     else if (k == "pour_algorithm") *value = c->pour_algorithm;
     else if (k == "noflat_algorithm") *value = c->noflat_st.algorithm;
+    else if (k == "noflat_pending") *value = c->noflat_pending ? 1 : 0;
     else if (k == "noflat_visits") *value = c->noflat_st.visits;
     else if (k == "noflat_reject") *value = c->noflat_st.geo_reject;
     else if (k == "noflat_reject_irregular") *value = c->noflat_st.geo_irregular;
diff --git a/malstroem_amd/csrc/ctx.hpp b/malstroem_amd/csrc/ctx.hpp
--- a/malstroem_amd/csrc/ctx.hpp
+++ b/malstroem_amd/csrc/ctx.hpp
@@ -82,6 +82,7 @@
     hipStream_t stream = nullptr;
     mh::DevBuf r[MHIP_R_COUNT_];
     bool have[MHIP_R_COUNT_] = {};
+    bool noflat_pending = false;
     mh::DevBuf tmp_i32;
     mh::CclKeep ccl_keep;
     bool ccl_pending = false;
@@ -91,6 +92,7 @@
     int accum_algorithm = 0;
     mh::DevBuf pp_mask0, pp_list, pp_tiles, pp_misc, pp_key;
     hipEvent_t ev_cand = nullptr;
+    hipEvent_t ev_prep = nullptr;
     int pour_algorithm = 0;
     int64_t nlabels_raw = -1, nlabels = -1;
     bool labels_components = false;
@@ -180,6 +182,12 @@
 static inline bool on_side(mhip_ctx *c) { return t_side_ctx == c; }
 
 void ctx_wrote(mhip_ctx *c, int which, bool uploaded = false);
+int ctx_noflat(mhip_ctx *c, double **g = nullptr);
+inline int ctx_settle(mhip_ctx *c, int which, bool write)
+{
+    if (which == MHIP_R_NOFLAT || (write && (which == MHIP_R_FILLED || which == MHIP_R_NGDIST))) return ctx_noflat(c);
+    return MHIP_OK;
+}
 int ctx_copy_rows(mhip_ctx *c, void *dev_base, size_t elem_bytes, int64_t row0, int64_t nrows, void *host, hipMemcpyKind kind);
 int ctx_fetch(mhip_ctx *c, const DevBuf &buf, size_t bytes, void *host);
 int ctx_fork_join_events(mhip_ctx *c);
diff --git a/malstroem_amd/csrc/ctx_band.hip b/malstroem_amd/csrc/ctx_band.hip
--- a/malstroem_amd/csrc/ctx_band.hip
+++ b/malstroem_amd/csrc/ctx_band.hip
@@ -29,6 +29,7 @@
 {
     MH_ARG(c && which >= 0 && which < MHIP_R_COUNT_, usage);
     MH_ARG(c->r[which].p, "raster has not been computed or uploaded");
+    MH_TRY(ctx_settle(c, which, false));
     const int side[2] = {side0, side1};
     void *const dst[2] = {dst0, dst1};
     for (int k = 0; k < 2; ++k) MH_ARG(!dst[k] || side[k] < 2 || (side[k] == 2 ? c->ht : c->hb), "this band has no halo row on that side");
@@ -107,6 +108,7 @@
     MH_ARG(side == 0 ? c->ht : c->hb, "this band has no halo row on that side");
     MH_HIP(hipSetDevice(c->device));
     MH_TRY(ctx_raster(c, which));
+    MH_TRY(ctx_settle(c, which, true));
     int ch = 0;
     MH_TRY(row_update_dev(row_ptr(c, which, 2 + side), dev_src, (int64_t)row_bytes(c, which), &ch, cs(c)));
     if (changed) *changed = ch;
@@ -126,6 +128,7 @@
     if (!host_top && !host_bottom) return MHIP_OK;
     MH_HIP(hipSetDevice(c->device));
     MH_TRY(ctx_raster(c, which));
+    MH_TRY(ctx_settle(c, which, true));
     hipStream_t s = cs(c);
     const size_t rowb = row_bytes(c, which);
     DevBuf &stage = on_side(c) ? c->comm_stage_b : c->comm_stage;
@@ -146,6 +149,7 @@
     if (!c->ht && !c->hb) return MHIP_OK;
     MH_ARG(c->r[which].p, "raster has not been computed or uploaded");
     MH_HIP(hipSetDevice(c->device));
+    MH_TRY(ctx_settle(c, which, true));
     hipStream_t s = cs(c);
     const size_t rowb = row_bytes(c, which);
     MH_TRY(c->comm_stage.alloc(2 * rowb));
@@ -165,6 +169,7 @@
     MH_ARG(c->r[which].p, "raster has not been computed or uploaded");
     MH_ARG((!c->ht || host_from_up) && (!c->hb || host_from_down), "ctx_exchange_edge_rows: a buffer per neighbour");
     MH_HIP(hipSetDevice(c->device));
+    MH_TRY(ctx_settle(c, which, false));
     hipStream_t s = cs(c);
     const size_t rowb = row_bytes(c, which);
     DevBuf &stage = on_side(c) ? c->comm_stage_b : c->comm_stage;
@@ -201,6 +206,7 @@
     MH_ARG(c && which >= 0 && which < MHIP_R_COUNT_, "ctx_zero_raster(ctx, which)");
     MH_HIP(hipSetDevice(c->device));
     MH_TRY(ctx_raster(c, which));
+    MH_TRY(ctx_settle(c, which, true));
     ctx_wrote(c, which);
     MH_HIP(hipMemsetAsync(c->r[which].p, 0, raster_elem(which) * (size_t)(c->H * c->W), cs(c)));
     return MHIP_OK;
@@ -517,6 +523,7 @@
     } else {
         const int src = which == 2 ? MHIP_R_ACCUM : MHIP_R_NOFLAT;
         MH_ARG(c->have[src], which == 2 ? "pour points need the accumulated flow" : "pour points need the no-flats surface");
+        MH_TRY(ctx_settle(c, src, false));
         MH_TRY(label_arg_dev(c->r[src].as<double>() + off, c->r[MHIP_R_LABELS].as<int32_t>() + off, c->H_owned, c->W, c->nlabels,
                              which == 2, buf.as<mhip_index_record>(), cs(c), c->labels_components));
         hipLaunchKernelGGL(global_rows_kernel, dim3((unsigned)cdiv(nrec, 256)), dim3(256), 0, cs(c), buf.as<mhip_index_record>(), nrec,
@@ -609,6 +616,7 @@
     MH_HIP(hipSetDevice(c->device));
     const int which = kind ? MHIP_R_NOFLAT : MHIP_R_FILLED;
     MH_TRY(ctx_raster(c, which));
+    MH_TRY(ctx_settle(c, which, true));
     ctx_wrote(c, which);
     if (kind == 0) {
         const bool force_iter = [] { const char *e = dev_env("MHIP_FILL"); return e && std::string(e) == "iterative"; }();
@@ -657,6 +665,7 @@
     const int which = kind ? MHIP_R_NOFLAT : MHIP_R_FILLED;
     MH_ARG(c->r[which].p, "ctx_fill_attach: the raster to start from does not exist");
     MH_HIP(hipSetDevice(c->device));
+    MH_TRY(ctx_settle(c, which, true));
     ctx_wrote(c, which);
     if (kind == 0) {
         delete c->pf;
@@ -675,7 +684,9 @@
     MH_ARG(c && ok && c->have[MHIP_R_NOFLAT] && c->have[MHIP_R_DEM], "ctx_noflat_verify(ctx, ok) needs the no-flats surface");
     MH_HIP(hipSetDevice(c->device));
     bool good = false;
-    MH_TRY(noflat_verify_dev(c->r[MHIP_R_DEM].as<float>(), c->r[MHIP_R_NOFLAT].as<double>(), c->H, c->W, c->sh, c->dg, c->stream, &good, c->ht, c->hb));
+    double *g = nullptr;
+    MH_TRY(ctx_noflat(c, &g));
+    MH_TRY(noflat_verify_dev(c->r[MHIP_R_DEM].as<float>(), g, c->H, c->W, c->sh, c->dg, c->stream, &good, c->ht, c->hb));
     *ok = good ? 1 : 0;
     return MHIP_OK;
 }
@@ -805,6 +816,7 @@
     MH_HIP(hipSetDevice(c->device));
     MH_TRY(ctx_raster(c, MHIP_R_NOFLAT));
     MH_TRY(ctx_raster(c, MHIP_R_NGDIST));
+    MH_TRY(ctx_noflat(c));
     ctx_wrote(c, MHIP_R_NOFLAT);
     delete c->geo;
     GeoRun *g = c->geo = new GeoRun();
diff --git a/malstroem_amd/csrc/ctx_run.hip b/malstroem_amd/csrc/ctx_run.hip
--- a/malstroem_amd/csrc/ctx_run.hip
+++ b/malstroem_amd/csrc/ctx_run.hip
@@ -8,11 +8,18 @@
 
 constexpr int LABEL_START_DEFAULT = 3;
 constexpr int FILL_HANDOVER_DEFAULT = 1;
+constexpr int NOFLAT_LAZY_DEFAULT = 1;
 
 static bool fill_handover_env()
 {
     const char *e = dev_env("MHIP_FILL_HANDOVER");
     return e ? e[0] != '0' : FILL_HANDOVER_DEFAULT != 0;
+}
+
+static bool noflat_lazy_env()
+{
+    const char *e = dev_env("MHIP_NOFLAT_LAZY");
+    return e ? e[0] != '0' : NOFLAT_LAZY_DEFAULT != 0;
 }
 
 static int stage_depths(mhip_ctx *c, hipStream_t s)
@@ -70,6 +77,7 @@
     const int64_t H = c->H, W = c->W, n = H * W;
     MH_ARG(c->have[MHIP_R_DEM], "NOFLAT needs the DEM");
     MH_TRY(ctx_raster(c, MHIP_R_NOFLAT));
+    c->noflat_pending = false;
     MH_TRY(stage_begin(c, MHIP_STAGE_NOFLAT, s));
     if (!shdg_done) {
         if ((c->have[MHIP_R_FILLED] || (ho && ho->pending)) && c->fill_st.have_minmax) short_diag_from_minmax(c->fill_st.dem_min, c->fill_st.dem_max, c->fill_st.dem_nan, &c->sh, &c->dg);
@@ -91,6 +99,11 @@
         MH_HIP(hipMemsetAsync(c->nodir_cnt.p, 0, 4, s));
         d8.flowdir = c->r[MHIP_R_FLOWDIR].as<uint8_t>();
         d8.nodir = c->nodir_cnt.as<unsigned int>();
+        if (c->nranks == 1 && noflat_lazy_env()) {
+            MH_TRY(ctx_raster(c, MHIP_R_NGDIST));
+            d8.dist = c->r[MHIP_R_NGDIST].as<uint32_t>();
+            d8.defer = true;
+        }
     }
     const int rc_nf = fill_noflat_dev(c->r[MHIP_R_DEM].as<float>(), c->r[MHIP_R_NOFLAT].as<double>(), H, W, c->sh, c->dg, s, &st,
                                       c->r[MHIP_R_FILLED].as<float>(), tail_hook, d8.flowdir ? &d8 : nullptr, ho);
@@ -102,19 +115,21 @@
     c->noflat_st = st;
     ctx_wrote(c, MHIP_R_NOFLAT);
     c->have[MHIP_R_NOFLAT] = true;
+    c->noflat_pending = d8.deferred;
     return MHIP_OK;
 }
 
 static int stage_flowdir(mhip_ctx *c, hipStream_t s)
 {
     MH_ARG(c->have[MHIP_R_NOFLAT], "FLOWDIR needs the no-flats surface");
+    double *g = nullptr;
+    MH_TRY(ctx_noflat(c, &g));
     MH_TRY(ctx_raster(c, MHIP_R_FLOWDIR));
     MH_TRY(stage_begin(c, MHIP_STAGE_FLOWDIR, s));
     ctx_wrote(c, MHIP_R_FLOWDIR);
     MH_TRY(c->nodir_cnt.alloc(4));
     MH_HIP(hipMemsetAsync(c->nodir_cnt.p, 0, 4, s));
-    MH_TRY(d8_dev(c->r[MHIP_R_NOFLAT].as<double>(), c->r[MHIP_R_FLOWDIR].as<uint8_t>(), c->H, c->W, 1, s, c->row0 - c->ht,
-                  c->H_global, c->nodir_cnt.as<unsigned int>()));
+    MH_TRY(d8_dev(g, c->r[MHIP_R_FLOWDIR].as<uint8_t>(), c->H, c->W, 1, s, c->row0 - c->ht, c->H_global, c->nodir_cnt.as<unsigned int>()));
     MH_TRY(stage_end(c, MHIP_STAGE_FLOWDIR, s));
     c->have[MHIP_R_FLOWDIR] = true;
     c->flowdir_own = true;
@@ -133,7 +148,7 @@
     return MHIP_OK;
 }
 
-static int stage_accum(mhip_ctx *c, hipStream_t s, PourLink *pour = nullptr)
+static int stage_accum(mhip_ctx *c, hipStream_t s, PourLink *pour = nullptr, AccumPrep *prep = nullptr)
 {
     MH_ARG(c->have[MHIP_R_FLOWDIR], "ACCUM needs flow directions");
     MH_TRY(ctx_raster(c, MHIP_R_ACCUM));
@@ -144,7 +159,8 @@
     c->accum_algorithm = delta_done ? 1 : 0;
     ctx_wrote(c, MHIP_R_ACCUM);
     if (!delta_done)
-        MH_TRY(accum_dev(c->r[MHIP_R_FLOWDIR].as<uint8_t>(), c->r[MHIP_R_ACCUM].as<double>(), c->H, c->W, s, c->ht, c->hb, 0, nullptr, pour));
+        MH_TRY(accum_dev(c->r[MHIP_R_FLOWDIR].as<uint8_t>(), c->r[MHIP_R_ACCUM].as<double>(), c->H, c->W, s, c->ht, c->hb, 0, nullptr, pour, nullptr,
+                         prep));
     MH_TRY(stage_end(c, MHIP_STAGE_ACCUM, s));
     c->have[MHIP_R_ACCUM] = true;
     return MHIP_OK;
@@ -220,6 +236,8 @@
     MH_TRY(ctx_ensure_labels_final(c, s));
     MH_TRY(ctx_label_max(c, s));
     MH_TRY(c->pour.alloc(sizeof(mhip_index_record) * (size_t)(c->nlabels + 1)));
+    double *g = nullptr;
+    if (!c->have[MHIP_R_ACCUM]) MH_TRY(ctx_noflat(c, &g));
     MH_TRY(stage_begin(c, MHIP_STAGE_POURPOINTS, s));
     bool from_keys = false;
     if (pour && pour->consumed && c->have[MHIP_R_ACCUM]) {
@@ -236,8 +254,7 @@
         MH_TRY(label_arg_dev(c->r[MHIP_R_ACCUM].as<double>(), c->r[MHIP_R_LABELS].as<int32_t>(), H, W, c->nlabels, true,
                              c->pour.as<mhip_index_record>(), s, c->labels_components));
     else
-        MH_TRY(label_arg_dev(c->r[MHIP_R_NOFLAT].as<double>(), c->r[MHIP_R_LABELS].as<int32_t>(), H, W, c->nlabels, false,
-                             c->pour.as<mhip_index_record>(), s));
+        MH_TRY(label_arg_dev(g, c->r[MHIP_R_LABELS].as<int32_t>(), H, W, c->nlabels, false, c->pour.as<mhip_index_record>(), s));
     MH_TRY(stage_end(c, MHIP_STAGE_POURPOINTS, s));
     c->pour_valid = true;
     return MHIP_OK;
@@ -294,6 +311,7 @@
     if (!c->stream_c) MH_TRY(side_stream(&c->stream_c));
     MH_TRY(ctx_fork_join_events(c));
     if (!c->ev_cand) MH_HIP(hipEventCreateWithFlags(&c->ev_cand, hipEventDisableTiming));
+    if (!c->ev_prep) MH_HIP(hipEventCreateWithFlags(&c->ev_prep, hipEventDisableTiming));
     hipStream_t sb = c->stream_b;
     const bool do_fill = (mask & MHIP_STAGE_FILL) != 0;
     MH_ARG(c->have[MHIP_R_DEM] || !(mask & (MHIP_STAGE_FILL | MHIP_STAGE_NOFLAT)), "FILL / NOFLAT need the DEM");
@@ -328,6 +346,8 @@
     pour_link.wait = [](void *a) { return static_cast<CandHand *>(a)->f.get(); };
     static const bool pour_pass = [] { const char *e = dev_env("MHIP_POUR"); return e && std::string(e) == "pass"; }();
     PourLink *const pour = ((mask & MHIP_STAGE_ACCUM) && (mask & MHIP_STAGE_WATERSHED) && (mask & MHIP_STAGE_POURPOINTS) && !pour_pass) ? &pour_link : nullptr;
+    AccumPrep acc_prep;
+    const bool prep_accum = (mask & MHIP_STAGE_ACCUM) && (mask & (MHIP_STAGE_NOFLAT | MHIP_STAGE_FLOWDIR)) && !c->ht && !c->hb;
     const bool ws_needs_new_flowdir = (mask & MHIP_STAGE_WATERSHED) && (mask & MHIP_STAGE_FLOWDIR);
     int rc_b = MHIP_OK;
     char err_b[512] = "";
@@ -383,6 +403,7 @@
             if (c->fill_st.have_minmax) short_diag_from_minmax(c->fill_st.dem_min, c->fill_st.dem_max, c->fill_st.dem_nan, &c->sh, &c->dg);
             else MH_TRY(short_diag_dev(c->r[MHIP_R_DEM].as<float>(), c->H * c->W, &c->sh, &c->dg, s));
         }
+        if (prep_accum) MH_TRY(accum_prepare_dev(&acc_prep, c->H, c->W, c->stream_c, c->ev_prep));
         const int label_start = label_start_env();
         const bool owed = ho && ho->pending;
         if (label_start == 0 && !owed) tail_hook.fire(s);
@@ -399,7 +420,7 @@
     }();
     tail_hook.fire(s);
     flowdir_ready.set_value(rc_a);
-    if (rc_a == MHIP_OK && (mask & MHIP_STAGE_ACCUM)) rc_a = stage_accum(c, s, pour);
+    if (rc_a == MHIP_OK && (mask & MHIP_STAGE_ACCUM)) rc_a = stage_accum(c, s, pour, &acc_prep);
     const int rc_l = label_fut.get();
     if (rc_a == MHIP_OK && rc_l == MHIP_OK && (mask & MHIP_STAGE_POURPOINTS)) {
         rc_a = hipStreamWaitEvent(s, c->ev_label, 0) == hipSuccess ? stage_pourpoints(c, s, pour) : MHIP_EHIP;
diff --git a/malstroem_amd/csrc/noflat_geo.hip b/malstroem_amd/csrc/noflat_geo.hip
--- a/malstroem_amd/csrc/noflat_geo.hip
+++ b/malstroem_amd/csrc/noflat_geo.hip
@@ -1046,6 +1046,17 @@
     }
 }
 
+__device__ __forceinline__ double ng_value(float f, uint32_t dd, double seed_add, bool *beyond)
+{
+    *beyond = false;
+    if (dd == D_IRR) return (double)f + seed_add;
+    if (dd >= 0x80000000u) {
+        *beyond = true;
+        return (double)f + seed_add;
+    }
+    return dd ? (double)f + (double)dd * class_ulp(class_above(f)) : (double)f;
+}
+
 __global__ __launch_bounds__(256) void ng_assemble_kernel(const float *__restrict__ F, const uint32_t *__restrict__ d, double *__restrict__ G, int64_t n,
                                                           double seed_add, unsigned long long *counters)
 {
@@ -1053,13 +1064,10 @@
     if (i0 >= n) return;
     unsigned bad = 0;
     auto value = [&](float f, uint32_t dd) {
-        if (dd == D_IRR) return (double)f + seed_add;
-        if (dd >= 0x80000000u) {
-            ++bad;
-            return (double)f + seed_add;
-        }
-        const uint32_t e = class_above(f);
-        return dd ? (double)f + (double)dd * class_ulp(e) : (double)f;
+        bool beyond;
+        const double v = ng_value(f, dd, seed_add, &beyond);
+        bad += beyond ? 1u : 0u;
+        return v;
     };
     if (i0 + 4 <= n) {
         const float4 f = *reinterpret_cast<const float4 *>(F + i0);
@@ -1070,7 +1078,7 @@
     } else {
         for (int64_t i = i0; i < n; ++i) G[i] = value(F[i], d[i]);
     }
-    if (bad) atomicAdd(&counters[C_UNREACHED], (unsigned long long)bad);
+    if (bad && counters) atomicAdd(&counters[C_UNREACHED], (unsigned long long)bad);
 }
 
 constexpr int VRB = 16;
@@ -1129,7 +1137,7 @@
     const uint32_t lo = from_right((uint32_t)b), hi = from_right((uint32_t)(b >> 32));
     return __longlong_as_double((long long)(((uint64_t)hi << 32) | lo));
 }
-template <bool D8>
+template <bool D8, bool STORE = true>
 __global__ __launch_bounds__(256) void ng_finish_kernel(const float *__restrict__ F, const uint32_t *__restrict__ d, const float *__restrict__ dem,
                                                         double *__restrict__ G, int64_t H, int64_t W, double sh, double dg, double seed_add, int fixed_top,
                                                         int fixed_bot, unsigned long long *counters, uint8_t *__restrict__ flowdir, unsigned int *nodir)
@@ -1145,14 +1153,10 @@
     unsigned unreached = 0, bad = 0, anynodir = 0;
     auto value = [&](int64_t r) -> double {
         if (!(r >= 0 && r < H && col_in)) return PINF;
-        const float f = F[r * W + cc];
-        const uint32_t dd = d[r * W + cc];
-        if (dd == D_IRR) return (double)f + seed_add;
-        if (dd >= 0x80000000u) {
-            unreached += mine && r >= rb && r < rb + FRB ? 1u : 0u;
-            return (double)f + seed_add;
-        }
-        return dd ? (double)f + (double)dd * class_ulp(class_above(f)) : (double)f;
+        bool beyond;
+        const double v = ng_value(F[r * W + cc], d[r * W + cc], seed_add, &beyond);
+        unreached += beyond && mine && r >= rb && r < rb + FRB ? 1u : 0u;
+        return v;
     };
     double a = value(rb - 1), b = value(rb);
     for (int i = 0; i < FRB; ++i) {
@@ -1170,7 +1174,7 @@
             }
             const bool halo = (r == 0 && fixed_top) || (r == H - 1 && fixed_bot);
             bad += (b == want || halo) ? 0u : 1u;
-            G[r * W + c] = b;
+            if (STORE) G[r * W + c] = b;
             if (D8) {
                 unsigned code;
                 if (r == 0 || r == H - 1 || c == 0 || c == W - 1) code = edge_code(r, c, H - 1, W - 1);
@@ -1201,12 +1205,10 @@
 #define NG_FINISH_RESIDENCY
 #endif
 #if NG_FINISH_AHEAD
-template <>
-__global__ __launch_bounds__(256) NG_FINISH_RESIDENCY void ng_finish_kernel<true>(const float *__restrict__ F, const uint32_t *__restrict__ d,
-                                                                                  const float *__restrict__ dem, double *__restrict__ G, int64_t H, int64_t W,
-                                                                                  double sh, double dg, double seed_add, int fixed_top, int fixed_bot,
-                                                                                  unsigned long long *counters, uint8_t *__restrict__ flowdir,
-                                                                                  unsigned int *nodir)
+template <bool STORE>
+__device__ __forceinline__ void ng_finish_ahead(const float *__restrict__ F, const uint32_t *__restrict__ d, const float *__restrict__ dem,
+                                                double *__restrict__ G, int64_t H, int64_t W, double sh, double dg, double seed_add, int fixed_top,
+                                                int fixed_bot, unsigned long long *counters, uint8_t *__restrict__ flowdir, unsigned int *nodir)
 {
     const int lane = threadIdx.x & 63, wave = threadIdx.x >> 6;
     const int64_t c = ((int64_t)blockIdx.x * 4 + wave) * TI + lane - 1;
@@ -1227,12 +1229,10 @@
     };
     auto value = [&](int64_t r, const Row &x) -> double {
         if (!(r >= 0 && r < H && col_in)) return PINF;
-        if (x.dd == D_IRR) return (double)x.f + seed_add;
-        if (x.dd >= 0x80000000u) {
-            unreached += mine && r >= rb && r < rb + FRB ? 1u : 0u;
-            return (double)x.f + seed_add;
-        }
-        return x.dd ? (double)x.f + (double)x.dd * class_ulp(class_above(x.f)) : (double)x.f;
+        bool beyond;
+        const double v = ng_value(x.f, x.dd, seed_add, &beyond);
+        unreached += beyond && mine && r >= rb && r < rb + FRB ? 1u : 0u;
+        return v;
     };
     const Row xa = load(rb - 1), xb = load(rb);
     Row x0 = load(rb + 1), x1{0.0f, 0.0f, 0u};
@@ -1255,7 +1255,7 @@
             }
             const bool halo = (r == 0 && fixed_top) || (r == H - 1 && fixed_bot);
             bad += (b == want || halo) ? 0u : 1u;
-            G[r * W + c] = b;
+            if (STORE) G[r * W + c] = b;
             unsigned code;
             if (r == 0 || r == H - 1 || c == 0 || c == W - 1) code = edge_code(r, c, H - 1, W - 1);
             else {
@@ -1281,6 +1281,18 @@
     if (bad) atomicAdd(&counters[C_MISMATCH], (unsigned long long)bad);
     if (__any(anynodir != 0u) && lane == 0) *nodir = 1u;
 }
+#define NG_FINISH_AHEAD_KERNEL(STORE)                                                                                                                  \
+    template <>                                                                                                                                        \
+    __global__ __launch_bounds__(256) NG_FINISH_RESIDENCY void ng_finish_kernel<true, STORE>(                                                          \
+        const float *__restrict__ F, const uint32_t *__restrict__ d, const float *__restrict__ dem, double *__restrict__ G, int64_t H, int64_t W,      \
+        double sh, double dg, double seed_add, int fixed_top, int fixed_bot, unsigned long long *counters, uint8_t *__restrict__ flowdir,              \
+        unsigned int *nodir)                                                                                                                           \
+    {                                                                                                                                                  \
+        ng_finish_ahead<STORE>(F, d, dem, G, H, W, sh, dg, seed_add, fixed_top, fixed_bot, counters, flowdir, nodir);                                  \
+    }
+NG_FINISH_AHEAD_KERNEL(true)
+NG_FINISH_AHEAD_KERNEL(false)
+#undef NG_FINISH_AHEAD_KERNEL
 #endif
 
 uint32_t class_weight(double eps, int e)
@@ -1537,7 +1549,12 @@
     d8_done = false;
     const bool with_d8 = !partial && d8_out && d8_nodir && !fixed_top && !fixed_bot;
     if (tail_hook) tail_hook->fire_at(StageHook::FINISH, s);
-    if (with_d8)
+    const bool no_store = with_d8 && defer_out;
+    out_deferred = false;
+    if (no_store)
+        hipLaunchKernelGGL((ng_finish_kernel<true, false>), dim3((unsigned)((W + 4 * TI - 1) / (4 * TI)), (unsigned)((H + FRB - 1) / FRB)), dim3(256), 0, s, filled, dist,
+                           dem, out, H, W, sh, dg, seed_add, fixed_top, fixed_bot, m.d_cnt, d8_out, d8_nodir);
+    else if (with_d8)
         hipLaunchKernelGGL(ng_finish_kernel<true>, dim3((unsigned)((W + 4 * TI - 1) / (4 * TI)), (unsigned)((H + FRB - 1) / FRB)), dim3(256), 0, s, filled, dist, dem,
                            out, H, W, sh, dg, seed_add, fixed_top, fixed_bot, m.d_cnt, d8_out, d8_nodir);
     else if (!partial)
@@ -1591,7 +1608,19 @@
     }
     *ok = partial ? true : !(h_all[C_UNREACHED] || h_all[C_MISMATCH]);
     d8_done = with_d8 && !partial && *ok;
+    if (no_store) {
+        if (d8_done) out_deferred = true;
+        else MH_TRY(noflat_assemble_dev(filled, dist, out, n, seed_add, s));
+    }
     m.ws.release();
+    return MHIP_OK;
+}
+
+int noflat_assemble_dev(const float *d_filled, const uint32_t *d_dist, double *d_out, int64_t n, double seed_add, hipStream_t s)
+{
+    hipLaunchKernelGGL(ng_assemble_kernel, dim3((unsigned)((n + 1023) / 1024)), dim3(256), 0, s, d_filled, d_dist, d_out, n, seed_add,
+                       (unsigned long long *)nullptr);
+    MH_HIP(hipGetLastError());
     return MHIP_OK;
 }
 
@@ -1617,7 +1646,11 @@
     GeoRun g;
     g.handover = ho;
     g.tail_hook = tail_hook;
-    if (d8) { g.d8_out = d8->flowdir; g.d8_nodir = d8->nodir; d8->done = false; }
+    if (d8) {
+        g.d8_out = d8->flowdir; g.d8_nodir = d8->nodir; d8->done = false; d8->deferred = false;
+        if (d8->dist) g.dist = d8->dist;
+        g.defer_out = d8->defer && d8->dist;
+    }
     g.dem = d_dem; g.filled = d_filled; g.out = d_out; g.H = H; g.W = W; g.sh = sh; g.dg = dg;
     g.allow_partial = partial != nullptr && seed_add == seed_add && seed_add < 1e300;
     g.seed_add = seed_add;
@@ -1639,7 +1672,7 @@
     while (active) MH_TRY(g.batch(s, &active));
     MH_TRY(g.end(s, &ok, st));
     if (partial) *partial = g.partial;
-    if (d8) d8->done = g.d8_done;
+    if (d8) { d8->done = g.d8_done; d8->deferred = g.out_deferred; }
     if (!ok && st) st->geo_reject = 2;
     return ok ? MHIP_OK : MHIP_ELIMIT;
 }
diff --git a/malstroem_amd/csrc/pflood.hip b/malstroem_amd/csrc/pflood.hip
--- a/malstroem_amd/csrc/pflood.hip
+++ b/malstroem_amd/csrc/pflood.hip
@@ -1031,7 +1031,10 @@
                     else __builtin_amdgcn_s_sleep(48);
                 }
             }
-            if (blk >= 0) (void)atomicExch(&sa.mark_cur[blk], 2u);
+            if (blk >= 0) {
+                (void)atomicExch(&sa.mark_cur[blk], 2u);
+                asm volatile("s_waitcnt vmcnt(0)" ::: "memory");
+            }
             s_blk = blk;
             s_wake = 0;
         }
```

Measured after the change: 12900 Mcells/s (median of 6 runs). 1.02x the previous value.
